# Luckick/EAGCN

Hardware: AMD Instinct MI355X
Metric: molecules/sec fwd+bwd, 2-layer 5-view EAGCN, Tox21 batch (higher is better)
Workload: dtype f32 (bf16x3 split, fp32 accumulate): every fp32 operand leaves its producer as three bf16 planes, six v_mfma_f32_32x32x16_bf16 piece products per 16 k rebuild the fp32 product (csrc/gemm_bx3.hip); aggregation, BatchNorm, head, first layer fp32

## Files before the change

eagcn_amd/_lib.py:

```python
import ctypes as C
import os

_HERE = os.path.dirname(os.path.abspath(__file__))
LIB_PATH = os.path.join(_HERE, 'lib', 'libeagcn_hip.so')

MAX_VIEWS = 8
MAX_SEGS = 8
META_WORDS = 16
META_NLOG = 8
META_T, META_NMAX, META_NTILES, META_BAD_ADJ, META_BAD_REL, META_NEDGE, META_OVERFLOW, META_EDGE_OVERFLOW = range(8)
META_NBLK = 9
STRUCT_CONCATE, STRUCT_WEIGHTED = 0, 1

_fp = C.c_void_p


class Batch(C.Structure):
    _fields_ = [('B', C.c_int32), ('N', C.c_int32), ('K', C.c_int32), ('ldc', C.c_int32),
                ('T', C.c_int32), ('n_max', C.c_int32), ('n_tiles', C.c_int32),
                ('channels', C.c_int32 * MAX_VIEWS),
                ('code', _fp), ('deg_bn', _fp), ('nat', _fp), ('row0', _fp), ('tile0', _fp),
                ('meta', _fp), ('row_mol', _fp), ('row_loc', _fp), ('row_m', _fp), ('row_deg', _fp),
                ('tile_mol', _fp), ('row_info', _fp), ('tile_info', _fp),
                ('rel_vec', _fp * MAX_VIEWS), ('rel_c', C.c_int32 * MAX_VIEWS),
# ... 33 lines not shown
    _fields_ = [('K', C.c_int32), ('mode', C.c_int32), ('att_c', C.c_int32 * MAX_VIEWS), ('att_w', _fp * MAX_VIEWS),
                ('ave_a', _fp), ('self_r', _fp), ('datt_w', _fp * MAX_VIEWS), ('dave_a', _fp), ('dself_r', _fp)]


class Layout(C.Structure):
    _fields_ = [('nseg', C.c_int32), ('width', C.c_int32 * MAX_SEGS), ('pad', C.c_int32 * MAX_SEGS)]


class LayerParams(C.Structure):
    _fields_ = [('K', C.c_int32), ('structure', C.c_int32), ('training', C.c_int32),
                ('width', C.c_int32 * MAX_VIEWS), ('inp', Layout),
                ('dropout', C.c_float), ('bn_eps', C.c_float), ('bn_momentum', C.c_float),
                ('seed', C.c_uint64), ('seed_dev', _fp),
                ('att_w', _fp * MAX_VIEWS), ('self_r', _fp * MAX_VIEWS), ('W', _fp * MAX_VIEWS),
                ('bias', _fp * MAX_VIEWS), ('gamma', _fp * MAX_VIEWS), ('beta', _fp * MAX_VIEWS),
                ('run_mean', _fp * MAX_VIEWS), ('run_var', _fp * MAX_VIEWS), ('ave_w', _fp)]


class LayerBufs(C.Structure):
    _fields_ = [('x', _fp), ('P', _fp), ('Y', _fp), ('rscale', _fp), ('bn', _fp), ('xout', _fp),
                ('pad_row', _fp), ('scratch', _fp), ('scratch_bytes', C.c_size_t),
                ('aux_stream', _fp), ('packed', _fp), ('packed_bytes', C.c_size_t),
                ('stats_hook', _fp), ('stats_user', _fp), ('x_planes', _fp), ('xout_planes', _fp)]


class LayerGrads(C.Structure):
    _fields_ = [('dW', _fp * MAX_VIEWS), ('dbias', _fp * MAX_VIEWS), ('dgamma', _fp * MAX_VIEWS),
                ('dbeta', _fp * MAX_VIEWS), ('datt_w', _fp * MAX_VIEWS), ('dself_r', _fp * MAX_VIEWS),
                ('dave_w', _fp)]


class HeadParams(C.Structure):
    _fields_ = [('f_in', C.c_int32), ('n_den1', C.c_int32), ('n_den2', C.c_int32), ('nclass', C.c_int32),
                ('dropout', C.c_float), ('bn_eps', C.c_float), ('bn_momentum', C.c_float),
                ('den1_w', _fp), ('den2_w', _fp), ('den3_w', _fp),
                ('gbn_w', _fp), ('gbn_b', _fp), ('gbn_rm', _fp), ('gbn_rv', _fp),
                ('bn1_w', _fp), ('bn1_b', _fp), ('bn1_rm', _fp), ('bn1_rv', _fp),
                ('bn2_w', _fp), ('bn2_b', _fp), ('bn2_rm', _fp), ('bn2_rv', _fp)]


class HeadGrads(C.Structure):
    _fields_ = [(n, _fp) for n in ('d_den1_w', 'd_den2_w', 'd_den3_w', 'd_gbn_w', 'd_gbn_b', 'd_bn1_w', 'd_bn1_b',
                                   'd_bn2_w', 'd_bn2_b')]


class Model(C.Structure):
    _fields_ = [('n_layers', C.c_int32), ('molfp_mode', C.c_int32), ('training', C.c_int32),
                ('head_seed', C.c_uint64), ('head_seed_dev', _fp), ('input_packed', C.c_int32), ('aux_stream', _fp),
                ('layer', LayerParams * 4), ('head', HeadParams), ('stats_hook', _fp), ('stats_user', _fp),
                ('stats_world', C.c_int32), ('fuse_readout', C.c_int32), ('fwd_signal', _fp), ('wait_flag', _fp), ('start_signal', _fp)]


class StepLoss(C.Structure):
    _fields_ = [('kind', C.c_int32), ('labels', _fp), ('class_weight', _fp), ('loss', _fp), ('scale', _fp), ('dout', _fp)]


ALLREDUCE_FN = C.CFUNCTYPE(C.c_int, C.c_void_p, C.c_int, C.c_void_p, C.c_void_p)


SIGNATURES = {
    'eagcn_abi_version': (C.c_int, []),
    'eagcn_struct_size': (C.c_size_t, [C.c_int]),
    'eagcn_last_error': (C.c_char_p, []),
    'eagcn_pad16': (C.c_int, [C.c_int]),
    'eagcn_layer_out_ld': (C.c_int, [C.POINTER(LayerParams)]),
    'eagcn_layer_fp': (C.c_int, [C.POINTER(LayerParams)]),
    'eagcn_layer_packed_bytes': (C.c_size_t, [C.POINTER(Batch), C.POINTER(LayerParams)]),
    'eagcn_layer_fwd_scratch_bytes': (C.c_size_t, [C.POINTER(Batch), C.POINTER(LayerParams)]),
    'eagcn_layer_bwd_scratch_bytes': (C.c_size_t, [C.POINTER(Batch), C.POINTER(LayerParams)]),
    'eagcn_index_build': (C.c_int, [_fp, C.POINTER(_fp), C.POINTER(Batch), _fp, _fp]),
    'eagcn_index_from_bonds': (C.c_int, [_fp, _fp, _fp, _fp, C.c_int64, C.POINTER(Batch), _fp, _fp]),
    'eagcn_index_rows': (C.c_int, [C.POINTER(Batch), _fp]),
    'eagcn_set_gemm_mode': (C.c_int, [C.c_int]),
    'eagcn_stream_wait_counter': (C.c_int, [_fp, C.c_uint32, _fp]),
    'eagcn_stream_signal_flag': (C.c_int, [_fp, _fp]),
    'eagcn_stream_wait_flag': (C.c_int, [_fp, C.c_double, _fp]),
    'eagcn_stream_wait_timeouts': (C.c_int, []),
    'eagcn_stream_wait_reset': (None, []),
    'eagcn_adam_step': (C.c_int, [_fp, _fp, _fp, _fp, C.c_int64, _fp, _fp, _fp, _fp]),
    'eagcn_agg_wants_bond_lists': (C.c_int, [C.c_int, C.c_int]),
    'eagcn_agg_wants_bond_lists_for': (C.c_int, [C.c_int, C.c_int, C.c_int]),
    'eagcn_bx3_used_splits': (C.c_int, [C.c_int, C.c_int, C.c_int, C.c_int]),
    'eagcn_set_bx3_wide': (C.c_int, [C.c_int]),
    'eagcn_bx3_pair_used_splits': (C.c_int, [C.c_int] * 7),
    'eagcn_bx3_plane_elems': (C.c_size_t, [C.c_int, C.c_int]),
    'eagcn_bx3_split': (C.c_int, [_fp, C.c_int, C.c_int, _fp, C.c_size_t, C.c_int, C.c_int, _fp]),
    'eagcn_gemm_bx3': (C.c_int, [C.c_int, C.c_int, C.c_int, C.c_int, _fp, C.c_size_t, C.c_int, C.c_int, _fp, C.c_size_t, C.c_int, C.c_int,
                                 _fp, C.c_int, C.c_int, C.c_size_t, C.c_int, _fp]),
    'eagcn_gemm_bx3_pair': (C.c_int, [C.c_int, C.c_int, C.c_int, _fp, C.c_size_t, C.c_int, C.c_int, _fp, C.c_size_t, C.c_int, C.c_int, _fp, C.c_int,
                                      C.c_int, C.c_int, C.c_int, _fp, C.c_size_t, C.c_int, C.c_int, _fp, C.c_size_t, C.c_int, C.c_int, _fp, C.c_int,
                                      C.c_int, C.c_size_t, C.c_int, _fp]),
    'eagcn_pack_rows': (C.c_int, [C.POINTER(Batch), _fp, C.c_int, C.POINTER(Layout), _fp, _fp]),
    'eagcn_unpack_rows': (C.c_int, [C.POINTER(Batch), _fp, C.POINTER(Layout), _fp, _fp, C.c_int, _fp]),
    'eagcn_pad_rows': (C.c_int, [_fp, _fp, C.c_int, C.c_int, C.c_int, _fp, _fp]),
    'eagcn_gat_scratch_bytes': (C.c_size_t, [C.POINTER(Batch), C.c_int]),
    'eagcn_gat_forward': (C.c_int, [C.POINTER(Batch), C.POINTER(GatParams), _fp, _fp, _fp, _fp, _fp]),
    'eagcn_gat_backward': (C.c_int, [C.POINTER(Batch), C.POINTER(GatParams), _fp, _fp, _fp, _fp, _fp, _fp, _fp, _fp, _fp,
                                     C.c_size_t, _fp]),
    'eagcn_pool_scratch_bytes': (C.c_size_t, []),
    'eagcn_pool_attention_forward': (C.c_int, [C.POINTER(Batch), C.POINTER(PoolAtt), _fp, C.c_int, _fp, _fp, _fp]),
    'eagcn_pool_attention_backward': (C.c_int, [C.POINTER(Batch), C.POINTER(PoolAtt), _fp, C.c_int, _fp, _fp, _fp, C.c_size_t,
                                                _fp]),
    'eagcn_pool_mix_forward': (C.c_int, [C.POINTER(Batch), C.POINTER(Layout), _fp, C.c_int, _fp, _fp, _fp, _fp, C.c_int, _fp]),
    'eagcn_pool_mix_backward': (C.c_int, [C.POINTER(Batch), C.POINTER(Layout), _fp, C.c_int, _fp, _fp, _fp, _fp, C.c_int, _fp,
                                          _fp, _fp, _fp]),
    'eagcn_pool_reduce_forward': (C.c_int, [C.POINTER(Batch), _fp, C.c_int, C.c_int, C.c_int, _fp, _fp, _fp, _fp]),
    'eagcn_pool_reduce_backward': (C.c_int, [C.POINTER(Batch), _fp, C.c_int, C.c_int, C.c_int, _fp, _fp, _fp, _fp, _fp]),
    'eagcn_layer_forward': (C.c_int, [C.POINTER(Batch), C.POINTER(LayerParams), C.POINTER(LayerBufs), _fp]),
    'eagcn_layer_backward': (C.c_int, [C.POINTER(Batch), C.POINTER(LayerParams), C.POINTER(LayerBufs),
                                       _fp, _fp, _fp, C.POINTER(LayerGrads), _fp]),
    'eagcn_attention_dense': (C.c_int, [C.POINTER(Batch), C.POINTER(LayerParams), _fp, _fp]),
    'eagcn_readout_forward': (C.c_int, [C.POINTER(Batch), _fp, C.POINTER(Layout), _fp, _fp, C.c_int, _fp,
                                        C.c_int, _fp]),
    'eagcn_readout_backward': (C.c_int, [C.POINTER(Batch), _fp, C.POINTER(Layout), _fp, C.c_int, C.c_int,
                                         _fp, _fp, _fp]),
    'eagcn_gemm_f32': (C.c_int, [C.c_int, C.c_int, C.c_int, C.c_int, C.c_int, _fp, C.c_int, _fp, C.c_int,
                                 _fp, C.c_int, _fp]),
    'eagcn_gemm_f32_dev': (C.c_int, [C.c_int, C.c_int, C.c_int, C.c_int, C.c_int, _fp, C.c_int, _fp, C.c_int,
                                     _fp, C.c_int, _fp, C.c_int, _fp]),
    'eagcn_gemm_sk_workspace_bytes': (C.c_size_t, []),
    'eagcn_gemm_f32_sk': (C.c_int, [C.c_int, C.c_int, C.c_int, C.c_int, C.c_int, _fp, C.c_int, _fp, C.c_int,
                                    _fp, C.c_int, _fp, C.c_size_t, _fp]),
    'eagcn_gemm_pair_sk': (C.c_int, [C.c_int, C.c_int, C.c_int, _fp, C.c_int, _fp, C.c_int, _fp, C.c_int,
                                     C.c_int, C.c_int, C.c_int, _fp, C.c_int, _fp, C.c_int, _fp, C.c_int,
                                     _fp, C.c_size_t, _fp]),
    'eagcn_gemm_pair_sk_slabs': (C.c_int, [C.c_int, C.c_int, C.c_int, _fp, C.c_int, _fp, C.c_int, _fp, C.c_int,
                                           C.c_int, C.c_int, C.c_int, _fp, C.c_int, _fp, C.c_int, _fp, C.c_int,
                                           C.c_size_t, _fp, C.c_size_t, _fp]),
    'eagcn_gemm_sk_plan': (C.c_int, [C.c_int] * 7 + [C.POINTER(C.c_int), C.POINTER(C.c_int)]),
    'eagcn_gemm_sk_timeouts': (C.c_int, []),
    'eagcn_gemm_sk_failed': (C.c_int, []),
    'eagcn_gemm_sk_reset_failed': (None, []),
    'eagcn_gemm_sk_inject_failure': (None, []),
    'eagcn_model_saved_bytes': (C.c_size_t, [C.POINTER(Batch), C.POINTER(Model)]),
    'eagcn_model_scratch_bytes': (C.c_size_t, [C.POINTER(Batch), C.POINTER(Model)]),
    'eagcn_model_atom_rep': (C.c_int, [C.POINTER(Batch), C.POINTER(Model), C.POINTER(C.c_size_t),
                                       C.POINTER(C.c_size_t), C.POINTER(C.c_int)]),
    'eagcn_model_atom_rep_materialize': (C.c_int, [C.POINTER(Batch), C.POINTER(Model), _fp, C.c_size_t, _fp]),
    'eagcn_model_pack_input': (C.c_int, [C.POINTER(Batch), C.POINTER(Model), _fp, _fp, C.c_size_t, _fp]),
    'eagcn_model_forward': (C.c_int, [C.POINTER(Batch), C.POINTER(Model), _fp, _fp, _fp, C.c_size_t, _fp,
                                      C.c_size_t, _fp, _fp, _fp]),
    'eagcn_model_backward': (C.c_int, [C.POINTER(Batch), C.POINTER(Model), _fp, _fp, C.c_size_t, _fp, C.c_size_t,
                                       _fp, _fp, C.POINTER(LayerGrads), C.POINTER(HeadGrads), _fp]),
    'eagcn_model_backward_range': (C.c_int, [C.POINTER(Batch), C.POINTER(Model), _fp, _fp, C.c_size_t, _fp, C.c_size_t,
                                             _fp, _fp, C.POINTER(LayerGrads), C.POINTER(HeadGrads), C.c_int, C.c_int, C.c_int, _fp]),
    'eagcn_model_input_scratch_bytes': (C.c_size_t, [C.POINTER(Batch), C.POINTER(Model)]),
    'eagcn_model_backward_input': (C.c_int, [C.POINTER(Batch), C.POINTER(Model), _fp, _fp, C.c_size_t, _fp, C.c_size_t,
                                             _fp, _fp, C.POINTER(LayerGrads), C.POINTER(HeadGrads), _fp, _fp]),
    'eagcn_attr_alpha': (C.c_float, [C.c_int, C.c_int]),
    'eagcn_attr_weight': (C.c_float, [C.c_int]),
    'eagcn_attr_acc_elems': (C.c_size_t, [C.POINTER(Batch), C.POINTER(Model)]),
    'eagcn_attr_pack_input': (C.c_int, [C.POINTER(Batch), C.POINTER(Model), _fp, _fp, C.c_float, _fp, C.c_size_t, _fp]),
    'eagcn_attr_step': (C.c_int, [C.POINTER(Batch), C.POINTER(Model), _fp, _fp, C.c_size_t, _fp, C.c_size_t, _fp, _fp, C.c_float,
                                  C.c_int, _fp, _fp]),
    'eagcn_attr_finalize': (C.c_int, [C.POINTER(Batch), C.POINTER(Model), _fp, _fp, _fp, _fp, _fp, _fp]),
    'eagcn_model_forward_step': (C.c_int, [C.POINTER(Batch), C.POINTER(Model), _fp, _fp, _fp, C.c_size_t, _fp, C.c_size_t, _fp, _fp,
                                           C.POINTER(StepLoss), _fp, C.POINTER(HeadGrads), _fp]),
    'eagcn_head_saved_bytes': (C.c_size_t, [C.POINTER(HeadParams), C.c_int]),
    'eagcn_head_scratch_bytes': (C.c_size_t, [C.POINTER(HeadParams), C.c_int]),
    'eagcn_head_forward': (C.c_int, [C.POINTER(HeadParams), C.c_int, C.c_int, C.c_uint64, _fp, _fp, _fp, C.c_size_t, _fp, C.c_size_t,
                                     _fp, _fp, _fp]),
    'eagcn_head_backward': (C.c_int, [C.POINTER(HeadParams), C.c_int, C.c_int, C.c_uint64, _fp, _fp, _fp, C.c_size_t, _fp, C.c_size_t,
                                      _fp, _fp, C.POINTER(HeadGrads), _fp, _fp]),
    'eagcn_bce_loss': (C.c_int, [_fp, _fp, _fp, C.c_int, C.c_int, _fp, _fp, _fp]),
    'eagcn_mse_loss': (C.c_int, [_fp, _fp, C.c_int, _fp, _fp, _fp]),
    'eagcn_eval_append': (C.c_int, [_fp, _fp, C.c_int, C.c_int, C.c_int, _fp, _fp, _fp, C.c_int64, _fp]),
# ... 65 lines not shown
```

eagcn_amd/build.py:

```python
import os
import shutil
import subprocess
import sys
from concurrent.futures import ThreadPoolExecutor

HERE = os.path.dirname(os.path.abspath(__file__))
CSRC = os.path.join(HERE, 'csrc')
LIBDIR = os.path.join(HERE, 'lib')
LIB = os.path.join(LIBDIR, 'libeagcn_hip.so')
HIP_SOURCES = ['index.hip', 'gemm.hip', 'gemm3.hip', 'gemm_bx3.hip', 'gemm_bx3w.hip', 'agg.hip', 'lagg.hip', 'lagg_in.hip', 'gat.hip', 'pool.hip', 'layer.hip', 'readout.hip', 'head.hip', 'head2.hip', 'loss.hip', 'attr.hip']
CPP_SOURCES = ['api.cpp']
HEADERS = ['common.h', 'kernels.h', 'lagg_kernel.h', 'gemm_x6.h', 'bx3.h', os.path.join('..', '..', 'include', 'eagcn_hip.h')]
ARCH = 'gfx950'


def _hipcc():
    for cand in (shutil.which('hipcc'), '/opt/rocm/bin/hipcc'):
        if cand and os.path.exists(cand):
            return cand
    raise RuntimeError('hipcc not found: the EAGCN HIP library cannot be built')


def _newest(paths):
    return max(os.path.getmtime(p) for p in paths)


def needs_build():
    srcs = [os.path.join(CSRC, s) for s in HIP_SOURCES + CPP_SOURCES + HEADERS if os.path.exists(os.path.join(CSRC, s))]
    return (not os.path.exists(LIB)) or os.path.getmtime(LIB) < _newest(srcs)


def build_library(force=False, verbose=False):
    if not force and not needs_build():
        return LIB
    hipcc = _hipcc()
    os.makedirs(LIBDIR, exist_ok=True)
    objdir = os.path.join(LIBDIR, 'obj')
    os.makedirs(objdir, exist_ok=True)
    flags = ['--offload-arch=' + ARCH, '-O3', '-std=c++17', '-fPIC', '-Wall', '-Wno-unused-function', '-munsafe-fp-atomics']

    hdr_time = _newest([os.path.join(CSRC, h) for h in HEADERS if os.path.exists(os.path.join(CSRC, h))])

    def compile_one(src):
        obj = os.path.join(objdir, os.path.splitext(src)[0] + '.o')
        if not force and os.path.exists(obj) and os.path.getmtime(obj) > max(hdr_time, os.path.getmtime(os.path.join(CSRC, src))):
            return obj
        cmd = [hipcc] + flags + ['-c', os.path.join(CSRC, src), '-o', obj]
        if src.endswith('.cpp'):
            cmd = [hipcc, '-O2', '-std=c++17', '-fPIC', '-c', os.path.join(CSRC, src), '-o', obj]
        r = subprocess.run(cmd, capture_output=True, text=True)
        if r.returncode != 0:
            raise RuntimeError('hipcc failed on %s:\n%s\n%s' % (src, r.stdout, r.stderr))
        if verbose and r.stderr.strip():
            print(r.stderr, file=sys.stderr)
        return obj

    sources = [s for s in HIP_SOURCES + CPP_SOURCES if os.path.exists(os.path.join(CSRC, s))]
    with ThreadPoolExecutor(max_workers=min(8, len(sources))) as ex:
        objs = list(ex.map(compile_one, sources))
    tmp = LIB + '.tmp'
    r = subprocess.run([hipcc, '--offload-arch=' + ARCH, '-shared', '-fPIC', '-o', tmp] + objs,
                       capture_output=True, text=True)
    if r.returncode != 0:
        raise RuntimeError('link failed:\n%s\n%s' % (r.stdout, r.stderr))
    os.replace(tmp, LIB)
    return LIB


if __name__ == '__main__':
    print(build_library(force='--force' in sys.argv, verbose=True))
```

eagcn_amd/csrc/attr.hip:

```cpp
#include <algorithm>

#include "common.h"
#include "kernels.h"

namespace eagcn {

__device__ __forceinline__ int attr_exact_to_packed(const ColMapD& m, int ce) {
    int eo = 0, po = 0;
    for (int s = 0; s < m.nseg; ++s) {
        if (ce < eo + m.w[s]) return po + (ce - eo);
        eo += m.w[s];
        po += m.p[s];
    }
    return -1;
}
__device__ __forceinline__ int attr_packed_to_exact(const ColMapD& m, int cp) {
    int eo = 0, po = 0;
    for (int s = 0; s < m.nseg; ++s) {
        if (cp < po + m.p[s]) return cp - po < m.w[s] ? eo + (cp - po) : -1;
        eo += m.w[s];
        po += m.p[s];
    }
    return -1;
}
// ... 7 lines not shown
        float v = 0.0f;
        if (ce >= 0) {
            const size_t i = ((size_t)bt.row_mol[r] * Nin + bt.row_loc[r]) * F + ce;
            const float b0 = base ? base[i] : 0.0f;
            v = fmaf(alpha, x[i] - b0, b0);
        }
        packed[e] = v;
    }
}

__global__ __launch_bounds__(256) void attr_accumulate_kernel(eagcn_batch bt, const float* __restrict__ g, float w, int ld, int first,
                                                               float* __restrict__ acc) {
    const uint32_t n4 = (uint32_t)dev_rows(bt) * (uint32_t)ld / 4;
    float4* a4 = reinterpret_cast<float4*>(acc);
    const float4* g4 = reinterpret_cast<const float4*>(g);
    for (uint32_t e = blockIdx.x * blockDim.x + threadIdx.x; e < n4; e += gridDim.x * blockDim.x) {
        const float4 v = g4[e];
        float4 o = first ? make_float4(0.f, 0.f, 0.f, 0.f) : a4[e];
        o.x = fmaf(w, v.x, o.x); o.y = fmaf(w, v.y, o.y); o.z = fmaf(w, v.z, o.z); o.w = fmaf(w, v.w, o.w);
        a4[e] = o;
    }
}

__global__ __launch_bounds__(256) void attr_dense_kernel(eagcn_batch bt, const float* __restrict__ acc, ColMapD m, int ld, int F, int Nin,
                                                          const float* __restrict__ x, const float* __restrict__ base,
                                                          float* __restrict__ attr, float* __restrict__ score) {
    const int nrow = bt.B * Nin;
    for (int q = blockIdx.x * blockDim.x + threadIdx.x; q < nrow; q += gridDim.x * blockDim.x) {
        const int b = q / Nin, i = q - b * Nin;
        const bool stored = i < bt.nat[b] && bt.row0[b] + i < dev_rows(bt);
        const float* ar = acc + (size_t)(stored ? bt.row0[b] + i : 0) * ld;
        const size_t o = (size_t)q * F;
        float s = 0.0f;
        for (int f = 0; f < F; ++f) {
            float v = 0.0f;
            if (stored) {
                v = ar[attr_exact_to_packed(m, f)];
                if (x) v *= x[o + f] - (base ? base[o + f] : 0.0f);
            }
            attr[o + f] = v;
            s += v;
        }
        if (score) score[q] = s;
    }
}

static inline int attr_grid(size_t n) { return (int)std::max<size_t>(1, std::min<size_t>((n + 255) / 256, 4096)); }
static inline int attr_nin(const eagcn_batch* b) { return b->n_logical > 0 ? b->n_logical : b->N; }

int launch_attr_dense(const eagcn_batch* b, const eagcn_layout* in, const float* acc, const float* x, const float* base, float* attr,
                      float* score, hipStream_t s) {
    const int Nin = attr_nin(b);
    ProfScope ps(PROF_PACK, s);
    attr_dense_kernel<<<attr_grid((size_t)b->B * Nin), 256, 0, s>>>(*b, acc, make_colmap(in), layout_ld(in), layout_width(in), Nin, x,
                                                                   base, attr, score);
    EAGCN_LAUNCH_CHECK();
    return EAGCN_OK;
}

}

using namespace eagcn;

extern "C" float eagcn_attr_alpha(int step, int steps) { return steps > 0 ? ((float)step + 0.5f) / (float)steps : 0.0f; }
extern "C" float eagcn_attr_weight(int steps) { return steps > 0 ? 1.0f / (float)steps : 0.0f; }

extern "C" size_t eagcn_attr_acc_elems(const eagcn_batch* b, const eagcn_model* m) {
    return (b && m) ? (size_t)std::max(b->T, 1) * layout_ld(&m->layer[0].in) : 0;
}

extern "C" int eagcn_attr_pack_input(const eagcn_batch* b, const eagcn_model* m, const float* afm, const float* baseline, float alpha,
                                     void* saved, size_t saved_bytes, void* stream) {
    EAGCN_CHECK_ARG(b && m && afm && saved, "eagcn_attr_pack_input: null argument");
    float* x0 = nullptr;
    int rc = model_input_slot(b, m, saved, saved_bytes, &x0, "eagcn_attr_pack_input");
    if (rc) return rc;
    if (b->T == 0) return EAGCN_OK;
    const eagcn_layout* in = &m->layer[0].in;
    hipStream_t s = (hipStream_t)stream;
    ProfScope ps(PROF_PACK, s);
    attr_pack_kernel<<<attr_grid((size_t)b->T * layout_ld(in)), 256, 0, s>>>(*b, afm, baseline, alpha, make_colmap(in), layout_ld(in),
                                                                           layout_width(in), attr_nin(b), x0);
    EAGCN_LAUNCH_CHECK();
    return EAGCN_OK;
}

extern "C" int eagcn_attr_step(const eagcn_batch* b, const eagcn_model* m, const int64_t* size, void* saved, size_t saved_bytes,
                               void* scratch, size_t scratch_bytes, const float* dout, const float* dgraph_rep, float weight, int first,
                               float* acc, void* stream) {
    EAGCN_CHECK_ARG(b && m && acc, "eagcn_attr_step: null argument");
    const int ld = layout_ld(&m->layer[0].in);
    EAGCN_CHECK_ARG((ld & 3) == 0 && (reinterpret_cast<uintptr_t>(acc) & 15) == 0,
                    "eagcn_attr_step: accumulator not 16-byte aligned / input row width %d not a multiple of 4", ld);
    float* dx0 = nullptr;
    int rc = model_backward_input_packed(b, m, size, saved, saved_bytes, scratch, scratch_bytes, dout, dgraph_rep, nullptr, nullptr,
                                         &dx0, stream, "eagcn_attr_step");
    if (rc) return rc;
    if (b->T == 0) return EAGCN_OK;
    hipStream_t s = (hipStream_t)stream;
    ProfScope ps(PROF_PACK, s);
    attr_accumulate_kernel<<<attr_grid((size_t)b->T * ld / 4), 256, 0, s>>>(*b, dx0, weight, ld, first ? 1 : 0, acc);
    EAGCN_LAUNCH_CHECK();
    return EAGCN_OK;
}

extern "C" int eagcn_attr_finalize(const eagcn_batch* b, const eagcn_model* m, const float* afm, const float* baseline, const float* acc,
                                   float* attr, float* score, void* stream) {
    EAGCN_CHECK_ARG(b && m && afm && attr && score, "eagcn_attr_finalize: null argument");
    EAGCN_CHECK_ARG(b->T == 0 || acc, "eagcn_attr_finalize: null accumulator");
    return launch_attr_dense(b, &m->layer[0].in, acc, afm, baseline, attr, score, (hipStream_t)stream);
}
```

eagcn_amd/csrc/head.hip:

```cpp
#include <stdlib.h>

#include <algorithm>

#include "common.h"
#include "kernels.h"

namespace eagcn {

__global__ void wait_counter_kernel(const uint32_t* __restrict__ word, uint32_t value, int* __restrict__ err,
                                    unsigned long long budget_ticks) {
    if (threadIdx.x == 0) {
        const unsigned long long t0 = wall_clock64();
        while ((int32_t)(__hip_atomic_load(word, __ATOMIC_ACQUIRE, __HIP_MEMORY_SCOPE_AGENT) - value) < 0) {
            __builtin_amdgcn_s_sleep(64);
            if (wall_clock64() - t0 > budget_ticks) {
                if (err) __hip_atomic_store(err, 1, __ATOMIC_RELAXED, __HIP_MEMORY_SCOPE_SYSTEM);
                break;
            }
        }
    }
}



// ... 156 lines not shown
    EAGCN_CHECK_ARG(h->f_in >= 1 && h->n_den1 >= 1 && h->n_den2 >= 1 && h->nclass >= 1, "%s: bad head sizes", who);
    EAGCN_CHECK_ARG(h->den1_w && h->den2_w && h->den3_w && h->gbn_w && h->gbn_b && h->gbn_rm && h->gbn_rv &&
                        h->bn1_w && h->bn1_b && h->bn1_rm && h->bn1_rv && h->bn2_w && h->bn2_b && h->bn2_rm &&
                        h->bn2_rv, "%s: null head parameter", who);
    const eagcn_layer_params* last = &m->layer[m->n_layers - 1];
    const int f_last = last->structure == EAGCN_STRUCT_CONCATE ? [&] { int s = 0; for (int k = 0; k < last->K; ++k) s += last->width[k]; return s; }()
                                                                 : last->width[0];
    EAGCN_CHECK_ARG(f_last == h->f_in, "%s: head expects %d features, last layer yields %d", who, h->f_in, f_last);
    EAGCN_CHECK_ARG(!m->training || b->B > 1, "%s: BatchNorm in training mode needs more than one molecule", who);
    return EAGCN_OK;
}

static eagcn_layout out_layout(const eagcn_layer_params* p) {
    eagcn_layout l;
    memset(&l, 0, sizeof(l));
    if (p->structure == EAGCN_STRUCT_CONCATE) {
        l.nseg = p->K;
        for (int k = 0; k < p->K; ++k) { l.width[k] = p->width[k]; l.pad[k] = pad16(p->width[k]); }
    } else {
        l.nseg = 1;
        l.width[0] = p->width[0];
        l.pad[0] = pad16(p->width[0]);
    }
    return l;
}

static bool fused_readout(const eagcn_model* m) {
    static const bool env = [] { const char* v = getenv("EAGCN_NO_FUSED_READOUT"); return !(v && v[0] == '1'); }();
    return env && m->fuse_readout && m->layer[m->n_layers - 1].structure == EAGCN_STRUCT_CONCATE;
}

static bool hidden_planes_only(const eagcn_batch* b, const eagcn_model* m, const ModelSaved& sv, int l) {
    return l + 1 < m->n_layers && sv.L[l].xout_planes && layer_reads_planes_only(b, &m->layer[l + 1], m->aux_stream != nullptr);
}

static void fill_drop(float p, int training, int* do_drop, uint32_t* thr, float* inv_keep) {
    *do_drop = (training && p > 0.0f) ? 1 : 0;
    *thr = (uint32_t)std::min(4294967295.0, (double)p * 4294967296.0);
    *inv_keep = 1.0f / (1.0f - p);
}

}

using namespace eagcn;

#define RC(call) do { int rc_ = (call); if (rc_) return rc_; } while (0)

extern "C" size_t eagcn_model_saved_bytes(const eagcn_batch* b, const eagcn_model* m) {
    return carve_saved(nullptr, b, m, nullptr);
}
extern "C" size_t eagcn_model_scratch_bytes(const eagcn_batch* b, const eagcn_model* m) {
    return carve_scratch(nullptr, b, m, nullptr);
}
extern "C" int eagcn_model_atom_rep(const eagcn_batch* b, const eagcn_model* m, size_t* xout_offset,
                                    size_t* pad_row_offset, int* ld) {
    EAGCN_CHECK_ARG(b && m && xout_offset && pad_row_offset && ld, "eagcn_model_atom_rep: null argument");
    ModelSaved s;
    carve_saved(nullptr, b, m, &s);
    *xout_offset = s.xout_last_off;
    *pad_row_offset = s.pad_last_off;
    *ld = eagcn_layer_out_ld(&m->layer[m->n_layers - 1]);
    return EAGCN_OK;
}

extern "C" int eagcn_model_atom_rep_materialize(const eagcn_batch* b, const eagcn_model* m, void* saved, size_t saved_bytes,
                                                 void* stream) {
    EAGCN_CHECK_ARG(b && m && saved, "eagcn_model_atom_rep_materialize: null argument");
    if (!fused_readout(m)) return EAGCN_OK;
    ModelSaved sv;
    EAGCN_CHECK_ARG(carve_saved(saved, b, m, &sv) <= saved_bytes, "eagcn_model_atom_rep_materialize: saved block too small");
    const int l = m->n_layers - 1;
    LayerSaved& L = sv.L[l];
    eagcn_layer_bufs w;
    memset(&w, 0, sizeof(w));
    w.Y = L.Y; w.bn = L.bn; w.xout = L.xout; w.pad_row = L.pad_row; w.packed = L.packed; w.packed_bytes = L.packed_bytes;
    return layer_apply_impl(b, &m->layer[l], &w, stream);
}

extern "C" int eagcn_model_pack_input(const eagcn_batch* b, const eagcn_model* m, const float* afm, void* saved,
                                      size_t saved_bytes, void* stream) {
    EAGCN_CHECK_ARG(b && m && afm && saved, "eagcn_model_pack_input: null argument");
    ModelSaved sv;
    EAGCN_CHECK_ARG(carve_saved(saved, b, m, &sv) <= saved_bytes, "eagcn_model_pack_input: saved block too small");
    return eagcn_pack_rows(b, afm, layout_width(&m->layer[0].in), &m->layer[0].in, sv.x0, stream);
}

struct HeadPlan {
    HeadFwd f1, f2, f3;
    HeadBwd b3, b2, b1;
    HeadGbn bg;
    double *st_g, *st_1, *st_2, *sb_g, *sb_1, *sb_2;
    bool sync;
};
static HeadPlan head_plan(const eagcn_batch* b, const eagcn_model* m, const ModelSaved& sv, const ModelScratch& sc, float* out,
                          float* graph_rep, const float* dout, const float* dgraph_rep, const eagcn_head_grads* hg) {
    HeadPlan P;
    const eagcn_head_params* h = &m->head;
    const int B = b->B, F = h->f_in, n1 = h->n_den1, n2 = h->n_den2, nc = h->nclass;
    P.st_g = sc.hst; P.st_1 = sc.hst + 2 * F + 2; P.st_2 = sc.hst + 2 * (F + n1) + 4;
    P.sb_g = sc.hsb; P.sb_1 = sc.hsb + 2 * F + 2; P.sb_2 = sc.hsb + 2 * (F + n1) + 4;
    P.sync = m->stats_hook && m->training;
    const int copies = P.sync ? 1 : HEAD_COPIES;
    HeadDrop nodrop{0, 0u, 1.0f, 0, nullptr}, drop1 = nodrop;
    {
        int on; uint32_t thr; float inv_keep;
        fill_drop(h->dropout, m->training, &on, &thr, &inv_keep);
        drop1 = HeadDrop{on, thr, inv_keep, m->head_seed, m->head_seed_dev};
    }
    P.f1 = HeadFwd{B, F, n1, sv.g, P.st_g, h->gbn_w, h->gbn_b, h->gbn_rm, h->gbn_rv, sv.bn_g, h->den1_w, sv.h1, nullptr, P.st_1,
                   m->training, 0, h->bn_eps, h->bn_momentum, nodrop};
    P.f2 = HeadFwd{B, n1, n2, sv.h1, P.st_1, h->bn1_w, h->bn1_b, h->bn1_rm, h->bn1_rv, sv.bn_1, h->den2_w, sv.h2, graph_rep, P.st_2,
                   m->training, 1, h->bn_eps, h->bn_momentum, drop1};
    P.f3 = HeadFwd{B, n2, nc, sv.h2, P.st_2, h->bn2_w, h->bn2_b, h->bn2_rm, h->bn2_rv, sv.bn_2, h->den3_w, out, nullptr, nullptr,
                   m->training, 1, h->bn_eps, h->bn_momentum, nodrop};
    if (P.sync) { P.f1.cnt_in = P.st_g + 2 * F; P.f2.cnt_in = P.st_1 + 2 * n1; P.f3.cnt_in = P.st_2 + 2 * n2; }
    P.f3.nw = 8;
    P.f1.signal = m->fwd_signal;
    P.f1.st_copies = P.f2.st_copies = P.f3.st_copies = copies;
    P.f1.st_stride = P.f2.st_stride = P.f3.st_stride = sc.n_hst;
    if (!hg) return P;
    const double *cn_g = sc.hst + 2 * F, *cn_1 = sc.hst + 2 * F + 2 + 2 * n1, *cn_2 = sc.hst + 2 * (F + n1) + 4 + 2 * n2;
    const float gscale = P.sync && m->stats_world > 1 ? 1.0f / (float)m->stats_world : 1.0f;
    P.b3 = HeadBwd{B, n2, nc, sv.h2, sv.bn_2, 1, nodrop, h->den3_w, dout, nullptr, nullptr, nullptr, nullptr, nullptr, nullptr,
                   sc.da2, P.sb_2, hg->d_den3_w, m->training};
    P.b2 = HeadBwd{B, n1, n2, sv.h1, sv.bn_1, 1, drop1, h->den2_w, sc.da2, sv.h2, sv.bn_2, P.sb_2, dgraph_rep, hg->d_bn2_w, hg->d_bn2_b,
                   sc.da1, P.sb_1, hg->d_den2_w, m->training};
    P.b1 = HeadBwd{B, F, n1, sv.g, sv.bn_g, 0, nodrop, h->den1_w, sc.da1, sv.h1, sv.bn_1, P.sb_1, nullptr, hg->d_bn1_w, hg->d_bn1_b,
                   sc.dgn, P.sb_g, hg->d_den1_w, m->training};
    if (P.sync) { P.b2.cnt_y = cn_2; P.b2.gscale = gscale; P.b1.cnt_y = cn_1; P.b1.gscale = gscale; }
    P.b3.nw = 8;
    const int ks = sc.hdw_ks;
    float* part3 = sc.hdw;
    float* part2 = part3 + (size_t)ks * n2 * nc;
    float* part1 = part2 + (size_t)ks * n1 * n2;
    if (ks > 1) {
        P.b3.ks = ks; P.b3.dW_part = part3;
        P.b2.ks = ks; P.b2.dW_part = part2;
        P.b1.ks = ks; P.b1.dW_part = part1;
    }
    P.bg = HeadGbn{B, F, sc.dgn, sv.g, sv.bn_g, P.sb_g, sc.dg, hg->d_gbn_w, hg->d_gbn_b, m->training};
    if (P.sync) { P.bg.cnt = cn_g; P.bg.gscale = gscale; }
    if (ks > 1) {
        P.bg.sum[0] = HeadDwSum{hg->d_den3_w, part3, n2 * nc, ks};
        P.bg.sum[1] = HeadDwSum{hg->d_den2_w, part2, n1 * n2, ks};
        P.bg.sum[2] = HeadDwSum{hg->d_den1_w, part1, F * n1, ks};
        P.bg.nsum = 3;
    }
    return P;
}

static int model_forward_trunk(const eagcn_batch* b, const eagcn_model* m, const float* afm, const int64_t* size, void* saved,
                               size_t saved_bytes, void* scratch, size_t scratch_bytes, ModelSaved& sv, ModelScratch& sc,
                               void* stream, const char* who) {
    hipStream_t s = (hipStream_t)stream;
    RC(check_model(b, m, who));
    EAGCN_CHECK_GEMM3(who);
    EAGCN_CHECK_ARG((afm || m->input_packed) && saved && scratch, "%s: null buffer", who);
    EAGCN_CHECK_ARG(m->molfp_mode == 0 || size, "%s: 'ave' read-out needs size", who);
    EAGCN_CHECK_ARG(carve_saved(saved, b, m, &sv) <= saved_bytes, "%s: saved block too small", who);
    EAGCN_CHECK_ARG(carve_scratch(scratch, b, m, &sc) <= scratch_bytes, "%s: scratch too small", who);
    const eagcn_head_params* h = &m->head;
    HandOff ho{m->start_signal, m->wait_flag, wait_err_word(), 200000000ull};
    if (!m->input_packed && (m->wait_flag || m->start_signal)) {
        handoff_kernel<<<1, 64, 0, s>>>(ho);
        EAGCN_LAUNCH_CHECK();
        ho.start = nullptr; ho.flag = nullptr;
    }
    ZeroJob zj;
    RC(gemm3_zero_job(sc.layer, sc.layer_bytes, sc.hst, (HEAD_COPIES + 1) * sc.n_hst + HEAD_WS, &zj));
    if (!m->input_packed)
        RC(eagcn_pack_rows(b, afm, layout_width(&m->layer[0].in), &m->layer[0].in, sv.x0, stream));
    const float* x = sv.x0;
    {
        const eagcn_layer_params* ps[4];
        void* pk[4];
        size_t pkb[4];
        for (int l = 0; l < m->n_layers; ++l) { ps[l] = &m->layer[l]; pk[l] = sv.L[l].packed; pkb[l] = sv.L[l].packed_bytes; }
        RC(pack_params_all(b, ps, pk, pkb, m->n_layers, stream, &zj, &ho));
    }
    for (int l = 0; l < m->n_layers; ++l) {
        LayerSaved& L = sv.L[l];
        eagcn_layer_bufs w;
        memset(&w, 0, sizeof(w));
        w.x = x; w.P = L.P; w.Y = L.Y; w.rscale = L.rscale; w.bn = L.bn; w.xout = L.xout; w.pad_row = L.pad_row;
        w.scratch = sc.layer; w.scratch_bytes = sc.layer_bytes; w.packed = L.packed; w.packed_bytes = L.packed_bytes;
        w.stats_hook = m->stats_hook; w.stats_user = m->stats_user;
        w.x_planes = l > 0 ? sv.L[l - 1].xout_planes : nullptr; w.xout_planes = L.xout_planes;
        const bool po = hidden_planes_only(b, m, sv, l);
        RC(layer_forward_impl(b, &m->layer[l], &w, stream, true, l == m->n_layers - 1 && fused_readout(m), po));
        x = po ? nullptr : L.xout;
    }
    const eagcn_layer_params* last = &m->layer[m->n_layers - 1];
    const LayerSaved& LL = sv.L[m->n_layers - 1];
    const eagcn_layout lay = out_layout(last);
    const int B = b->B, F = h->f_in, n1 = h->n_den1, n2 = h->n_den2;
    double *st_g = sc.hst, *st_1 = sc.hst + 2 * F + 2, *st_2 = sc.hst + 2 * (F + n1) + 4;
    const int copies = (m->stats_hook && m->training) ? 1 : HEAD_COPIES;
    if (fused_readout(m)) {
        ReadoutBn rb;
        rb.Y = LL.Y; rb.ldy = LL.fp; rb.bn = LL.bn; rb.fp = LL.fp;
        fill_drop(last->dropout, last->training, &rb.do_drop, &rb.thr, &rb.inv_keep);
        rb.seed = last->seed; rb.seed_dev = last->seed_dev;
        rb.size = size; rb.mode = m->molfp_mode; rb.g = sv.g; rb.F = F; rb.st = st_g;
        rb.cnt0 = st_g + 2 * F; rb.cnt1 = st_1 + 2 * n1; rb.cnt2 = st_2 + 2 * n2;
        rb.st_copies = copies; rb.st_stride = sc.n_hst;
        RC(readout_bn_forward(b, &lay, rb, stream));
    } else if (pad_sampled(m))
        RC(readout_forward_sampled(b, LL.xout, &lay, last, LL.bn + (size_t)LL.fp , size,
                                   m->molfp_mode, sv.g, F, sv.pad_cnt, sv.padc, sv.pad_tab, stream));
    else
        RC(eagcn_readout_forward(b, LL.xout, &lay, last->structure == EAGCN_STRUCT_WEIGHTED ? LL.pad_row : nullptr,
                                 size, m->molfp_mode, sv.g, F, stream));
    if (!fused_readout(m)) RC(head_colstats(sv.g, B, F, st_g, s, st_g + 2 * F, st_1 + 2 * n1, st_2 + 2 * n2));
    return EAGCN_OK;
}

static int stats_hook_call(const eagcn_model* m, bool sync, double* buf, int n, void* stream) {
    if (!sync) return EAGCN_OK;
    if (m->stats_hook(buf, n, stream, m->stats_user)) {
        set_error("eagcn_model: the sync-BatchNorm all-reduce hook failed");
        return EAGCN_ERR_HIP;
    }
    return EAGCN_OK;
}

static int head_forward_launches(const eagcn_model* m, const HeadPlan& P, void* stream) {
    hipStream_t s = (hipStream_t)stream;
    const eagcn_head_params* h = &m->head;
    RC(stats_hook_call(m, P.sync, P.st_g, 2 * h->f_in + 1, stream));
    RC(head_fwd(P.f1, s));
    RC(stats_hook_call(m, P.sync, P.st_1, 2 * h->n_den1 + 1, stream));
    RC(head_fwd(P.f2, s));
    RC(stats_hook_call(m, P.sync, P.st_2, 2 * h->n_den2 + 1, stream));
    RC(head_fwd(P.f3, s));
    return EAGCN_OK;
}
static int head_backward_launches(const eagcn_model* m, const HeadPlan& P, void* stream) {
    hipStream_t s = (hipStream_t)stream;
    const eagcn_head_params* h = &m->head;
    RC(head_bwd(P.b3, s));
    RC(stats_hook_call(m, P.sync, P.sb_2, 2 * h->n_den2, stream));
    RC(head_bwd(P.b2, s));
    RC(stats_hook_call(m, P.sync, P.sb_1, 2 * h->n_den1, stream));
    RC(head_bwd(P.b1, s));
    RC(stats_hook_call(m, P.sync, P.sb_g, 2 * h->f_in, stream));
    RC(head_gbn_bwd(P.bg, s));
    return EAGCN_OK;
}
static int readout_pad_backward(const eagcn_batch* b, const eagcn_model* m, const int64_t* size, const ModelSaved& sv,
                                const ModelScratch& sc, void* stream) {
    const eagcn_layer_params* last = &m->layer[m->n_layers - 1];
    const eagcn_layout lay = out_layout(last);
    const int F = m->head.f_in;
    if (pad_sampled(m)) return readout_backward_pad_views(b, sc.dg, &lay, size, m->molfp_mode, F, last->K, sv.pad_cnt, last->dropout, sc.dpad, stream);
    if (last->structure == EAGCN_STRUCT_WEIGHTED) return readout_backward_pad(b, sc.dg, &lay, size, m->molfp_mode, F, sc.dpad, stream);
    return EAGCN_OK;
}

extern "C" int eagcn_model_forward(const eagcn_batch* b, const eagcn_model* m, const float* afm,
                                   const int64_t* size, void* saved, size_t saved_bytes, void* scratch,
                                   size_t scratch_bytes, float* out, float* graph_rep, void* stream) {
    EAGCN_CHECK_ARG(out && graph_rep, "eagcn_model_forward: null buffer");
    ModelSaved sv;
    ModelScratch sc;
    RC(model_forward_trunk(b, m, afm, size, saved, saved_bytes, scratch, scratch_bytes, sv, sc, stream, "eagcn_model_forward"));
    const HeadPlan P = head_plan(b, m, sv, sc, out, graph_rep, nullptr, nullptr, nullptr);
    return head_forward_launches(m, P, stream);
}

namespace eagcn {
static int check_head(const eagcn_head_params* h, int B, int training, const char* who) {
    EAGCN_CHECK_ARG(h, "%s: null argument", who);
// ... 198 lines not shown
    pend_out.eacc = nullptr;
    for (int l = layer_hi; l >= layer_lo; --l) {
        const int t = top_l - l;
        float* cur = (t & 1) ? sc.dxb : sc.dxa;
        float* other = (t & 1) ? sc.dxa : sc.dxb;
        LayerSaved& L = sv.L[l];
        eagcn_layer_bufs w;
        memset(&w, 0, sizeof(w));
        w.x = l == 0 ? sv.x0 : (hidden_planes_only(b, m, sv, l - 1) ? nullptr : sv.L[l - 1].xout);
        w.P = L.P; w.Y = L.Y; w.rscale = L.rscale; w.bn = L.bn; w.xout = L.xout; w.pad_row = L.pad_row;
        w.scratch = sc.layer; w.scratch_bytes = sc.layer_bytes; w.packed = L.packed; w.packed_bytes = L.packed_bytes;
        w.aux_stream = m->aux_stream;
        w.stats_hook = m->stats_hook; w.stats_user = m->stats_user;
        w.x_planes = l > 0 ? sv.L[l - 1].xout_planes : nullptr;
        const bool top = l == top_l;
        const float* dpad = (weighted && top) ? sc.dpad : nullptr;
        RC(layer_backward_impl(b, &m->layer[l], &w, top ? nullptr : cur, top ? &rgd : nullptr, dpad,
                               l > 0 ? other : dx0, input_only ? nullptr : &lg[l], stream, top && sampled, top ? &zb : nullptr,
                               pend_in.eacc ? &pend_in : nullptr, (l > layer_lo && !input_only) ? &pend_out : nullptr, input_only));
        pend_in = pend_out;
        if (l == layer_lo) pend_in.eacc = nullptr;
    }
    if (forked) RC(stream_after(s, side));
    return EAGCN_OK;
}

extern "C" int eagcn_model_backward_range(const eagcn_batch* b, const eagcn_model* m, const int64_t* size, void* saved,
                                          size_t saved_bytes, void* scratch, size_t scratch_bytes, const float* dout,
                                          const float* dgraph_rep, const eagcn_layer_grads* lg,
                                          const eagcn_head_grads* hg, int with_head, int layer_hi, int layer_lo, void* stream) {
    RC(check_model(b, m, "eagcn_model_backward"));
    EAGCN_CHECK_GEMM3("eagcn_model_backward");
    return model_backward_impl(b, m, size, saved, saved_bytes, scratch, scratch_bytes, dout, dgraph_rep, lg, hg, with_head, layer_hi,
                               layer_lo, nullptr, false, stream);
}

struct InputScratch { float* dx0; eagcn_head_grads hg; };
static size_t carve_input_scratch(void* base, const eagcn_batch* b, const eagcn_model* m, InputScratch* out) {
    Carver2 c(base);
    c.off = carve_scratch(nullptr, b, m, nullptr);
    InputScratch t;
    const eagcn_head_params* h = &m->head;
    const size_t F = h->f_in, n1 = h->n_den1, n2 = h->n_den2, nc = h->nclass;
    t.dx0 = c.take<float>((size_t)std::max(b->T, 1) * layout_ld(&m->layer[0].in));
    t.hg.d_den1_w = c.take<float>(F * n1);
    t.hg.d_den2_w = c.take<float>(n1 * n2);
    t.hg.d_den3_w = c.take<float>(n2 * nc);
    t.hg.d_gbn_w = c.take<float>(F);
    t.hg.d_gbn_b = c.take<float>(F);
    t.hg.d_bn1_w = c.take<float>(n1);
    t.hg.d_bn1_b = c.take<float>(n1);
    t.hg.d_bn2_w = c.take<float>(n2);
    t.hg.d_bn2_b = c.take<float>(n2);
    if (out) *out = t;
    return c.off;
}

static int check_engine_model(const eagcn_batch* b, const eagcn_model* m, const char* who) {
    RC(check_model(b, m, who));
    EAGCN_CHECK_ARG(m->molfp_mode == 0 || m->molfp_mode == 1, "%s: read-out mode %d has no engine path", who, m->molfp_mode);
    for (int l = 0; l < m->n_layers; ++l)
        EAGCN_CHECK_ARG(m->layer[l].structure == EAGCN_STRUCT_CONCATE || m->layer[l].structure == EAGCN_STRUCT_WEIGHTED,
                        "%s: layer %d has structure %d, which the engine does not run", who, l, m->layer[l].structure);
    return EAGCN_OK;
}

int eagcn::model_backward_input_packed(const eagcn_batch* b, const eagcn_model* m, const int64_t* size, void* saved, size_t saved_bytes,
                                       void* scratch, size_t scratch_bytes, const float* dout, const float* dgraph_rep,
                                       const eagcn_layer_grads* lg, const eagcn_head_grads* hg, float** dx0, void* stream,
                                       const char* who) {
    EAGCN_CHECK_ARG(b && m, "%s: null argument", who);
    EAGCN_CHECK_ARG((lg == nullptr) == (hg == nullptr), "%s: lg and hg are both given (full backward) or both NULL (input-only)", who);
    RC(check_engine_model(b, m, who));
    EAGCN_CHECK_GEMM3(who);
    EAGCN_CHECK_ARG(saved && scratch && dout, "%s: null buffer", who);
    InputScratch is;
    EAGCN_CHECK_ARG(carve_input_scratch(scratch, b, m, &is) <= scratch_bytes, "%s: scratch too small (eagcn_model_input_scratch_bytes)", who);
    *dx0 = is.dx0;
    const bool input_only = lg == nullptr;
    return model_backward_impl(b, m, size, saved, saved_bytes, scratch, scratch_bytes, dout, dgraph_rep, lg, input_only ? &is.hg : hg, 1,
                               m->n_layers - 1, 0, is.dx0, input_only, stream);
}

int eagcn::model_input_slot(const eagcn_batch* b, const eagcn_model* m, void* saved, size_t saved_bytes, float** x0, const char* who) {
    ModelSaved sv;
    EAGCN_CHECK_ARG(carve_saved(saved, b, m, &sv) <= saved_bytes, "%s: saved block too small", who);
    *x0 = sv.x0;
    return EAGCN_OK;
}

extern "C" size_t eagcn_model_input_scratch_bytes(const eagcn_batch* b, const eagcn_model* m) {
    return (b && m) ? carve_input_scratch(nullptr, b, m, nullptr) : 0;
}

extern "C" int eagcn_model_backward_input(const eagcn_batch* b, const eagcn_model* m, const int64_t* size, void* saved,
                                          size_t saved_bytes, void* scratch, size_t scratch_bytes, const float* dout,
                                          const float* dgraph_rep, const eagcn_layer_grads* lg, const eagcn_head_grads* hg,
                                          float* dafm, void* stream) {
    EAGCN_CHECK_ARG(dafm, "eagcn_model_backward_input: null dafm");
    float* dx0 = nullptr;
    RC(model_backward_input_packed(b, m, size, saved, saved_bytes, scratch, scratch_bytes, dout, dgraph_rep, lg, hg, &dx0, stream,
                                   "eagcn_model_backward_input"));
    return launch_attr_dense(b, &m->layer[0].in, dx0, nullptr, nullptr, dafm, nullptr, (hipStream_t)stream);
}

extern "C" int eagcn_stream_signal_flag(uint32_t* flag, void* stream) {
    EAGCN_CHECK_ARG(flag != nullptr, "eagcn_stream_signal_flag: null flag");
    eagcn::signal_flag_kernel<<<1, 64, 0, (hipStream_t)stream>>>(flag);
    EAGCN_LAUNCH_CHECK();
    return EAGCN_OK;
}
extern "C" int eagcn_stream_wait_flag(uint32_t* flag, double budget_seconds, void* stream) {
    EAGCN_CHECK_ARG(flag != nullptr && budget_seconds > 0.0, "eagcn_stream_wait_flag: null flag / no budget");
    return eagcn::launch_wait_flag(flag, budget_seconds, (hipStream_t)stream);
}
extern "C" int eagcn_stream_wait_timeouts(void) {
    return eagcn::g_wait_err_host ? __atomic_load_n(eagcn::g_wait_err_host, __ATOMIC_RELAXED) : 0;
}
extern "C" void eagcn_stream_wait_reset(void) {
    if (eagcn::g_wait_err_host) __atomic_store_n(eagcn::g_wait_err_host, 0, __ATOMIC_RELAXED);
}

extern "C" int eagcn_stream_wait_counter(const uint32_t* counter, uint32_t value, void* stream) {
    EAGCN_CHECK_ARG(counter != nullptr, "eagcn_stream_wait_counter: null counter");
    eagcn::wait_counter_kernel<<<1, 64, 0, (hipStream_t)stream>>>(counter, value, eagcn::wait_err_word(), 200000000ull);
    EAGCN_LAUNCH_CHECK();
    return EAGCN_OK;
}
```

eagcn_amd/csrc/index.hip:

```cpp
#include <algorithm>

#include <stdlib.h>

#include "common.h"
#include "kernels.h"

namespace eagcn {

struct RelPtrs {
    const float* p[EAGCN_MAX_VIEWS];
    int c[EAGCN_MAX_VIEWS];
};

template <int NIT, int RPW>
__global__ __launch_bounds__(256) void index_scan_kernel(const float* __restrict__ adj, RelPtrs rel,
                                                          int B, int N, int Ncap, int K, int ldc,
                                                          uint8_t* __restrict__ code,
                                                          int32_t* __restrict__ deg_bn,
                                                          int32_t* __restrict__ nat,
                                                          int32_t* __restrict__ ecnt,
                                                          int32_t* __restrict__ meta) {
    const int lane = threadIdx.x & 63;
    const long row_first = ((long)blockIdx.x * 4 + (threadIdx.x >> 6)) * RPW;
    const long nrows = (long)B * N;
// ... 547 lines not shown
                for (int u = 0; u < 8; ++u) v[u] = (i0 + u < n && s_live[i0 + u]) ? code0[(size_t)(i0 + u) * bt.ldc + j] : 0;
#pragma unroll
                for (int u = 0; u < 8; ++u) cc += v[u] ? 1 : 0;
            }
        }
        s_ccnt[j] = cc;
    }
    __syncthreads();
    for (int pass = 0; pass < 2; ++pass) {
        int* cnt = pass ? s_ccnt : s_cnt;
        int v[4], tot = 0;
#pragma unroll
        for (int u = 0; u < 4; ++u) { const int i = tid * 4 + u; v[u] = i < n ? cnt[i] : 0; tot += v[u]; }
        s_scan[tid] = tot;
        __syncthreads();
        for (int o = 1; o < 256; o <<= 1) {
            const int x = tid >= o ? s_scan[tid - o] : 0;
            __syncthreads();
            s_scan[tid] += x;
            __syncthreads();
        }
        int run = s_scan[tid] - tot;
        __syncthreads();
#pragma unroll
        for (int u = 0; u < 4; ++u) {
            const int i = tid * 4 + u;
            if (i < n) {
                int* ptr = (pass ? bt.col_ptr : bt.row_ptr) + (size_t)(r0 + i) * 2;
                const bool fits = e0 + run + v[u] <= bt.E;
                ptr[0] = e0 + run;
                ptr[1] = fits ? v[u] : 0;
                cnt[i] = fits ? e0 + run : -1;
                run += v[u];
            }
        }
        __syncthreads();
    }
    auto codes = [&](int i, int j) -> uint64_t {
        uint8_t c[EAGCN_MAX_VIEWS];
#pragma unroll
        for (int k = 0; k < EAGCN_MAX_VIEWS; ++k) c[k] = k < bt.K ? code0[k * plane + (size_t)i * bt.ldc + j] : 0;
        uint64_t c64 = 0;
#pragma unroll
        for (int k = 0; k < EAGCN_MAX_VIEWS; ++k) c64 |= (uint64_t)c[k] << (8 * k);
        return c64;
    };
    for (int i = tid; i < n; i += 256) {
        int e = s_cnt[i];
        int ec = s_ccnt[i];
        if constexpr (BITMAP) {
            if (s_live[i] && e >= 0)
                for (int w = 0; w < Wn; ++w) {
                    uint32_t m = bits[i * W + w];
                    while (m) { const int j = 32 * w + __ffs(m) - 1; m &= m - 1u; bt.nbr[e] = j; bt.ecode[e] = codes(i, j); ++e; }
                }
            if (ec >= 0)
                for (int w = 0; w < Wn; ++w) {
                    uint32_t m = bitsT[i * W + w];
                    while (m) { const int ii = 32 * w + __ffs(m) - 1; m &= m - 1u; bt.tnbr[ec] = ii; bt.tcode[ec] = codes(ii, i); ++ec; }
                }
        } else {
            if (s_live[i] && e >= 0)
                for (int j = 0; j < n; ++j)
                    if (bond(i, j)) { bt.nbr[e] = j; bt.ecode[e] = codes(i, j); ++e; }
            if (ec >= 0)
                for (int ii = 0; ii < n; ++ii)
                    if (bond(ii, i)) { bt.tnbr[ec] = ii; bt.tcode[ec] = codes(ii, i); ++ec; }
        }
    }
}

typedef ColMapD ColMap;
__device__ __forceinline__ int packed_to_exact(const ColMap& m, int cp) {
    int eo = 0, po = 0;
    for (int s = 0; s < m.nseg; ++s) {
        if (cp < po + m.p[s]) return (cp - po < m.w[s]) ? eo + (cp - po) : -1;
        eo += m.w[s];
        po += m.p[s];
    }
    return -1;
}

__global__ __launch_bounds__(256) void pack_rows_kernel(eagcn_batch bt, const float* __restrict__ dense,
                                                         int F, ColMap m, int ld, float* __restrict__ packed, int Nin) {
    const uint32_t total = (uint32_t)dev_rows(bt) * (uint32_t)ld;
    for (uint32_t e = blockIdx.x * blockDim.x + threadIdx.x; e < total; e += gridDim.x * blockDim.x) {
        int r = (int)(e / (uint32_t)ld), cp = (int)(e - (uint32_t)r * (uint32_t)ld);
        int ce = packed_to_exact(m, cp);
        float v = 0.0f;
        if (ce >= 0) v = dense[((size_t)bt.row_mol[r] * Nin + bt.row_loc[r]) * F + ce];
        packed[e] = v;
    }
}

__global__ __launch_bounds__(256) void pad_rows_kernel(const float* __restrict__ rows, const int32_t* __restrict__ off,
                                                        int B, int N, int F, float* __restrict__ out) {
    const size_t total = (size_t)B * N * F;
    for (size_t e = (size_t)blockIdx.x * blockDim.x + threadIdx.x; e < total; e += (size_t)gridDim.x * blockDim.x) {
        const int f = (int)(e % F);
        const size_t bi = e / F;
        const int i = (int)(bi % N), b = (int)(bi / N);
        const int o = off[b], n = off[b + 1] - o;
        out[e] = i < n ? rows[(size_t)(o + i) * F + f] : 0.0f;
    }
}

__global__ __launch_bounds__(256) void unpack_rows_kernel(eagcn_batch bt, const float* __restrict__ packed,
                                                           ColMap m, int ld, const float* __restrict__ pad_row,
                                                           float* __restrict__ dense, int F) {
    const size_t total = (size_t)bt.B * bt.N * F;
    for (size_t e = (size_t)blockIdx.x * blockDim.x + threadIdx.x; e < total;
         e += (size_t)gridDim.x * blockDim.x) {
        int ce = (int)(e % F);
        size_t bi = e / F;
        int i = (int)(bi % bt.N), b = (int)(bi / bt.N);
        int eo = 0, po = 0, cp = -1;
        for (int s = 0; s < m.nseg; ++s) {
            if (ce < eo + m.w[s]) { cp = po + (ce - eo); break; }
            eo += m.w[s];
            po += m.p[s];
        }
        float v;
        if (i < bt.nat[b]) v = packed[(size_t)(bt.row0[b] + i) * ld + cp];
        else v = pad_row ? pad_row[cp] : 0.0f;
        dense[e] = v;
    }
}

}

using namespace eagcn;

extern "C" int eagcn_index_build(const float* adj, const float* const* rel, eagcn_batch* b,
                                 int32_t* host_meta, void* stream) {
    hipStream_t s = (hipStream_t)stream;
    EAGCN_CHECK_ARG(adj && rel && b && host_meta, "eagcn_index_build: null argument");
    EAGCN_CHECK_ARG(b->B > 0 && b->N > 0, "eagcn_index_build: B and N must be positive");
    EAGCN_CHECK_ARG(b->K >= 1 && b->K <= EAGCN_MAX_VIEWS, "eagcn_index_build: K=%d out of range", b->K);
    EAGCN_CHECK_ARG(b->ldc >= b->N && (b->ldc % 16) == 0, "eagcn_index_build: ldc must be a multiple of 16 >= N");
    EAGCN_CHECK_ARG(b->code && b->deg_bn && b->nat && b->row0 && b->tile0 && b->meta,
                    "eagcn_index_build: index buffers not allocated");
    RelPtrs rp;
    for (int k = 0; k < EAGCN_MAX_VIEWS; ++k) {
        rp.p[k] = k < b->K ? rel[k] : nullptr;
        rp.c[k] = k < b->K ? b->channels[k] : 0;
        if (k < b->K) {
            EAGCN_CHECK_ARG(rel[k] != nullptr, "eagcn_index_build: relation tensor %d is null", k);
            EAGCN_CHECK_ARG(rp.c[k] >= 1 && rp.c[k] <= EAGCN_MAX_CHANNELS,
                            "eagcn_index_build: view %d has %d channels (1..%d supported)", k, rp.c[k],
                            EAGCN_MAX_CHANNELS);
        }
    }
    const int Nin = b->n_logical > 0 ? b->n_logical : b->N;
    EAGCN_CHECK_ARG(Nin <= b->N, "eagcn_index_build: n_logical %d exceeds the capacity N=%d", Nin, b->N);
    ProfScope ps(PROF_INDEX, s);
    EAGCN_CHECK_ARG(b->ecnt && b->edge0, "eagcn_index_build: bond-list buffers not allocated");
    EAGCN_CHECK_ARG((long)b->B * b->N < (1L << 31), "eagcn_index_build: B * N = %ld rows", (long)b->B * b->N);
    {
        const int rcz = index_clear(b->meta, b->nat, b->ecnt, b->B, Nin < b->N ? b->deg_bn : nullptr, (long)b->B * b->N, s);
        if (rcz) return rcz;
    }
    const long rows = (long)b->B * Nin;
    constexpr int RPW = 1;
    const unsigned sgrid = (unsigned)((rows + 4 * RPW - 1) / (4 * RPW));
    const int nit = cdiv((Nin + 15) / 16 * 16, 256);
    EAGCN_CHECK_ARG(nit <= 4, "eagcn_index_build: N=%d exceeds the supported 1024 atoms", b->N);
    static const bool scan4 = [] { const char* v = getenv("EAGCN_SCAN4"); return !(v && v[0] == '0'); }();
    if (scan4) {
// ... 13 lines not shown
        switch (nit) {
            case 1: EAGCN_SCAN(1); break;
            case 2: EAGCN_SCAN(2); break;
            case 3: EAGCN_SCAN(3); break;
            default: EAGCN_SCAN(4); break;
        }
#undef EAGCN_SCAN
        EAGCN_LAUNCH_CHECK();
    }
    index_offsets_kernel<<<1, 1024, 0, s>>>(b->nat, b->B, b->deg_bn, b->B * b->N, b->row0, b->tile0, b->meta, b->T, b->ecnt, b->edge0, b->E, b->n_logical > 0 ? b->n_logical : 0);
    EAGCN_LAUNCH_CHECK();
    EAGCN_HIP(hipMemcpyAsync(host_meta, b->meta, EAGCN_META_WORDS * sizeof(int32_t), hipMemcpyDeviceToHost, s));
    return EAGCN_OK;
}

extern "C" int eagcn_index_from_bonds(const int32_t* bond_mol, const int32_t* bond_i, const int32_t* bond_j,
                                      const uint8_t* bond_code, int64_t E, eagcn_batch* b, int32_t* host_meta,
                                      void* stream) {
    hipStream_t s = (hipStream_t)stream;
    EAGCN_CHECK_ARG(b && host_meta, "eagcn_index_from_bonds: null argument");
    EAGCN_CHECK_ARG(E == 0 || (bond_mol && bond_i && bond_j && bond_code), "eagcn_index_from_bonds: null bond arrays");
    EAGCN_CHECK_ARG(b->B > 0 && b->N > 0 && b->K >= 1 && b->K <= EAGCN_MAX_VIEWS, "eagcn_index_from_bonds: bad batch shape");
    EAGCN_CHECK_ARG(b->ldc >= b->N && (b->ldc % 16) == 0, "eagcn_index_from_bonds: ldc must be a multiple of 16 >= N");
    EAGCN_CHECK_ARG(b->code && b->deg_bn && b->nat && b->row0 && b->tile0 && b->meta,
                    "eagcn_index_from_bonds: index buffers not allocated");
    RelPtrs rp;
    for (int k = 0; k < EAGCN_MAX_VIEWS; ++k) { rp.p[k] = nullptr; rp.c[k] = k < b->K ? b->channels[k] : 0; }
    ProfScope ps(PROF_INDEX, s);
    EAGCN_CHECK_ARG(b->ecnt && b->edge0, "eagcn_index_from_bonds: bond-list buffers not allocated");
    EAGCN_CHECK_ARG((long)b->B * b->N < (1L << 31), "eagcn_index_from_bonds: B * N = %ld rows", (long)b->B * b->N);
    {
        const int rcz = index_clear(b->meta, b->nat, b->ecnt, b->B, b->deg_bn, (long)b->B * b->N, s);
        if (rcz) return rcz;
    }
    EAGCN_HIP(hipMemsetAsync(b->code, 0, (size_t)b->K * b->B * b->N * b->ldc, s));
    if (E > 0) {
        const int grid = (int)std::min<long>((E + 255) / 256, 4096);
        index_bonds_kernel<<<grid, 256, 0, s>>>(bond_mol, bond_i, bond_j, bond_code, (long)E, b->B, b->N,
                                                b->n_logical > 0 ? std::min(b->n_logical, b->N) : b->N, b->K, b->ldc, rp,
                                                b->code, b->deg_bn, b->nat, b->ecnt, b->meta);
        EAGCN_LAUNCH_CHECK();
    }
    index_offsets_kernel<<<1, 1024, 0, s>>>(b->nat, b->B, b->deg_bn, b->B * b->N, b->row0, b->tile0, b->meta, b->T, b->ecnt, b->edge0, b->E, b->n_logical > 0 ? b->n_logical : 0);
    EAGCN_LAUNCH_CHECK();
    EAGCN_HIP(hipMemcpyAsync(host_meta, b->meta, EAGCN_META_WORDS * sizeof(int32_t), hipMemcpyDeviceToHost, s));
    return EAGCN_OK;
}

extern "C" int eagcn_index_rows(const eagcn_batch* b, void* stream) {
    hipStream_t s = (hipStream_t)stream;
    EAGCN_CHECK_ARG(b, "eagcn_index_rows: null batch");
    if (b->T == 0) return EAGCN_OK;
    EAGCN_CHECK_ARG(b->row_mol && b->row_loc && b->row_m && b->row_deg && b->tile_mol && b->row_info && b->tile_info,
                    "eagcn_index_rows: per-row buffers not allocated");
    EAGCN_CHECK_ARG(b->N <= 1024, "eagcn_index_rows: N=%d exceeds the supported 1024 atoms", b->N);
    EAGCN_CHECK_ARG(b->edge0 && b->mol_info && b->row_ptr && b->col_ptr && (b->E == 0 || (b->nbr && b->tnbr && b->ecode && b->tcode)),
                    "eagcn_index_rows: bond-list buffers not allocated");
    ProfScope ps(PROF_INDEX, s);
    index_rows_kernel<<<b->B, 256, 0, s>>>(*b);
    EAGCN_LAUNCH_CHECK();
    if (!b->build_lists) return EAGCN_OK;
    const int rb = b->blk ? lagg_block_rows(b) : 0;
    const int W = (b->N + 31) / 32;
    const size_t dyn = (size_t)2 * b->N * W * sizeof(uint32_t);
    static const size_t lds_cap = [] {
        int dev = 0, v = 0;
        if (hipGetDevice(&dev) != hipSuccess || hipDeviceGetAttribute(&v, hipDeviceAttributeMaxSharedMemoryPerBlock, dev) != hipSuccess) v = 64 * 1024;
        size_t cap = (size_t)v > 12 * 1024 ? (size_t)v - 12 * 1024 : 0;
        if (cap > 52 * 1024 &&
            hipFuncSetAttribute((const void*)index_csr_kernel<true>, hipFuncAttributeMaxDynamicSharedMemorySize, (int)cap) != hipSuccess) {
            (void)hipGetLastError();
            cap = 52 * 1024;
        }
        return cap;
    }();
    if (b->N <= 512 && dyn <= lds_cap) index_csr_kernel<true><<<b->B + (rb > 0 ? 1 : 0), 256, dyn, s>>>(*b, W, rb);
    else index_csr_kernel<false><<<b->B + (rb > 0 ? 1 : 0), 256, 0, s>>>(*b, W, rb);
    EAGCN_LAUNCH_CHECK();
    return EAGCN_OK;
}

extern "C" int eagcn_pack_rows(const eagcn_batch* b, const float* dense, int F, const eagcn_layout* lay,
                               float* packed, void* stream) {
    hipStream_t s = (hipStream_t)stream;
    EAGCN_CHECK_ARG(b && dense && lay && packed, "eagcn_pack_rows: null argument");
    EAGCN_CHECK_ARG(layout_width(lay) == F, "eagcn_pack_rows: layout width %d != F %d", layout_width(lay), F);
    if (b->T == 0) return EAGCN_OK;
    int ld = layout_ld(lay);
    size_t total = (size_t)b->T * ld;
    int grid = (int)std::min<size_t>((total + 255) / 256, 4096);
    ProfScope ps(PROF_PACK, s);
    pack_rows_kernel<<<grid, 256, 0, s>>>(*b, dense, F, make_colmap(lay), ld, packed, b->n_logical > 0 ? b->n_logical : b->N);
    EAGCN_LAUNCH_CHECK();
    return EAGCN_OK;
}

extern "C" int eagcn_pad_rows(const float* rows, const int32_t* mol_offset, int B, int N, int F, float* out, void* stream) {
    hipStream_t s = (hipStream_t)stream;
    EAGCN_CHECK_ARG(rows && mol_offset && out && B > 0 && N > 0 && F > 0, "eagcn_pad_rows: bad argument");
    const size_t total = (size_t)B * N * F;
    ProfScope ps(PROF_PACK, s);
    pad_rows_kernel<<<(int)std::min<size_t>((total + 255) / 256, 4096), 256, 0, s>>>(rows, mol_offset, B, N, F, out);
    EAGCN_LAUNCH_CHECK();
    return EAGCN_OK;
}

extern "C" int eagcn_unpack_rows(const eagcn_batch* b, const float* packed, const eagcn_layout* lay,
                                 const float* pad_row, float* dense, int F, void* stream) {
    hipStream_t s = (hipStream_t)stream;
    EAGCN_CHECK_ARG(b && lay && dense, "eagcn_unpack_rows: null argument");
    EAGCN_CHECK_ARG(b->T == 0 || packed, "eagcn_unpack_rows: null packed matrix");
    EAGCN_CHECK_ARG(layout_width(lay) == F, "eagcn_unpack_rows: layout width %d != F %d", layout_width(lay), F);
    int ld = layout_ld(lay);
    size_t total = (size_t)b->B * b->N * F;
    int grid = (int)std::min<size_t>((total + 255) / 256, 4096);
    ProfScope ps(PROF_PACK, s);
    unpack_rows_kernel<<<grid, 256, 0, s>>>(*b, packed, make_colmap(lay), ld, pad_row, dense, F);
    EAGCN_LAUNCH_CHECK();
    return EAGCN_OK;
}
```

eagcn_amd/csrc/kernels.h:

```cpp
#pragma once
#include "bx3.h"
#include "common.h"

namespace eagcn {

struct AggArgs {
    eagcn_batch bt;
    ViewCols vc;
    const float* src; int lds;
    float* dst; int ldd;
    const float* sig;
    const float* rsig;
    float* rscale;
    double* stats;
    int nchunk;
    int cpw = 1;
    int xcd = 0;
    bool w_rowm = false;
    BxOut planes = {nullptr, 0, 0, 0};
    const float* bn_tab = nullptr; const float* bn_cc = nullptr; int bn_fp = 0;
    const float* w_aw = nullptr;
    int w_drop = 0; uint32_t w_thr = 0; float w_inv_keep = 1.0f; uint64_t w_seed = 0; const uint64_t* w_seed_dev = nullptr;
};
int agg_grid_x(const eagcn_batch* b);
bool agg_ksplit(const eagcn_batch* b);
int launch_agg(AggArgs a, bool trans, hipStream_t s);
constexpr int LAGG_RB = 256;
constexpr int LAGG_MAXM = 16;
struct EdgeArgs;
int lagg_parts();
bool lagg_wfuse();
bool lagg_use(const eagcn_batch* b, int dir, bool absorbs_bn, const ViewCols* vc = nullptr);
bool lagg_wanted(int B, int N, int structure);
int lagg_block_rows(const eagcn_batch* b);
int lagg_slabs(const eagcn_batch* b);
int launch_lagg_fwd(AggArgs a, hipStream_t s);
int launch_lagg_bwd(AggArgs a, const EdgeArgs& e, hipStream_t s, bool edge = true);
int launch_lagg_bwd_input(const AggArgs& a, const EdgeArgs& e, dim3 grid, hipStream_t s);

struct EdgeArgs {
    eagcn_batch bt;
    ViewCols vc;
    const float* dY; const float* Y; const float* P; int ld;
    const float* sig; const float* rsig; const float* rscale;
    double* datt;
    int atomic;
    int xcd = 0;
};
constexpr int EDGE_SLAB = 264;
constexpr int EDGE_COPIES = 8;
inline size_t edge_acc_bytes() { return align256((size_t)EDGE_COPIES * EAGCN_MAX_VIEWS * EDGE_SLAB * sizeof(double)); }
int edge_grid_x(const eagcn_batch* b);
int launch_edge_grad(const EdgeArgs& a, hipStream_t s);
int launch_agg_edge(AggArgs a, const EdgeArgs& e, hipStream_t s);

enum { BN_SC = 0, BN_SH, BN_MU, BN_INV };

struct ColMapD {
    int nseg;
    int w[EAGCN_MAX_SEGS], p[EAGCN_MAX_SEGS];
};
inline ColMapD make_colmap(const eagcn_layout* l) {
    ColMapD m;
    m.nseg = l->nseg;
    for (int i = 0; i < EAGCN_MAX_SEGS; ++i) {
        m.w[i] = i < l->nseg ? l->width[i] : 0;
        m.p[i] = i < l->nseg ? l->pad[i] : 0;
    }
    return m;
}

struct ReadoutGrad {
    const float* dg; int F;
    const int64_t* size; int mode;
    ColMapD map;
};
int launch_readout_bwd_rows(const eagcn_batch* b, const ReadoutGrad& rg, int ld, float* dx, hipStream_t s);
struct G2Prob {
    const float* A; const float* B; float* C;
    int lda, ldb, ldc;
    int M, N, K;
    const int* M_dev;
    const int* K_dev;
};
struct DwScatter {
    float* dW[EAGCN_MAX_VIEWS];
    ViewCols vc;
    ColMapD in;
    int in_identity;
};
constexpr int G3_XSEG = 8;
struct G3Plan {
    int a[G3_XSEG + 1];
    int c[G3_XSEG + 1];
};
__host__ __device__ inline void g3_plan(int RB, int CT0, int ipt0, int T1, int ipt1, int G, G3Plan& pl) {
    const long total = (long)RB * CT0 * ipt0 + (long)T1 * ipt1;
    const int R = 4 * G;
    const long per = total / R, rem = total - per * R;
    const int qn = G >> 3, rn = G & 7;
    pl.a[0] = 0;
    pl.c[0] = 0;
    for (int x = 1; x < G3_XSEG; ++x) {
        const long L = 4L * (x * qn + (x < rn ? x : rn));
        const long tgt = L * per + (L < rem ? L : rem);
        int a = (int)(((long)RB * L + R / 2) / R);
        a = a < pl.a[x - 1] ? pl.a[x - 1] : (a > RB ? RB : a);
        long cc = T1 > 0 ? (tgt - (long)a * CT0 * ipt0 + T1 / 2) / T1 : 0;
        if (tgt - (long)a * CT0 * ipt0 < 0) cc = 0;
        int c = (int)(cc > ipt1 ? ipt1 : cc);
        c = c < pl.c[x - 1] ? pl.c[x - 1] : c;
        pl.a[x] = a;
        pl.c[x] = c;
    }
    pl.a[G3_XSEG] = RB;
    pl.c[G3_XSEG] = ipt1;
}
size_t gemm3_workspace_bytes();
bool gemm3_xk_enabled();
int gemm3_grid();
int gemm3_clear_flags(void* workspace, size_t bytes, hipStream_t s, double* zero = nullptr, int nzero = 0);
// ... 11 lines not shown
inline int gemm_planes() { const int m = gemm_mode(); return m == 3 ? 3 : m == 4 ? 1 : 0; }
struct ZeroJob { unsigned* u; int nu; double* d; int nd; };
struct HandOff { uint32_t* start; uint32_t* flag; int* err; unsigned long long budget; };
__device__ __forceinline__ void handoff_body(const HandOff& h) {
    if (h.start) __hip_atomic_fetch_add(h.start, 1u, __ATOMIC_RELEASE, __HIP_MEMORY_SCOPE_AGENT);
    if (h.flag) {
        const unsigned long long t0 = wall_clock64();
        while (__hip_atomic_load(h.flag, __ATOMIC_ACQUIRE, __HIP_MEMORY_SCOPE_AGENT) == 0u) {
            __builtin_amdgcn_s_sleep(8);
            if (wall_clock64() - t0 > h.budget) {
                if (h.err) __hip_atomic_store(h.err, 1, __ATOMIC_RELAXED, __HIP_MEMORY_SCOPE_SYSTEM);
                break;
            }
        }
        __hip_atomic_store(h.flag, 0u, __ATOMIC_RELAXED, __HIP_MEMORY_SCOPE_AGENT);
    }
}
int gemm3_zero_job(void* workspace, size_t bytes, double* zero, int nzero, ZeroJob* out);
int zero_fill(void* p, size_t bytes, hipStream_t s);
bool gemm3_ok(const GemmDesc& g);
int launch_gemm3(const GemmDesc& g, const DwScatter* sc, void* workspace, size_t bytes, hipStream_t s);
int launch_gemm3_pair(const GemmDesc& dx, const GemmDesc& dw, const DwScatter* sc, void* workspace, size_t bytes, hipStream_t s,
                      size_t xk_slab = 0);

constexpr int HEAD_COPIES = 8;
struct HeadDrop { int on; uint32_t thr; float inv_keep; uint64_t seed; const uint64_t* seed_dev; };
struct HeadFwd {
    int B, K, N;
    const float* x; const double* st_in; const float *gamma, *beta; float *run_mean, *run_var; float* bn;
    const float* W; float* y; float* y2; double* st_out;
    int training, relu; float eps, momentum; HeadDrop drop;
    const double* cnt_in = nullptr;
    int st_copies = 1, st_stride = 0;
    const float* lab = nullptr; int nlab = 0; unsigned* lab_cnt = nullptr;
    int nw = 0;
    uint32_t* signal = nullptr;
};
struct HeadBwd {
    int B, K, N;
    const float* x; const float* bnp; int relu_p; HeadDrop drop; const float* W;
    const float* dy; const float* y; const float* bny; const double* sb_y; const float* extra;
    float *dgamma_y, *dbeta_y; float* dyp; double* sb_p; float* dW; int training;
    const double* cnt_y = nullptr;
    float gscale = 1.0f;
    int ks = 1; float* dW_part = nullptr;
    int nw = 0;
};
inline int head_dw_chunks(int B) { return B > 256 ? (B + 255) / 256 < 16 ? (B + 255) / 256 : 16 : 1; }
struct HeadDwSum { float* dst; const float* part; int n, ks; };
struct HeadGbn { int B, F; const float *dgn, *g, *bn; const double* sb; float *dg, *dgamma, *dbeta; int training;
                 const double* cnt = nullptr; float gscale = 1.0f;
                 HeadDwSum sum[3] = {}; int nsum = 0; };
struct HeadLoss { int kind;
                  const float* labels; const float* weight; float* loss; const float* scale; float* dout; };
struct HeadMid { HeadFwd f3; HeadBwd b3; HeadLoss L;
                 double* ws; };
constexpr int HEAD_WS = 4;
struct HeadLossFin { float* loss; const double* ws; const float* scale; int kind, n; };
bool head_mid_ok(int n_den2, int nclass);
int head_mid(const HeadMid& a, hipStream_t s);
int head_bwd_pair(const HeadBwd& a, const HeadBwd& e, const HeadLossFin& lf, hipStream_t s);
int head_colstats(const float* g, int B, int F, double* st, hipStream_t s, double* cnt0 = nullptr, double* cnt1 = nullptr,
                  double* cnt2 = nullptr);
int head_fwd(const HeadFwd& a, hipStream_t s);
int head_bwd(const HeadBwd& a, hipStream_t s);
int head_gbn_bwd(const HeadGbn& a, hipStream_t s);

struct EdgeDrain {
    double* eacc; int K;
    float* datt_w[EAGCN_MAX_VIEWS]; float* dself_r[EAGCN_MAX_VIEWS]; int channels[EAGCN_MAX_VIEWS];
    const float* rsig;
};
int layer_backward_impl(const eagcn_batch* b, const eagcn_layer_params* p, const eagcn_layer_bufs* w,
                        const float* dxout, const ReadoutGrad* rg, const float* dpad_row, float* dx,
                        const eagcn_layer_grads* g, void* stream, bool dpad_views = false,
                        const ZeroJob* zero_after = nullptr, const EdgeDrain* drain_in = nullptr, EdgeDrain* drain_out = nullptr,
                        bool input_only = false);
int model_backward_input_packed(const eagcn_batch* b, const eagcn_model* m, const int64_t* size, void* saved, size_t saved_bytes,
                                void* scratch, size_t scratch_bytes, const float* dout, const float* dgraph_rep,
                                const eagcn_layer_grads* lg, const eagcn_head_grads* hg, float** dx0, void* stream, const char* who);
int launch_attr_dense(const eagcn_batch* b, const eagcn_layout* in, const float* acc, const float* x, const float* base, float* attr,
                      float* score, hipStream_t s);
int model_input_slot(const eagcn_batch* b, const eagcn_model* m, void* saved, size_t saved_bytes, float** x0, const char* who);
int layer_forward_impl(const eagcn_batch* b, const eagcn_layer_params* p, const eagcn_layer_bufs* w, void* stream,
                       bool prepacked, bool skip_apply = false, bool planes_only = false);
bool layer_reads_planes_only(const eagcn_batch* b, const eagcn_layer_params* p, bool aux_stream);
int layer_apply_impl(const eagcn_batch* b, const eagcn_layer_params* p, const eagcn_layer_bufs* w, void* stream);
int pack_params_all(const eagcn_batch* b, const eagcn_layer_params* const* ps, void* const* packed,
                    const size_t* packed_bytes, int n, void* stream, const ZeroJob* zj = nullptr, const HandOff* ho = nullptr);
struct ReadoutBn {
    const float* Y; int ldy;
    const float* bn; int fp;
    int do_drop; uint32_t thr; float inv_keep; uint64_t seed; const uint64_t* seed_dev;
    const int64_t* size; int mode;
    float* g; int F;
    double* st;
    int st_copies = 1, st_stride = 0;
    bool pair = false;
    double *cnt0, *cnt1, *cnt2;
};
int readout_bn_forward(const eagcn_batch* b, const eagcn_layout* lay, const ReadoutBn& a, void* stream);
int readout_forward_sampled(const eagcn_batch* b, const float* x, const eagcn_layout* lay, const eagcn_layer_params* p,
                            const float* bn_sh, const int64_t* size, int mode, float* g, int F, uint16_t* cnt, float* padc,
                            uint32_t* tab, void* stream);
int readout_backward_pad_views(const eagcn_batch* b, const float* dg, const eagcn_layout* lay, const int64_t* size, int mode,
                               int F, int K, const uint16_t* cnt, float dropout, float* dpad, void* stream);
int readout_backward_pad(const eagcn_batch* b, const float* dg, const eagcn_layout* lay, const int64_t* size,
                         int mode, int F, float* dpad_row, void* stream);

}
```

eagcn_amd/csrc/layer.hip:

```cpp
#include <algorithm>

#include <stdlib.h>

#include "common.h"
#include "kernels.h"

namespace eagcn {

struct ParamPtrs {
    const float* att_w[EAGCN_MAX_VIEWS];
    const float* self_r[EAGCN_MAX_VIEWS];
    const float* W[EAGCN_MAX_VIEWS];
    const float* bias[EAGCN_MAX_VIEWS];
    const float* gamma[EAGCN_MAX_VIEWS];
    const float* beta[EAGCN_MAX_VIEWS];
    float* run_mean[EAGCN_MAX_VIEWS];
    float* run_var[EAGCN_MAX_VIEWS];
    const float* ave_w;
    int channels[EAGCN_MAX_VIEWS];
    const float* rel_vec[EAGCN_MAX_VIEWS];
    int rel_c[EAGCN_MAX_VIEWS];
};
__device__ __forceinline__ float att_logit(const ParamPtrs& pp, int k, int c) {
    if (!pp.rel_vec[k]) return pp.att_w[k][c - 1];
// ... 469 lines not shown
                for (int v = 0; v < EAGCN_MAX_VIEWS; ++v) da[v] += (v == k) ? dak : 0.0;
            }
        }
    }
    if (weighted && !APPLY) {
#pragma unroll
        for (int v = 0; v < EAGCN_MAX_VIEWS; ++v) {
            const double t = wave_sum(da[v]);
            if ((threadIdx.x & 63) == 0 && t != 0.0) atomicAdd(&da_s[v], t);
        }
        __syncthreads();
        if (threadIdx.x < EAGCN_MAX_VIEWS)
            a.slab_da[((size_t)blockIdx.y * gridDim.x + blockIdx.x) * EAGCN_MAX_VIEWS + threadIdx.x] = da_s[threadIdx.x];
    }
}

template <int L>
__global__ __launch_bounds__(256) void bn_bwd_finalize_kernel(const double* __restrict__ slab,
                                                               const double* __restrict__ slab_da, int nslab,
                                                               int fp, double M, int training,
                                                               const float* __restrict__ bn, ViewCols vc,
                                                               GradPtrs gp, float* __restrict__ cc, const int32_t* __restrict__ meta, int nvirt,
                                                               int batch_B, int da_chunks, int da_stride,
                                                               const double* __restrict__ gsum, double* __restrict__ zero, int nzero) {
    if (blockIdx.x == 0 && zero)
        for (int i = threadIdx.x; i < nzero; i += blockDim.x) zero[i] = 0.0;
    if (meta[EAGCN_META_NLOG] > 0) M = (double)batch_B * (double)meta[EAGCN_META_NLOG];
    nslab = max(1, min(nslab, (meta[EAGCN_META_T] + nvirt + BWD_ROWS - 1) / BWD_ROWS));
    const int cpr = blockIdx.x * (256 / L) + threadIdx.x / L, sl = threadIdx.x % L;
    const int cp = min(cpr, fp - 1);
    if (blockIdx.x == 0 && gp.dave_w) {
        const int v = threadIdx.x >> 5, l = threadIdx.x & 31;
        double t = 0.0;
        if (v < vc.K)
            for (int y = 0; y < da_chunks; ++y)
                for (int s = l; s < nslab; s += 32) t += slab_da[((size_t)y * da_stride + s) * EAGCN_MAX_VIEWS + v];
#pragma unroll
        for (int o = 16; o > 0; o >>= 1) t += __shfl_xor(t, o);
        if (v < vc.K && l == 0) gp.dave_w[v] = (float)t;
    }
    double s1, s2;
    slab_sum<L>(slab, nslab, fp, cp, sl, s1, s2);
    if (cpr >= fp || sl != 0) return;
    {
        double g1 = s1, g2 = s2;
        if (gsum) { g1 = gsum[2 * cp]; g2 = gsum[2 * cp + 1]; M = gsum[2 * fp]; }
        cc[cp] = training ? (float)(g1 / M) : 0.0f;
        cc[fp + cp] = training ? (float)(g2 / M) : 0.0f;
    }
    const int k = col_view(vc, cp), f = cp - vc.off[k];
    if (f < vc.width[k]) {
        gp.dgamma[k][f] = (float)s2;
        gp.dbeta[k][f] = (float)s1;
        gp.dbias[k][f] = training ? 0.0f : (float)((double)bn[BN_SC * fp + cp] * s1);
    }
}

__global__ __launch_bounds__(256) void bn_bwd_apply_kernel(eagcn_batch bt, int fp, const float* __restrict__ Y, int ldy,
                                                            const float* __restrict__ bn,
                                                            const float* __restrict__ cc, float* __restrict__ dH) {
    const uint32_t g4 = fp / 4;
    const uint32_t total = (uint32_t)dev_rows(bt) * g4;
    for (uint32_t e = blockIdx.x * blockDim.x + threadIdx.x; e < total; e += gridDim.x * blockDim.x) {
        const int r = (int)(e / g4), c = (int)(e - (uint32_t)r * g4) * 4;
        const float4 y = *reinterpret_cast<const float4*>(Y + (size_t)r * ldy + c);
        float4 d = *reinterpret_cast<float4*>(dH + (size_t)r * fp + c);
        const float4 sc = *reinterpret_cast<const float4*>(bn + BN_SC * fp + c);
        const float4 mu = *reinterpret_cast<const float4*>(bn + BN_MU * fp + c);
        const float4 iv = *reinterpret_cast<const float4*>(bn + BN_INV * fp + c);
        const float4 c1 = *reinterpret_cast<const float4*>(cc + c);
        const float4 c2 = *reinterpret_cast<const float4*>(cc + fp + c);
        d.x = sc.x * (d.x - c1.x - (y.x - mu.x) * iv.x * c2.x);
        d.y = sc.y * (d.y - c1.y - (y.y - mu.y) * iv.y * c2.y);
        d.z = sc.z * (d.z - c1.z - (y.z - mu.z) * iv.z * c2.z);
        d.w = sc.w * (d.w - c1.w - (y.w - mu.w) * iv.w * c2.w);
        *reinterpret_cast<float4*>(dH + (size_t)r * fp + c) = d;
    }
}

__global__ __launch_bounds__(256) void unpack_grads_kernel(GradPtrs gp, ParamPtrs pp, ViewCols vc, ColMapD in,
                                                            int ld_in, int fp, const float* __restrict__ dWcat,
                                                            int nsplit, size_t slab, double* __restrict__ datt,
                                                            int nedge, const float* __restrict__ rsig, int wblocks,
                                                            const int32_t* __restrict__ meta, int xk_G, int edge_drain, int bx_per, int bx_wide) {
    nedge = nedge < 0 ? -nedge : min(nedge, (meta[EAGCN_META_T] + 15) / 16);
    const int bxm = bx_wide ? BX3W_BM : BX3_BM, bxn = bx_wide ? BX3W_BN : BX3_BN;
    nsplit = nsplit < 0 ? bx3_used_splits_wave(-nsplit, meta[EAGCN_META_T], ((ld_in + bxm - 1) / bxm) * ((fp + bxn - 1) / bxn),
                                          bx_per > 0 ? ((meta[EAGCN_META_T] + bxm - 1) / bxm) * ((ld_in + bxn - 1) / bxn) : 0, max(1, (fp + 31) >> 5), bx_per)
                        : max(1, min(nsplit, meta[EAGCN_META_T] >> 7));
    if ((int)blockIdx.x < wblocks) {
        const int tid = blockIdx.x * blockDim.x + threadIdx.x;
        if (xk_G > 0) {
            const int e = tid;
            if (e >= ld_in * fp) return;
            const int ip = e / fp, cp = e % fp;
            const int k = col_view(vc, cp), f = cp - vc.off[k];
            const int fi = packed_to_exact(in, ip);
            if (fi < 0 || f >= vc.width[k]) return;
            const int T = meta[EAGCN_META_T];
            G3Plan pl;
            g3_plan((T + 63) / 64, (ld_in + 63) / 64, max(1, (fp + 15) / 16), ((ld_in + 63) / 64) * ((fp + 63) / 64),
                    max(1, (T + 15) / 16), xk_G, pl);
            float v[G3_XSEG];
#pragma unroll
            for (int x = 0; x < G3_XSEG; ++x) v[x] = pl.c[x + 1] > pl.c[x] ? dWcat[(size_t)x * slab + e] : 0.0f;
            float t = 0.0f;
#pragma unroll
            for (int x = 0; x < G3_XSEG; ++x) t += v[x];
            gp.dW[k][(size_t)fi * vc.width[k] + f] = T > 0 ? t : 0.0f;
            return;
        }
        const int sub = tid & 3;
        const int e = (tid >> 2) * 4;
        if (e >= ld_in * fp) return;
        const int ip = e / fp, cp = e % fp;
        const int k = col_view(vc, cp), f = cp - vc.off[k];
        const int fi = packed_to_exact(in, ip);
        if (fi < 0 || f >= vc.width[k]) return;
        float4 s0 = make_float4(0.f, 0.f, 0.f, 0.f), s1 = s0;
        int z = sub;
#pragma unroll 4
        for (; z + 4 < nsplit; z += 8) {
            const float4 a0 = *reinterpret_cast<const float4*>(dWcat + (size_t)z * slab + e);
            const float4 a1 = *reinterpret_cast<const float4*>(dWcat + (size_t)(z + 4) * slab + e);
            s0.x += a0.x; s0.y += a0.y; s0.z += a0.z; s0.w += a0.w;
            s1.x += a1.x; s1.y += a1.y; s1.z += a1.z; s1.w += a1.w;
        }
        if (z < nsplit) {
            const float4 a0 = *reinterpret_cast<const float4*>(dWcat + (size_t)z * slab + e);
            s0.x += a0.x; s0.y += a0.y; s0.z += a0.z; s0.w += a0.w;
        }
        float t[4] = {s0.x + s1.x, s0.y + s1.y, s0.z + s1.z, s0.w + s1.w};
#pragma unroll
        for (int j = 0; j < 4; ++j) { t[j] += __shfl_xor(t[j], 1); t[j] += __shfl_xor(t[j], 2); }
        const float tv = sub == 0 ? t[0] : sub == 1 ? t[1] : sub == 2 ? t[2] : t[3];
        if (f + sub < vc.width[k]) gp.dW[k][(size_t)fi * vc.width[k] + f + sub] = tv;
        return;
    }
    const int er = ((int)blockIdx.x - wblocks) * 16 + (threadIdx.x >> 4), sl = threadIdx.x & 15;
    const int tot = vc.K * EDGE_SLAB;
    const int e = min(er, tot - 1);
    const int k = e / EDGE_SLAB, c = e % EDGE_SLAB;
    const bool general = pp.rel_vec[k] != nullptr && c != 256;
    double t = 0.0;
    if (!general) {
        for (int z0 = sl; z0 < nedge; z0 += 16 * 8) {
            double v[8];
#pragma unroll
            for (int u = 0; u < 8; ++u) {
                const int z = z0 + 16 * u;
                v[u] = z < nedge ? datt[(size_t)z * tot + e] : 0.0;
            }
#pragma unroll
            for (int u = 0; u < 8; ++u) t += v[u];
            if (edge_drain && er < tot) {
#pragma unroll
                for (int u = 0; u < 8; ++u) {
                    const int z = z0 + 16 * u;
                    if (z < nedge) datt[(size_t)z * tot + e] = 0.0;
                }
            }
        }
    } else if (c >= 1 && c <= pp.rel_c[k]) {
        const float* vec = pp.rel_vec[k];
        const int C = pp.rel_c[k], D = pp.channels[k];
        for (int z = sl; z < nedge; z += 16)
            for (int code = 1; code <= D; ++code)
                t += datt[(size_t)z * tot + k * EDGE_SLAB + code] * (double)vec[(size_t)(code - 1) * C + (c - 1)];
    }
#pragma unroll
    for (int o = 8; o > 0; o >>= 1) t += __shfl_xor(t, o);
    if (er >= tot || sl != 0) return;
    if (c == 256) {
        const double r = (double)rsig[k];
        gp.dself_r[k][0] = (float)(t * r * (1.0 - r));
    } else if (c >= 1 && c <= (pp.rel_vec[k] ? pp.rel_c[k] : pp.channels[k])) {
        gp.datt_w[k][c - 1] = (float)t;
    }
}

__global__ __launch_bounds__(256) void attention_dense_kernel(eagcn_batch bt, ParamPtrs pp, float* __restrict__ out) {
    const size_t total = (size_t)bt.K * bt.B * bt.N * bt.N;
    for (size_t e = (size_t)blockIdx.x * blockDim.x + threadIdx.x; e < total;
         e += (size_t)gridDim.x * blockDim.x) {
        const int j = (int)(e % bt.N);
        const size_t kbi = e / bt.N;
        const int k = (int)(kbi / ((size_t)bt.B * bt.N));
        const size_t bi = kbi - (size_t)k * bt.B * bt.N;
        const uint32_t c = bt.deg_bn[bi] > 0 ? bt.code[kbi * bt.ldc + j] : 0u;
        out[e] = (c >= 1 && (int)c <= pp.channels[k]) ? sigmoidf_(att_logit(pp, k, (int)c)) : 0.0f;
    }
}

struct Carver {
    char* base;
    size_t off = 0;
    explicit Carver(void* p) : base((char*)p) {}
    template <typename T>
    T* take(size_t n) {
        T* p = base ? (T*)(base + off) : nullptr;
        off = align256(off + n * sizeof(T));
        return p;
    }
};

struct LayerDims {
    ViewCols vc;
    int fp, ld_in, fin, ldo, gx, gxb, nsplit;
    int gslab;
    size_t wslab;
    size_t wpslab, wtpslab;
    int np;
    int bx_splits;
};
static LayerDims layer_dims(const eagcn_batch* b, const eagcn_layer_params* p) {
    LayerDims d;
    d.vc = view_cols(p);
    d.fp = d.vc.off[p->K];
    d.ld_in = layout_ld(&p->in);
    d.fin = layout_width(&p->in);
    d.ldo = p->structure == EAGCN_STRUCT_CONCATE ? d.fp : pad16(p->width[0]);
    d.gx = agg_grid_x(b);
    d.gslab = std::max(d.gx, lagg_use(b, 0, false, &d.vc) ? lagg_slabs(b) : 0);
    {
        const long by_rows = cdiv(b->T + 1, BWD_ROWS);
        const long by_bytes = std::max<long>(64, (32L << 20) / ((long)d.fp * 16));
        d.gxb = (int)std::max<long>(1, std::min<long>(std::min<long>(by_rows, 2048), by_bytes));
    }
    const int tiles = cdiv(d.ld_in, 64) * cdiv(d.fp, 64);
    d.nsplit = std::max(1, std::min(std::max(1, 1024 / tiles), cdiv(std::max(b->T, 1), 128)));
    d.wslab = (size_t)d.ld_in * d.fp;
    d.wpslab = bx_plane_elems(d.ld_in, d.fp);
    d.wtpslab = bx_plane_elems(d.fp, d.ld_in);
    d.np = (d.ld_in >= 128 && (d.ld_in & 15) == 0 && (d.fp & 15) == 0) ? gemm_planes() : 0;
    d.bx_splits = std::max(1, std::min(std::min(1023, std::max(64, cdiv(std::max(b->T, 1), 4096))), std::max(cdiv(std::max(b->T, 1), 4096), cdiv(std::max(b->T, 1), 256))));
    return d;
}

static bool gemm3_layer(int ld_in) {
    static const bool on = [] { const char* v = getenv("EAGCN_NO_GEMM3"); return !(v && v[0] == '1'); }();
    return on && ld_in >= 128 && gemm_mode() != 2;
}

struct Packed { float *Wcat, *WcatT, *colp, *sig, *rsig; uint16_t *Wp, *WTp; };
struct FwdScratch { void* gws; double* eacc; float *Wcat, *WcatT, *colp, *sig, *rsig; uint16_t *Wp, *WTp; double* stats; double* gsum;
                    uint16_t* xp; };
static size_t carve_packed(void* base, const LayerDims& d, Packed* s) {
    Carver c(base);
    Packed t;
    t.Wcat = c.take<float>(d.wslab);
    t.WcatT = c.take<float>(d.wslab);
    t.colp = c.take<float>((size_t)CP_ROWS * d.fp);
    t.sig = c.take<float>(EAGCN_MAX_VIEWS * 256);
    t.rsig = c.take<float>(EAGCN_MAX_VIEWS);
    t.Wp = c.take<uint16_t>(d.np ? (size_t)d.np * d.wpslab : 1);
    t.WTp = c.take<uint16_t>(d.np ? (size_t)d.np * d.wtpslab : 1);
    if (s) *s = t;
    return c.off;
}
struct BwdScratch {
    void* gws;
    double* eacc;
    float *Wcat, *WcatT, *colp, *sig, *rsig, *dY, *dP, *cc, *dWcat;
    uint16_t *Wp, *WTp;
    double *slab, *slab_da, *datt, *gsum;
    uint16_t *dPp, *xp;
};
static size_t carve_fwd(void* base, const eagcn_batch* b, const LayerDims& d, FwdScratch* s) {
    Carver c(base);
    FwdScratch t;
    t.gws = c.take<char>(gemm3_workspace_bytes());
    t.eacc = (double*)c.take<char>(edge_acc_bytes());
    t.Wcat = c.take<float>(d.wslab);
    t.WcatT = c.take<float>(d.wslab);
    t.colp = c.take<float>((size_t)CP_ROWS * d.fp);
    t.sig = c.take<float>(EAGCN_MAX_VIEWS * 256);
    t.rsig = c.take<float>(EAGCN_MAX_VIEWS);
    t.Wp = c.take<uint16_t>(d.np ? (size_t)d.np * d.wpslab : 1);
    t.WTp = c.take<uint16_t>(d.np ? (size_t)d.np * d.wtpslab : 1);
    t.stats = c.take<double>((size_t)d.gslab * d.fp * 2);
    t.gsum = c.take<double>((size_t)2 * d.fp + 8);
    t.xp = c.take<uint16_t>(d.np ? (size_t)d.np * bx_plane_elems(b->T, d.ld_in) : 1);
    if (s) *s = t;
    return c.off;
}
static size_t carve_bwd(void* base, const eagcn_batch* b, const LayerDims& d, BwdScratch* s) {
    Carver c(base);
    BwdScratch t;
    t.gws = c.take<char>(gemm3_workspace_bytes());
    t.eacc = (double*)c.take<char>(edge_acc_bytes());
    t.Wcat = c.take<float>(d.wslab);
    t.WcatT = c.take<float>(d.wslab);
    t.colp = c.take<float>((size_t)CP_ROWS * d.fp);
    t.sig = c.take<float>(EAGCN_MAX_VIEWS * 256);
    t.rsig = c.take<float>(EAGCN_MAX_VIEWS);
    t.Wp = c.take<uint16_t>(d.np ? (size_t)d.np * d.wpslab : 1);
    t.WTp = c.take<uint16_t>(d.np ? (size_t)d.np * d.wtpslab : 1);
    t.dY = c.take<float>((size_t)std::max(b->T, 1) * d.fp);
    t.dP = c.take<float>((size_t)std::max(b->T, 1) * d.fp);
    t.cc = c.take<float>((size_t)2 * d.fp);
    t.dWcat = c.take<float>(d.wslab * std::max(std::max(d.nsplit, G3_XSEG), d.np ? d.bx_splits : 1));
    t.slab = c.take<double>((size_t)d.gxb * d.fp * 2);
    t.slab_da = c.take<double>((size_t)d.gxb * cdiv(d.fp, 1024) * EAGCN_MAX_VIEWS);
    t.datt = c.take<double>((size_t)edge_grid_x(b) * EAGCN_MAX_VIEWS * EDGE_SLAB);
    t.gsum = c.take<double>((size_t)2 * d.fp + 8);
    t.dPp = c.take<uint16_t>(d.np ? (size_t)d.np * bx_plane_elems(b->T, d.fp) : 1);
    t.xp = c.take<uint16_t>(d.np ? (size_t)d.np * bx_plane_elems(b->T, d.ld_in) : 1);
    if (s) *s = t;
    return c.off;
}

static int check_layer(const eagcn_batch* b, const eagcn_layer_params* p, const char* who) {
    EAGCN_CHECK_ARG(b && p, "%s: null argument", who);
    EAGCN_CHECK_ARG(p->K >= 1 && p->K <= EAGCN_MAX_VIEWS && p->K == b->K,
                    "%s: layer has %d views, batch index has %d", who, p->K, b->K);
    EAGCN_CHECK_ARG(p->structure == EAGCN_STRUCT_CONCATE || p->structure == EAGCN_STRUCT_WEIGHTED,
                    "%s: unknown structure %d", who, p->structure);
    EAGCN_CHECK_ARG(p->in.nseg >= 1 && p->in.nseg <= EAGCN_MAX_SEGS, "%s: bad input layout", who);
    for (int s = 0; s < p->in.nseg; ++s)
        EAGCN_CHECK_ARG(p->in.width[s] >= 1 && p->in.pad[s] >= p->in.width[s] && (p->in.pad[s] % 4) == 0,
                        "%s: input segment %d: width %d pad %d (pad must be a multiple of 4 >= width)", who, s,
                        p->in.width[s], p->in.pad[s]);
    for (int k = 0; k < p->K; ++k) {
        EAGCN_CHECK_ARG(p->width[k] >= 1, "%s: view %d has width %d", who, k, p->width[k]);
        EAGCN_CHECK_ARG(p->att_w[k] && p->self_r[k] && p->W[k] && p->bias[k] && p->gamma[k] && p->beta[k] &&
                            p->run_mean[k] && p->run_var[k], "%s: view %d has a null parameter", who, k);
        if (p->structure == EAGCN_STRUCT_WEIGHTED)
            EAGCN_CHECK_ARG(p->width[k] == p->width[0], "%s: Weighted_sum needs equal view widths", who);
    }
    if (p->structure == EAGCN_STRUCT_WEIGHTED) EAGCN_CHECK_ARG(p->ave_w, "%s: Weighted_sum needs ave_w", who);
    EAGCN_CHECK_ARG(p->dropout >= 0.0f && p->dropout < 1.0f, "%s: dropout %f out of [0,1)", who, p->dropout);
    EAGCN_CHECK_ARG((uint64_t)std::max(b->T, 0) * (uint64_t)view_cols(p).off[p->K] / 4 < (1ull << 32),
                    "%s: %d rows x %d packed columns exceed the 32-bit element index of the BatchNorm passes", who, b->T,
                    view_cols(p).off[p->K]);
    return EAGCN_OK;
}

static ParamPtrs param_ptrs(const eagcn_batch* b, const eagcn_layer_params* p) {
    ParamPtrs pp;
    memset(&pp, 0, sizeof(pp));
    for (int k = 0; k < p->K; ++k) {
        pp.att_w[k] = p->att_w[k]; pp.self_r[k] = p->self_r[k]; pp.W[k] = p->W[k]; pp.bias[k] = p->bias[k];
        pp.gamma[k] = p->gamma[k]; pp.beta[k] = p->beta[k]; pp.run_mean[k] = p->run_mean[k];
        pp.run_var[k] = p->run_var[k]; pp.channels[k] = b->channels[k];
        pp.rel_vec[k] = b->rel_vec[k]; pp.rel_c[k] = b->rel_c[k];
    }
    pp.ave_w = p->structure == EAGCN_STRUCT_WEIGHTED ? p->ave_w : nullptr;
    return pp;
}

static inline int ew_grid(size_t n) { return (int)std::max<size_t>(1, std::min<size_t>((n + 255) / 256, 2048)); }

}

static int apply_launch_(const eagcn_batch* b, const eagcn_layer_params* p, const eagcn_layer_bufs* w, const eagcn::LayerDims& d,
                         const float* colp, hipStream_t s, bool planes_only = false);
#define apply_launch apply_launch_

using namespace eagcn;

extern "C" int eagcn_pad16(int w) { return pad16(w); }
extern "C" int eagcn_layer_fp(const eagcn_layer_params* p) { return view_cols(p).off[p->K]; }
extern "C" int eagcn_layer_out_ld(const eagcn_layer_params* p) {
    return p->structure == EAGCN_STRUCT_CONCATE ? eagcn_layer_fp(p) : pad16(p->width[0]);
}
extern "C" size_t eagcn_layer_packed_bytes(const eagcn_batch* b, const eagcn_layer_params* p) {
    LayerDims d = layer_dims(b, p);
    return carve_packed(nullptr, d, nullptr);
}
extern "C" size_t eagcn_layer_fwd_scratch_bytes(const eagcn_batch* b, const eagcn_layer_params* p) {
    LayerDims d = layer_dims(b, p);
    return carve_fwd(nullptr, b, d, nullptr);
}
extern "C" size_t eagcn_layer_bwd_scratch_bytes(const eagcn_batch* b, const eagcn_layer_params* p) {
    LayerDims d = layer_dims(b, p);
    return carve_bwd(nullptr, b, d, nullptr);
}

extern "C" int eagcn_layer_forward(const eagcn_batch* b, const eagcn_layer_params* p, const eagcn_layer_bufs* w,
                                   void* stream) {
    EAGCN_CHECK_GEMM3("eagcn_layer_forward");
    if (w && w->scratch && w->scratch_bytes >= gemm3_workspace_bytes()) {
        int rc = gemm3_clear_flags(w->scratch, w->scratch_bytes, (hipStream_t)stream);
        if (rc) return rc;
    }
    return layer_forward_impl(b, p, w, stream, false);
}

int eagcn::pack_params_all(const eagcn_batch* b, const eagcn_layer_params* const* ps, void* const* packed,
                           const size_t* packed_bytes, int n, void* stream, const ZeroJob* zj, const HandOff* ho) {
    hipStream_t s = (hipStream_t)stream;
    EAGCN_CHECK_ARG(n >= 1 && n <= 4, "pack_params_all: 1..4 layers");
    PackJob jobs[4];
    size_t wmax = 0;
    for (int l = 0; l < 4; ++l) {
        const int ll = l < n ? l : n - 1;
        int rc = check_layer(b, ps[ll], "eagcn_model_forward");
        if (rc) return rc;
        const LayerDims d = layer_dims(b, ps[ll]);
        Packed pk;
        const size_t pneed = carve_packed(packed[ll], d, &pk);
        if (pneed > packed_bytes[ll]) {
            set_error("pack_params_all: packed buffer of layer %d too small (%zu < %zu)", ll, packed_bytes[ll], pneed);
            return EAGCN_ERR_SCRATCH;
        }
        jobs[l].pp = param_ptrs(b, ps[ll]); jobs[l].vc = d.vc; jobs[l].in = make_colmap(&ps[ll]->in);
        jobs[l].ld_in = d.ld_in; jobs[l].fp = d.fp;
        jobs[l].Wcat = pk.Wcat; jobs[l].WcatT = pk.WcatT; jobs[l].colp = pk.colp; jobs[l].sig = pk.sig; jobs[l].rsig = pk.rsig;
        jobs[l].wp = BxOut{d.np ? pk.Wp : nullptr, d.wpslab, d.np, d.ld_in};
        jobs[l].wtp = BxOut{d.np ? pk.WTp : nullptr, d.wtpslab, d.np, d.fp};
        if (l < n) wmax = std::max(wmax, d.wslab);
    }
    PackJobs pj{jobs[0], jobs[1], jobs[2], jobs[3]};
    ProfScope ps_(PROF_PACK, s);
    const ZeroJob none{nullptr, 0, nullptr, 0};
    const HandOff noho{nullptr, nullptr, nullptr, 0};
    pack_params_multi_kernel<<<dim3(ew_grid(wmax), n), 256, 0, s>>>(pj, zj ? *zj : none, ho ? *ho : noho);
    EAGCN_LAUNCH_CHECK();
    return EAGCN_OK;
}

int eagcn::layer_forward_impl(const eagcn_batch* b, const eagcn_layer_params* p, const eagcn_layer_bufs* w,
                              void* stream, bool prepacked, bool skip_apply, bool planes_only) {
    hipStream_t s = (hipStream_t)stream;
    int rc = check_layer(b, p, "eagcn_layer_forward");
    if (rc) return rc;
    EAGCN_CHECK_ARG(w && w->bn && w->xout && w->pad_row && w->scratch, "eagcn_layer_forward: null buffer");
    EAGCN_CHECK_ARG(b->T == 0 || ((w->x || w->x_planes) && w->P && w->Y && w->rscale), "eagcn_layer_forward: null activation buffer");
    EAGCN_CHECK_ARG(!planes_only || (w->xout_planes && gemm_planes()), "eagcn_layer_forward: planes-only output without plane images");
    const LayerDims d = layer_dims(b, p);
    FwdScratch sc;
    const size_t need = carve_fwd(w->scratch, b, d, &sc);
    if (need > w->scratch_bytes) {
        set_error("eagcn_layer_forward: scratch too small (%zu < %zu)", w->scratch_bytes, need);
        return EAGCN_ERR_SCRATCH;
    }
    const ParamPtrs pp = param_ptrs(b, p);
    const ColMapD in = make_colmap(&p->in);
    if (w->packed) {
        Packed pk;
        const size_t pneed = carve_packed(w->packed, d, &pk);
        if (pneed > w->packed_bytes) {
            set_error("eagcn_layer_forward: packed buffer too small (%zu < %zu)", w->packed_bytes, pneed);
            return EAGCN_ERR_SCRATCH;
        }
        sc.Wcat = pk.Wcat; sc.WcatT = pk.WcatT; sc.colp = pk.colp; sc.sig = pk.sig; sc.rsig = pk.rsig;
        sc.Wp = pk.Wp; sc.WTp = pk.WTp;
    }
    EAGCN_CHECK_ARG(!prepacked || w->packed, "eagcn_layer_forward: prepacked parameters need the packed block");
    if (!prepacked) {
        ProfScope ps(PROF_PACK, s);
        pack_params_kernel<<<ew_grid(d.wslab), 256, 0, s>>>(pp, d.vc, in, d.ld_in, d.fp, sc.Wcat, sc.WcatT, sc.colp, sc.sig, sc.rsig,
                                                            BxOut{d.np ? sc.Wp : nullptr, d.wpslab, d.np, d.ld_in},
                                                            BxOut{d.np ? sc.WTp : nullptr, d.wtpslab, d.np, d.fp});
    }
    EAGCN_LAUNCH_CHECK();
    double fsum = 0.0;
    for (int k = 0; k < p->K; ++k) fsum += p->width[k];
    const double gemm_work = 2.0 * (double)b->T * (double)d.fin * fsum;
    int nslab = 0, tiles_per_wg = agg_ksplit(b) ? 1 : 4;
    if (b->T > 0) {
        GemmDesc g3{0, 1, b->T, d.fp, d.ld_in, w->x, d.ld_in, sc.WcatT, d.ld_in, w->P, d.fp, 1, 0, gemm_work};
        g3.M_dev = b->meta + EAGCN_META_T;
        BxProb bp;
        memset(&bp, 0, sizeof(bp));
        if (d.np) {
            const size_t xstride = bx_plane_elems(b->T, d.ld_in);
            const uint16_t* xp = w->x_planes;
            if (!xp) {
                EAGCN_CHECK_ARG(w->x, "eagcn_layer_forward: neither an fp32 input nor its plane images");
                rc = launch_bx3_split(w->x, b->T, b->meta + EAGCN_META_T, d.ld_in, sc.xp, xstride, b->T, d.np, s);
                if (rc) return rc;
                xp = sc.xp;
            }
            bp.A = BxPlanes{xp, xstride, d.ld_in, b->T}; bp.B = BxPlanes{sc.WTp, d.wtpslab, d.ld_in, d.fp}; bp.C = w->P; bp.ldc = d.fp;
            bp.M = b->T; bp.N = d.fp; bp.K = d.ld_in; bp.M_dev = b->meta + EAGCN_META_T; bp.tn = 0; bp.splits = 1;
        }
        if (d.np && bx3_ok(bp)) {
            rc = launch_bx3(bp, nullptr, d.np, s, gemm_work, PROF_GEMM, bx3_pick_wide(bp, nullptr, b->t_hint));
        } else if (!w->x) {
            set_error("eagcn_layer_forward: the input exists as plane images only and the plane product does not apply");
            return EAGCN_ERR_ARG;
        } else if (gemm3_layer(d.ld_in) && gemm3_ok(g3)) {
            rc = launch_gemm3(g3, nullptr, sc.gws, gemm3_workspace_bytes(), s);
        } else {
            GemmDesc g{0, 0, b->T, d.fp, d.ld_in, w->x, d.ld_in, sc.Wcat, d.fp, w->P, d.fp, 1, 0, gemm_work};
            g.M_dev = b->meta + EAGCN_META_T;
            rc = launch_gemm(g, s);
        }
        if (rc) return rc;
        {
            AggArgs a;
            a.bt = *b; a.vc = d.vc; a.src = w->P; a.lds = d.fp; a.dst = w->Y; a.ldd = d.fp;
            a.sig = sc.sig; a.rsig = sc.rsig; a.rscale = w->rscale; a.stats = sc.stats; a.nchunk = 1;
            if (lagg_use(b, 0, false, &d.vc)) {
                rc = launch_lagg_fwd(a, s);
                nslab = lagg_slabs(b);
                tiles_per_wg = -1;
            } else {
                rc = launch_agg(a, false, s);
                nslab = d.gx;
            }
            if (rc) return rc;
        }
    }
    const double M = (double)b->B * (double)b->N;
    {
    ProfScope psbn(PROF_BN, s);
    if (w->stats_hook && p->training) {
        if (nslab > 64) bn_stats_sum_kernel<64><<<cdiv(d.fp, 4), 256, 0, s>>>(sc.stats, nslab, d.fp, M, sc.gsum, b->meta, 1, tiles_per_wg, 0, b->B);
        else bn_stats_sum_kernel<16><<<cdiv(d.fp, 16), 256, 0, s>>>(sc.stats, nslab, d.fp, M, sc.gsum, b->meta, 1, tiles_per_wg, 0, b->B);
        EAGCN_LAUNCH_CHECK();
        if (w->stats_hook(sc.gsum, 2 * d.fp + 1, stream, w->stats_user)) {
            set_error("eagcn_layer_forward: the sync-BatchNorm all-reduce hook failed");
            return EAGCN_ERR_HIP;
        }
        bn_finalize_kernel<16><<<cdiv(d.fp, 16), 256, 0, s>>>(sc.gsum, 1, d.fp, M, p->training, p->bn_eps, p->bn_momentum, sc.colp,
                                                                pp, d.vc, w->bn, b->meta, 0, b->B, sc.gsum + 2 * d.fp);
    } else if (nslab > 64)
        bn_finalize_kernel<64><<<cdiv(d.fp, 4), 256, 0, s>>>(sc.stats, nslab, d.fp, M, p->training, p->bn_eps,
                                                               p->bn_momentum, sc.colp, pp, d.vc, w->bn, b->meta, tiles_per_wg, b->B, nullptr);
    else
        bn_finalize_kernel<16><<<cdiv(d.fp, 16), 256, 0, s>>>(sc.stats, nslab, d.fp, M, p->training, p->bn_eps,
                                                                p->bn_momentum, sc.colp, pp, d.vc, w->bn, b->meta, tiles_per_wg, b->B, nullptr);
    EAGCN_LAUNCH_CHECK();
    }
    if (skip_apply) return EAGCN_OK;
    return apply_launch(b, p, w, d, sc.colp, s, planes_only);
}

bool eagcn::layer_reads_planes_only(const eagcn_batch* b, const eagcn_layer_params* p, bool aux_stream) {
    static const bool on = [] { const char* v = getenv("EAGCN_PLANES_ONLY"); return !(v && v[0] == '0'); }();
    if (!on || aux_stream || !b || !p || b->T <= 0) return false;
    const LayerDims d = layer_dims(b, p);
    if (!d.np) return false;
    const uint16_t* pl = reinterpret_cast<const uint16_t*>(static_cast<uintptr_t>(4096));
    float* fo = reinterpret_cast<float*>(static_cast<uintptr_t>(4096));
    const size_t xstride = bx_plane_elems(b->T, d.ld_in), pstride = bx_plane_elems(b->T, d.fp);
    BxProb bp, bx, bw;
    memset(&bp, 0, sizeof(bp)); memset(&bx, 0, sizeof(bx)); memset(&bw, 0, sizeof(bw));
    bp.A = BxPlanes{pl, xstride, d.ld_in, b->T}; bp.B = BxPlanes{pl, d.wtpslab, d.ld_in, d.fp}; bp.C = fo; bp.ldc = d.fp;
    bp.M = b->T; bp.N = d.fp; bp.K = d.ld_in; bp.M_dev = b->meta + EAGCN_META_T; bp.tn = 0; bp.splits = 1;
    bx.A = BxPlanes{pl, pstride, d.fp, b->T}; bx.B = BxPlanes{pl, d.wpslab, d.fp, d.ld_in}; bx.C = fo; bx.ldc = d.ld_in;
    bx.M = b->T; bx.N = d.ld_in; bx.K = d.fp; bx.M_dev = b->meta + EAGCN_META_T; bx.tn = 0; bx.splits = 1;
// ... 73 lines not shown
    EAGCN_CHECK_ARG(!input_only || (dx && !drain_in), "eagcn_layer_backward: the input-only form needs dx and takes no edge reduction");
    EAGCN_CHECK_ARG(b->T == 0 || ((dxout || rg) && (input_only || w->x || w->x_planes) && w->P && w->Y && w->rscale),
                    "eagcn_layer_backward: null activation buffer");
    if (!input_only)
        for (int k = 0; k < p->K; ++k)
            EAGCN_CHECK_ARG(g->dW[k] && g->dbias[k] && g->dgamma[k] && g->dbeta[k] && g->datt_w[k] && g->dself_r[k],
                            "eagcn_layer_backward: view %d has a null gradient buffer", k);
    const LayerDims d = layer_dims(b, p);
    BwdScratch sc;
    const size_t need = carve_bwd(w->scratch, b, d, &sc);
    if (need > w->scratch_bytes) {
        set_error("eagcn_layer_backward: scratch too small (%zu < %zu)", w->scratch_bytes, need);
        return EAGCN_ERR_SCRATCH;
    }
    const ParamPtrs pp = param_ptrs(b, p);
    GradPtrs gp;
    memset(&gp, 0, sizeof(gp));
    if (input_only) {
        EAGCN_CHECK_ARG(d.wslab >= (size_t)3 * d.fp + EAGCN_MAX_VIEWS, "eagcn_layer_backward: no room for the discarded BatchNorm gradients");
        for (int k = 0; k < p->K; ++k) {
            gp.dgamma[k] = sc.dWcat + d.vc.off[k];
            gp.dbeta[k] = sc.dWcat + d.fp + d.vc.off[k];
            gp.dbias[k] = sc.dWcat + 2 * d.fp + d.vc.off[k];
        }
        gp.dave_w = p->structure == EAGCN_STRUCT_WEIGHTED ? sc.dWcat + 3 * d.fp : nullptr;
    } else {
        for (int k = 0; k < p->K; ++k) {
            gp.dW[k] = g->dW[k]; gp.dbias[k] = g->dbias[k]; gp.dgamma[k] = g->dgamma[k]; gp.dbeta[k] = g->dbeta[k];
            gp.datt_w[k] = g->datt_w[k]; gp.dself_r[k] = g->dself_r[k];
        }
        gp.dave_w = p->structure == EAGCN_STRUCT_WEIGHTED ? g->dave_w : nullptr;
    }
    const ColMapD in = make_colmap(&p->in);
    if (w->packed) {
        Packed pk;
        const size_t pneed = carve_packed(w->packed, d, &pk);
        if (pneed > w->packed_bytes) {
            set_error("eagcn_layer_backward: packed buffer too small (%zu < %zu)", w->packed_bytes, pneed);
            return EAGCN_ERR_SCRATCH;
        }
        sc.Wcat = pk.Wcat; sc.WcatT = pk.WcatT; sc.colp = pk.colp; sc.sig = pk.sig; sc.rsig = pk.rsig;
        sc.Wp = pk.Wp; sc.WTp = pk.WTp;
    } else {
        ProfScope ps(PROF_PACK, s);
        pack_params_kernel<<<ew_grid(d.wslab), 256, 0, s>>>(pp, d.vc, in, d.ld_in, d.fp, sc.Wcat, sc.WcatT, sc.colp, sc.sig, sc.rsig,
                                                            BxOut{d.np ? sc.Wp : nullptr, d.wpslab, d.np, d.ld_in},
                                                            BxOut{d.np ? sc.WTp : nullptr, d.wtpslab, d.np, d.fp});
    }
    EAGCN_LAUNCH_CHECK();
    double fsum = 0.0;
    for (int k = 0; k < p->K; ++k) fsum += p->width[k];
    const double gemm_work = 2.0 * (double)b->T * (double)d.fin * fsum;

    BwdArgs ba;
    ba.meta = b->meta; ba.Tcap = b->T; ba.row_mol = b->row_mol; ba.row_m = b->row_m;
    ba.vc = d.vc; ba.structure = p->structure; ba.fp = d.fp;
    ba.nvirt = (dpad_row && p->structure == EAGCN_STRUCT_WEIGHTED) ? 1 : 0;
    ba.dxout = dxout; ba.ldo = d.ldo; ba.dpad = dpad_row; ba.dpad_views = dpad_views ? 1 : 0;
    if (rg) ba.rg = *rg; else memset(&ba.rg, 0, sizeof(ba.rg)); ba.Y = w->Y; ba.ldy = d.fp; ba.bn = w->bn;
    ba.colp = sc.colp; ba.dH = sc.dY; ba.slab = sc.slab; ba.slab_da = sc.slab_da;
    ba.do_drop = (p->training && p->dropout > 0.0f) ? 1 : 0;
    ba.thr = (uint32_t)std::min(4294967295.0, (double)p->dropout * 4294967296.0);
    ba.inv_keep = 1.0f / (1.0f - p->dropout);
    ba.seed = p->seed;
    ba.seed_dev = p->seed_dev;
    ba.zero = zero_after ? zero_after->d : nullptr;
    ba.nzero = zero_after ? zero_after->nd : 0;
    if (drain_in && drain_in->eacc) ba.drain = *drain_in; else memset(&ba.drain, 0, sizeof(ba.drain));
    const int rows = b->T + ba.nvirt;
    const int gxb = std::max(1, std::min(rows, d.gxb));
    bool fused_bn_apply = false, fused_w_apply = false, w_rows = false, fused_c_apply = false;
    bool lagg_bwd = false;
    {
        static const bool edge_atomic0 = [] { const char* v = getenv("EAGCN_EDGE_SLABS"); return !(v && v[0] == '1'); }();
        bool general0 = false;
        for (int k = 0; k < p->K; ++k) general0 = general0 || pp.rel_vec[k] != nullptr;
        const bool wt0 = p->structure == EAGCN_STRUCT_WEIGHTED;
        const bool absorbs = lagg_fuses_bn() && (!bn_bwd_two_pass(wt0) || (wt0 && lagg_wfuse()));
        lagg_bwd = b->T > 0 && edge_atomic0 && !general0 && lagg_use(b, 1, absorbs);
        if (input_only) lagg_bwd = b->T > 0 && lagg_use(b, 1, true);
    }
    const double M = (double)b->B * (double)b->N;
    const bool eval_in = input_only && !p->training;
    if (eval_in) {
        const bool wt = p->structure == EAGCN_STRUCT_WEIGHTED, dg = ba.rg.dg != nullptr;
        if (b->T > 0 && lagg_bwd) {
            if (dg) {
                rc = launch_readout_bwd_rows(b, ba.rg, d.ldo, sc.dY, s);
                if (rc) return rc;
                w_rows = true;
            }
            if (wt) fused_w_apply = true; else fused_c_apply = true;
        } else if (b->T > 0) {
            rc = zero_fill(sc.cc, (size_t)2 * d.fp * sizeof(float), s);
            if (rc) return rc;
            ba.cc = sc.cc;
            launch_bn_bwd_pass(true, wt, dg, false, dim3(std::max(1, std::min(b->T, d.gxb)), cdiv(d.fp, 1024)), ba, s);
            EAGCN_LAUNCH_CHECK();
        }
        if (zero_after && zero_after->nd) { rc = zero_fill(zero_after->d, (size_t)zero_after->nd * sizeof(double), s); if (rc) return rc; }
    } else {
        ProfScope ps(PROF_BN, s);
        const int ny = cdiv(d.fp, 1024);
        {
            const bool wt = p->structure == EAGCN_STRUCT_WEIGHTED, dr = ba.do_drop != 0;
            bool dg = ba.rg.dg != nullptr;
            const dim3 grid(gxb, ny);
            ba.cc = sc.cc;
            ba.store_dh = bn_bwd_two_pass(wt) ? 0 : 1;
            static const bool rows_first = [] { const char* v = getenv("EAGCN_W_ROWS_FIRST"); return !(v && v[0] == '0'); }();
            if (wt && dg && b->T > 0 && bn_bwd_two_pass(wt) && lagg_bwd && lagg_fuses_bn() && lagg_wfuse() && rows_first) {
                rc = launch_readout_bwd_rows(b, ba.rg, d.ldo, sc.dY, s);
                if (rc) return rc;
                w_rows = true;
                ba.dxout = sc.dY;
                dg = false;
            }
            launch_bn_bwd_pass(false, wt, dg, dr, grid, ba, s);
        }
        EAGCN_LAUNCH_CHECK();
        const double* gsum = nullptr;
        if (w->stats_hook && p->training) {
            if (gxb > 64) bn_stats_sum_kernel<64><<<cdiv(d.fp, 4), 256, 0, s>>>(sc.slab, gxb, d.fp, M, sc.gsum, b->meta, 2, 0, ba.nvirt, b->B);
            else bn_stats_sum_kernel<16><<<cdiv(d.fp, 16), 256, 0, s>>>(sc.slab, gxb, d.fp, M, sc.gsum, b->meta, 2, 0, ba.nvirt, b->B);
            EAGCN_LAUNCH_CHECK();
            if (w->stats_hook(sc.gsum, 2 * d.fp + 1, stream, w->stats_user)) {
                set_error("eagcn_layer_backward: the sync-BatchNorm all-reduce hook failed");
                return EAGCN_ERR_HIP;
            }
            gsum = sc.gsum;
        }
        if (gxb > 64)
            bn_bwd_finalize_kernel<64><<<cdiv(d.fp, 4), 256, 0, s>>>(sc.slab, sc.slab_da, gxb, d.fp, M, p->training, w->bn,
                                                                       d.vc, gp, sc.cc, b->meta, ba.nvirt, b->B, ny, gxb, gsum, ba.zero, ba.nzero);
        else
            bn_bwd_finalize_kernel<16><<<cdiv(d.fp, 16), 256, 0, s>>>(sc.slab, sc.slab_da, gxb, d.fp, M, p->training, w->bn,
                                                                        d.vc, gp, sc.cc, b->meta, ba.nvirt, b->B, ny, gxb, gsum, ba.zero, ba.nzero);
        EAGCN_LAUNCH_CHECK();
        if (b->T > 0) {
            const bool wt = p->structure == EAGCN_STRUCT_WEIGHTED, dg = ba.rg.dg != nullptr, dr = ba.do_drop != 0;
            if (bn_bwd_two_pass(wt) && wt && lagg_bwd && lagg_fuses_bn() && lagg_wfuse()) {
                fused_w_apply = true;
                if (dg && !w_rows) {
                    rc = launch_readout_bwd_rows(b, ba.rg, d.ldo, sc.dY, s);
                    if (rc) return rc;
                }
            } else if (bn_bwd_two_pass(wt)) launch_bn_bwd_pass(true, wt, dg, dr, dim3(std::max(1, std::min(b->T, d.gxb)), ny), ba, s);
            else if (lagg_bwd && lagg_fuses_bn()) fused_bn_apply = true;
            else bn_bwd_apply_kernel<<<ew_grid((size_t)b->T * d.fp / 4), 256, 0, s>>>(*b, d.fp, w->Y, d.fp, w->bn, sc.cc, sc.dY);
            EAGCN_LAUNCH_CHECK();
        }
    }
    int nsplit = 0, nedge = 0, xk_G = 0;
    bool bx_slabs = false;
    int bx_per = 0;
    int bx_wide = 0;
    hipStream_t side = w->aux_stream ? (hipStream_t)w->aux_stream : s;
    const bool forked = side != s;
    if (b->T > 0) {
        AggArgs a;
        a.bt = *b; a.vc = d.vc; a.src = sc.dY; a.lds = d.fp; a.dst = sc.dP; a.ldd = d.fp;
        a.sig = sc.sig; a.rsig = sc.rsig; a.rscale = w->rscale; a.stats = nullptr; a.nchunk = 1;
        const size_t xstride = bx_plane_elems(b->T, d.ld_in), pstride = bx_plane_elems(b->T, d.fp);
        BxProb bx, bw;
        memset(&bx, 0, sizeof(bx));
        memset(&bw, 0, sizeof(bw));
        bool use_bx = false;
        if (d.np && !w->aux_stream) {
            bx.A = BxPlanes{sc.dPp, pstride, d.fp, b->T}; bx.B = BxPlanes{sc.Wp, d.wpslab, d.fp, d.ld_in}; bx.C = dx; bx.ldc = d.ld_in;
            bx.M = b->T; bx.N = d.ld_in; bx.K = d.fp; bx.M_dev = b->meta + EAGCN_META_T; bx.tn = 0; bx.splits = 1;
            bw.A = BxPlanes{w->x_planes ? w->x_planes : sc.xp, xstride, d.ld_in, b->T}; bw.B = BxPlanes{sc.dPp, pstride, d.fp, b->T};
            bw.C = sc.dWcat; bw.ldc = d.fp; bw.M = d.ld_in; bw.N = d.fp; bw.K = b->T; bw.K_dev = b->meta + EAGCN_META_T; bw.tn = 1;
            bw.splits = d.bx_splits; bw.slab = d.wslab;
            use_bx = bx3_ok(bw) && (!dx || bx3_ok(bx));
        }
        if (use_bx) {
            a.planes = BxOut{sc.dPp, pstride, d.np, b->T};
            if (!w->x_planes && !input_only) {
                rc = launch_bx3_split(w->x, b->T, b->meta + EAGCN_META_T, d.ld_in, sc.xp, xstride, b->T, d.np, s);
                if (rc) return rc;
            }
        } else if (!w->x && !input_only) {
            set_error("eagcn_layer_backward: the input exists as plane images only and the plane products do not apply");
            return EAGCN_ERR_ARG;
        }
        EdgeArgs e;
        e.bt = *b; e.vc = d.vc; e.dY = sc.dY; e.Y = w->Y; e.P = w->P; e.ld = d.fp; e.sig = sc.sig;
        e.rsig = sc.rsig; e.rscale = w->rscale; e.datt = sc.datt; e.atomic = 0;
        static const bool edge_atomic = [] { const char* v = getenv("EAGCN_EDGE_SLABS"); return !(v && v[0] == '1'); }();
        bool general_rel = false;
        for (int k = 0; k < p->K; ++k) general_rel = general_rel || pp.rel_vec[k] != nullptr;
        if (edge_atomic && !general_rel) { e.datt = sc.eacc; e.atomic = 1; }
        static const bool colaunch = [] { const char* v = getenv("EAGCN_NO_COLAUNCH"); return !(v && v[0] == '1'); }();
        nedge = e.atomic ? -EDGE_COPIES : edge_grid_x(b);
        if (input_only) {
            if (lagg_bwd) {
                if (fused_bn_apply || fused_w_apply || fused_c_apply) { a.bn_tab = w->bn; a.bn_cc = eval_in ? nullptr : sc.cc; a.bn_fp = d.fp; }
                if (fused_w_apply || fused_c_apply) {
                    a.src = (ba.rg.dg || w_rows) ? sc.dY : dxout; a.lds = d.ldo;
                    a.w_aw = sc.colp + (size_t)CP_AVEW * d.fp;
                    a.w_rowm = fused_c_apply;
                    a.w_drop = ba.do_drop; a.w_thr = ba.thr; a.w_inv_keep = ba.inv_keep; a.w_seed = ba.seed; a.w_seed_dev = ba.seed_dev;
                }
                rc = launch_lagg_bwd(a, e, s, false);
            } else {
                rc = launch_agg(a, true, s);
            }
            if (rc) return rc;
            if (use_bx) {
                rc = launch_bx3(bx, nullptr, d.np, s, gemm_work, PROF_GEMM, bx3_pick_wide(bx, nullptr, b->t_hint));
            } else {
                GemmDesc gx{0, 1, b->T, d.ld_in, d.fp, sc.dP, d.fp, sc.Wcat, d.fp, dx, d.ld_in, 1, 0, gemm_work};
                gx.M_dev = b->meta + EAGCN_META_T;
                rc = launch_gemm(gx, s);
            }
            return rc;
        }
        if (lagg_bwd && e.atomic) {
            if (fused_bn_apply || fused_w_apply) { a.bn_tab = w->bn; a.bn_cc = sc.cc; a.bn_fp = d.fp; }
            if (fused_w_apply) {
                a.src = (ba.rg.dg || w_rows) ? sc.dY : dxout; a.lds = d.ldo;
                a.w_aw = sc.colp + (size_t)CP_AVEW * d.fp;
                a.w_drop = ba.do_drop; a.w_thr = ba.thr; a.w_inv_keep = ba.inv_keep; a.w_seed = ba.seed; a.w_seed_dev = ba.seed_dev;
            }
            rc = launch_lagg_bwd(a, e, s);
            if (rc) return rc;
        } else if (!forked && colaunch) {
            rc = launch_agg_edge(a, e, s);
            if (rc) return rc;
        } else {
            if (forked) { rc = stream_after(side, s); if (rc) return rc; }
            rc = launch_edge_grad(e, side);
            if (rc) return rc;
            rc = launch_agg(a, true, s);
            if (rc) return rc;
        }
        if (forked) { rc = stream_after(side, s); if (rc) return rc; }
        nsplit = d.nsplit;
        GemmDesc gw{1, 0, d.ld_in, d.fp, b->T, w->x, d.ld_in, sc.dP, d.fp, sc.dWcat, d.fp, nsplit, d.wslab, gemm_work};
        gw.K_dev = b->meta + EAGCN_META_T;
        GemmDesc gx{0, 1, b->T, d.ld_in, d.fp, sc.dP, d.fp, sc.Wcat, d.fp, dx, d.ld_in, 1, 0, gemm_work};
        gx.M_dev = b->meta + EAGCN_META_T;
        static const bool pair = [] { const char* v = getenv("EAGCN_NO_PAIR"); return !(v && v[0] == '1'); }();
        static const bool use3 = [] { const char* v = getenv("EAGCN_NO_GEMM3"); return !(v && v[0] == '1'); }();
        DwScatter dsc;
        for (int k = 0; k < EAGCN_MAX_VIEWS; ++k) dsc.dW[k] = gp.dW[k];
        dsc.vc = d.vc;
        dsc.in = in;
        if (use_bx) {
            bx_wide = dx ? bx3_pick_wide(bx, &bw, b->t_hint) : bx3_pick_wide(bw, nullptr, b->t_hint);
            rc = dx ? launch_bx3(bx, &bw, d.np, s, 2.0 * gemm_work, PROF_GEMM_PAIR, bx_wide) : launch_bx3(bw, nullptr, d.np, s, gemm_work, PROF_GEMM, bx_wide);
            if (rc) return rc;
            nsplit = d.bx_splits;
            bx_slabs = true;
            bx_per = (dx && bx3_pair_policy()) ? std::max(1, bx3_grid() >> 3) : 0;
        } else if (use3 && !forked && dx && gemm3_layer(d.ld_in) && gemm3_ok(gw) && gemm3_ok(gx) && gemm3_xk_enabled()) {
            rc = launch_gemm3_pair(gx, gw, nullptr, sc.gws, gemm3_workspace_bytes(), s, d.wslab);
            if (rc) return rc;
            nsplit = 1;
            xk_G = gemm3_grid();
        } else if (use3 && !forked && dx && gemm3_layer(d.ld_in) && gemm3_ok(gw) && gemm3_ok(gx)) {
            rc = launch_gemm3_pair(gx, gw, &dsc, sc.gws, gemm3_workspace_bytes(), s);
            if (rc) return rc;
            nsplit = 0;
        } else if (dx && !forked && colaunch && pair) {
            rc = launch_gemm_pair(gx, gw, s);
            if (rc) return rc;
        } else {
            rc = launch_gemm(gw, side);
            if (rc) return rc;
            if (dx) { rc = launch_gemm(gx, s); if (rc) return rc; }
        }
    }
    if (b->T == 0 && input_only) return EAGCN_OK;
    if (b->T == 0) {
        for (int k = 0; k < p->K; ++k)
            { int rcz = zero_fill(gp.dW[k], (size_t)d.fin * p->width[k] * sizeof(float), side); if (rcz) return rcz; }
    }
    {
        const int wblocks = nsplit > 0 ? cdiv((int)d.wslab, 256) : 0;
        double* edge_src = nedge == -EDGE_COPIES ? sc.eacc : sc.datt;
        const int edge_drain = edge_src == sc.eacc ? 1 : 0;
        static const bool defer_env = [] { const char* v = getenv("EAGCN_NO_EDGE_DEFER"); return !(v && v[0] == '1'); }();
        if (defer_env && drain_out && edge_drain && wblocks == 0 && !forked && b->T > 0) {
            drain_out->eacc = sc.eacc; drain_out->K = p->K; drain_out->rsig = sc.rsig;
            for (int k = 0; k < EAGCN_MAX_VIEWS; ++k) {
                drain_out->datt_w[k] = gp.datt_w[k]; drain_out->dself_r[k] = gp.dself_r[k]; drain_out->channels[k] = pp.channels[k];
            }
            return EAGCN_OK;
        }
        ProfScope psu(PROF_PACK, side);
        unpack_grads_kernel<<<wblocks + cdiv(p->K * EDGE_SLAB, 16), 256, 0, side>>>(gp, pp, d.vc, in, d.ld_in, d.fp, sc.dWcat,
                                                                                    bx_slabs ? -nsplit : nsplit, d.wslab, edge_src, nedge, sc.rsig,
                                                                                    wblocks, b->meta, xk_G, edge_drain, bx_per, bx_wide);
        EAGCN_LAUNCH_CHECK();
    }
    if (forked) { rc = stream_after(s, side); if (rc) return rc; }
    return EAGCN_OK;
}

extern "C" int eagcn_attention_dense(const eagcn_batch* b, const eagcn_layer_params* p, float* out, void* stream) {
    hipStream_t s = (hipStream_t)stream;
    EAGCN_CHECK_ARG(b && p && out, "eagcn_attention_dense: null argument");
    EAGCN_CHECK_ARG(p->K == b->K, "eagcn_attention_dense: view count mismatch");
    EAGCN_CHECK_ARG(b->code, "eagcn_attention_dense: batch has no code map");
    ParamPtrs pp;
    memset(&pp, 0, sizeof(pp));
    for (int k = 0; k < p->K; ++k) {
        EAGCN_CHECK_ARG(p->att_w[k], "eagcn_attention_dense: view %d has no attention weight", k);
        pp.att_w[k] = p->att_w[k];
        pp.channels[k] = b->channels[k];
        pp.rel_vec[k] = b->rel_vec[k]; pp.rel_c[k] = b->rel_c[k];
    }
    const size_t total = (size_t)b->K * b->B * b->N * b->N;
    attention_dense_kernel<<<ew_grid(total), 256, 0, s>>>(*b, pp, out);
    EAGCN_LAUNCH_CHECK();
    return EAGCN_OK;
}
```

eagcn_amd/ops.py:

```python
import ctypes as C
import os

import torch

from . import _lib as L


def _stream():
    return C.c_void_p(torch.cuda.current_stream().cuda_stream)


def _ptr(t):
    return C.c_void_p(t.data_ptr()) if t is not None else C.c_void_p(0)


def _need_cuda_f32(t, name):
    if not isinstance(t, torch.Tensor) or not t.is_cuda:
        raise L.EagcnHipError('%s must be a tensor on the MI355X (got %s): eagcn_amd has no CPU path'
                              % (name, getattr(t, 'device', type(t))))
    if t.dtype != torch.float32:
        raise L.EagcnHipError('%s must be float32 (got %s)' % (name, t.dtype))
    return t.contiguous()


# ... 238 lines not shown
    return _UnpackRows.apply(index, layout, packed, pad_row)


def _seed_fields(seed):
    if isinstance(seed, torch.Tensor):
        if not seed.is_cuda or seed.dtype != torch.int64 or seed.numel() != 1:
            raise L.EagcnHipError('a device seed must be a 1-element int64 device tensor')
        return 0, seed.data_ptr()
    return int(seed) & (2 ** 63 - 1), None


class LayerSpec:

    def __init__(self, structure, widths, in_layout, dropout, bn_eps=1e-5, bn_momentum=0.1):
        self.structure = {'Concate': L.STRUCT_CONCATE, 'Weighted_sum': L.STRUCT_WEIGHTED}[structure]
        self.structure_name = structure
        self.widths = [int(w) for w in widths]
        self.K = len(self.widths)
        self.in_layout = in_layout
        self.dropout = float(dropout)
        self.bn_eps, self.bn_momentum = float(bn_eps), float(bn_momentum)
        self.fp = sum(L.pad16(w) for w in self.widths)
        if self.structure == L.STRUCT_CONCATE:
            self.out_layout = ColLayout(self.widths, [L.pad16(w) for w in self.widths])
        else:
            self.out_layout = ColLayout([self.widths[0]], [L.pad16(self.widths[0])])

    def cparams(self, training, seed, views, ave_w):
        p = L.LayerParams()
        p.K, p.structure, p.training = self.K, self.structure, int(bool(training))
        for k, w in enumerate(self.widths):
            p.width[k] = w
        p.inp = self.in_layout.c
        p.dropout, p.bn_eps, p.bn_momentum = self.dropout, self.bn_eps, self.bn_momentum
        p.seed, p.seed_dev = _seed_fields(seed)
        for k, v in enumerate(views):
            p.att_w[k], p.self_r[k], p.W[k] = v['att_w'].data_ptr(), v['self_r'].data_ptr(), v['W'].data_ptr()
            p.bias[k], p.gamma[k], p.beta[k] = v['bias'].data_ptr(), v['gamma'].data_ptr(), v['beta'].data_ptr()
            p.run_mean[k], p.run_var[k] = v['run_mean'].data_ptr(), v['run_var'].data_ptr()
        p.ave_w = ave_w.data_ptr() if ave_w is not None else None
        return p


_PARAM_KEYS = ('att_w', 'self_r', 'W', 'bias', 'gamma', 'beta')


class _LayerFn(torch.autograd.Function):

    @staticmethod
    def forward(ctx, index, spec, training, seed, buffers, x, ave_w, *flat):
        lib = L.load()
        K = spec.K
        x = x.contiguous()
        if x.shape != (index.T, spec.in_layout.ld):
            raise L.EagcnHipError('packed input is %s, expected %s' % (tuple(x.shape), (index.T, spec.in_layout.ld)))
        views = []
        for k in range(K):
            v = {name: flat[k * 6 + i] for i, name in enumerate(_PARAM_KEYS)}
            for name, t in v.items():
                if not t.is_cuda or t.dtype != torch.float32 or not t.is_contiguous():
                    raise L.EagcnHipError('parameter %s of view %d must be a contiguous fp32 device tensor' % (name, k))
            v['run_mean'], v['run_var'] = buffers[k]
            fin = spec.in_layout.width
            if tuple(v['W'].shape) != (fin, spec.widths[k]):
                raise L.EagcnHipError('view %d weight is %s, expected %s' % (k, tuple(v['W'].shape), (fin, spec.widths[k])))
            if v['att_w'].numel() != index.channels[k]:
                raise L.EagcnHipError('view %d attention weight has %d channels, relation tensor has %d'
                                      % (k, v['att_w'].numel(), index.channels[k]))
            views.append(v)
        p = spec.cparams(training, seed, views, ave_w)
        dev, T, fp = x.device, index.T, spec.fp
        f32 = dict(dtype=torch.float32, device=dev)
        P = torch.empty((T, fp), **f32)
        Y = torch.empty((T, fp), **f32)
        rscale = torch.empty((K, T), **f32)
        bn = torch.empty((4, fp), **f32)
        xout = torch.empty((T, spec.out_layout.ld), **f32)
        pad_row = torch.empty(spec.out_layout.ld, **f32)
        nbytes = lib.eagcn_layer_fwd_scratch_bytes(index.ref(), C.byref(p))
        scratch = torch.empty(nbytes, dtype=torch.uint8, device=dev)
        w = L.LayerBufs()
        w.x, w.P, w.Y, w.rscale, w.bn = x.data_ptr(), P.data_ptr(), Y.data_ptr(), rscale.data_ptr(), bn.data_ptr()
        w.xout, w.pad_row, w.scratch, w.scratch_bytes = xout.data_ptr(), pad_row.data_ptr(), scratch.data_ptr(), nbytes
        L.check(lib.eagcn_layer_forward(index.ref(), C.byref(p), C.byref(w), _stream()), 'eagcn_layer_forward')
        ctx.index, ctx.spec, ctx.training, ctx.seed, ctx.buffers = index, spec, training, seed, buffers
        ctx.save_for_backward(x, P, Y, rscale, bn, ave_w, *flat)
        if spec.structure == L.STRUCT_CONCATE:
            ctx.mark_non_differentiable(pad_row)
        return xout, pad_row

    @staticmethod
    def backward(ctx, dxout, dpad):
        lib = L.load()
        index, spec = ctx.index, ctx.spec
        x, P, Y, rscale, bn, ave_w, *flat = ctx.saved_tensors
        K = spec.K
        views = []
        for k in range(K):
            v = {name: flat[k * 6 + i] for i, name in enumerate(_PARAM_KEYS)}
            v['run_mean'], v['run_var'] = ctx.buffers[k]
            views.append(v)
        p = spec.cparams(ctx.training, ctx.seed, views, ave_w)
        dev = x.device
        dxout = dxout.contiguous()
        grads = [torch.empty_like(t) for t in flat]
        dave = torch.empty_like(ave_w) if ave_w is not None else None
        g = L.LayerGrads()
        for k in range(K):
            gk = grads[k * 6:(k + 1) * 6]
            g.datt_w[k], g.dself_r[k], g.dW[k] = gk[0].data_ptr(), gk[1].data_ptr(), gk[2].data_ptr()
            g.dbias[k], g.dgamma[k], g.dbeta[k] = gk[3].data_ptr(), gk[4].data_ptr(), gk[5].data_ptr()
        g.dave_w = dave.data_ptr() if dave is not None else None
        need_dx = ctx.needs_input_grad[5]
        dx = torch.empty_like(x) if need_dx else None
        nbytes = lib.eagcn_layer_bwd_scratch_bytes(index.ref(), C.byref(p))
        scratch = torch.empty(nbytes, dtype=torch.uint8, device=dev)
        w = L.LayerBufs()
        w.x, w.P, w.Y, w.rscale, w.bn = x.data_ptr(), P.data_ptr(), Y.data_ptr(), rscale.data_ptr(), bn.data_ptr()
        w.scratch, w.scratch_bytes = scratch.data_ptr(), nbytes
        dpad_ptr = C.c_void_p(0)
        if spec.structure == L.STRUCT_WEIGHTED and dpad is not None:
            dpad = dpad.contiguous()
            dpad_ptr = _ptr(dpad)
        L.check(lib.eagcn_layer_backward(index.ref(), C.byref(p), C.byref(w), _ptr(dxout), dpad_ptr, _ptr(dx),
                                         C.byref(g), _stream()), 'eagcn_layer_backward')
        return (None, None, None, None, None, dx, dave, *grads)


def layer_forward(index, spec, training, seed, buffers, x, ave_w, flat_params):
    return _LayerFn.apply(index, spec, training, seed, buffers, x, ave_w, *flat_params)


class _GatFn(torch.autograd.Function):

    @staticmethod
    def forward(ctx, index, fin, ld_in, F, training, seed, dropout, att_dropout, alpha, x, W, a):
        lib = L.load()
        if not getattr(index, 'bond_lists', False):
            raise L.EagcnHipError('the GAT layer needs a batch index with bond lists: BatchIndex(..., bond_lists=True)')
        x, W, a = x.contiguous(), W.contiguous(), a.contiguous()
        if x.shape != (index.T, ld_in) or tuple(W.shape) != (fin, F) or a.numel() != 2 * F:
            raise L.EagcnHipError('GAT layer: x %s W %s a %s for fin=%d ld=%d F=%d' % (tuple(x.shape), tuple(W.shape), tuple(a.shape), fin, ld_in, F))
        p = L.GatParams()
        p.fin, p.ld_in, p.F, p.training = fin, ld_in, F, int(bool(training))
        p.alpha, p.att_dropout, p.dropout = float(alpha), float(att_dropout), float(dropout)
        p.seed, p.seed_dev = _seed_fields(seed)
        p.W, p.a = W.data_ptr(), a.data_ptr()
        Fp = (F + 15) // 16 * 16
        f32 = dict(dtype=torch.float32, device=x.device)
        h = torch.empty((index.T, Fp), **f32)
        s12 = torch.empty((2, index.T), **f32)
        xout = torch.empty((index.T, Fp), **f32)
        L.check(lib.eagcn_gat_forward(index.ref(), C.byref(p), x.data_ptr(), h.data_ptr(), s12.data_ptr(), xout.data_ptr(),
                                      _stream()), 'eagcn_gat_forward')
        ctx.index, ctx.p_args = index, (fin, ld_in, F, training, seed, dropout, att_dropout, alpha)
        ctx.save_for_backward(x, W, a, h, s12, xout)
        return xout

    @staticmethod
    def backward(ctx, dxout):
        lib = L.load()
        x, W, a, h, s12, xout = ctx.saved_tensors
        fin, ld_in, F, training, seed, dropout, att_dropout, alpha = ctx.p_args
        index = ctx.index
        p = L.GatParams()
        p.fin, p.ld_in, p.F, p.training = fin, ld_in, F, int(bool(training))
        p.alpha, p.att_dropout, p.dropout = float(alpha), float(att_dropout), float(dropout)
        p.seed, p.seed_dev = _seed_fields(seed)
        p.W, p.a = W.data_ptr(), a.data_ptr()
        dxout = dxout.contiguous()
        dW, da = torch.empty_like(W), torch.empty_like(a)
        dx = torch.empty_like(x) if ctx.needs_input_grad[9] else None
        nbytes = lib.eagcn_gat_scratch_bytes(index.ref(), F)
        scratch = torch.empty(nbytes, dtype=torch.uint8, device=x.device)
        L.check(lib.eagcn_gat_backward(index.ref(), C.byref(p), x.data_ptr(), h.data_ptr(), s12.data_ptr(), xout.data_ptr(),
                                       dxout.data_ptr(), _ptr(dx) if dx is not None else C.c_void_p(0), dW.data_ptr(),
                                       da.data_ptr(), scratch.data_ptr(), nbytes, _stream()), 'eagcn_gat_backward')
        return (None,) * 9 + (dx, dW, da)


def gat_layer(index, fin, ld_in, F, training, seed, dropout, att_dropout, alpha, x, W, a):
    return _GatFn.apply(index, fin, ld_in, F, training, seed, dropout, att_dropout, alpha, x, W, a)


def attention_dense(index, att_weights):
    lib = L.load()
    p = L.LayerParams()
    p.K = index.K
    for k, a in enumerate(att_weights):
        p.att_w[k] = a.data_ptr()
    out = torch.empty((index.K, index.B, index.N, index.N), dtype=torch.float32, device=index.device)
    L.check(lib.eagcn_attention_dense(index.ref(), C.byref(p), _ptr(out), _stream()), 'eagcn_attention_dense')
    return out


class _Readout(torch.autograd.Function):
    @staticmethod
    def forward(ctx, index, layout, mode, size, x, pad_row):
        F = layout.width
        g = torch.empty((index.B, F), dtype=torch.float32, device=x.device)
        if mode == 1:
            size = size.to(device=x.device, dtype=torch.int64).contiguous()
        L.check(L.load().eagcn_readout_forward(index.ref(), _ptr(x), C.byref(layout.c), _ptr(pad_row),
                                               _ptr(size) if mode == 1 else C.c_void_p(0), mode, _ptr(g), F,
                                               _stream()), 'eagcn_readout_forward')
        ctx.index, ctx.layout, ctx.mode, ctx.size = index, layout, mode, size
        ctx.has_pad = pad_row is not None
        return g
# ... 534 lines not shown
```

include/eagcn_hip.h:

```cpp
#ifndef EAGCN_HIP_H
#define EAGCN_HIP_H

#include <stddef.h>
#include <stdint.h>

#ifdef __cplusplus
extern "C" {
#endif

#define EAGCN_MAX_VIEWS 8
#define EAGCN_MAX_SEGS 8
#define EAGCN_MAX_CHANNELS 255
#define EAGCN_STRUCT_CONCATE 0
#define EAGCN_STRUCT_WEIGHTED 1

#define EAGCN_OK 0
#define EAGCN_ERR_ARG (-1)
#define EAGCN_ERR_HIP (-2)
#define EAGCN_ERR_SCRATCH (-3)

#define EAGCN_META_T 0
#define EAGCN_META_NMAX 1
#define EAGCN_META_NTILES 2
#define EAGCN_META_BAD_ADJ 3
// ... 217 lines not shown

int eagcn_stream_signal_flag(uint32_t* flag, void* stream);
int eagcn_stream_wait_flag(uint32_t* flag, double budget_seconds, void* stream);
int eagcn_stream_wait_timeouts(void);
void eagcn_stream_wait_reset(void);

int eagcn_stream_wait_counter(const uint32_t* counter, uint32_t value, void* stream);

size_t eagcn_model_saved_bytes(const eagcn_batch* b, const eagcn_model* m);
size_t eagcn_model_scratch_bytes(const eagcn_batch* b, const eagcn_model* m);
int eagcn_model_atom_rep(const eagcn_batch* b, const eagcn_model* m, size_t* xout_offset,
                         size_t* pad_row_offset, int* ld);
int eagcn_model_atom_rep_materialize(const eagcn_batch* b, const eagcn_model* m, void* saved, size_t saved_bytes, void* stream);
int eagcn_model_pack_input(const eagcn_batch* b, const eagcn_model* m, const float* afm, void* saved,
                           size_t saved_bytes, void* stream);
int eagcn_model_forward(const eagcn_batch* b, const eagcn_model* m, const float* afm, const int64_t* size,
                        void* saved, size_t saved_bytes, void* scratch, size_t scratch_bytes, float* out,
                        float* graph_rep, void* stream);
int eagcn_model_backward(const eagcn_batch* b, const eagcn_model* m, const int64_t* size, void* saved,
                         size_t saved_bytes, void* scratch, size_t scratch_bytes, const float* dout,
                         const float* dgraph_rep, const eagcn_layer_grads* lg, const eagcn_head_grads* hg,
                         void* stream);

int eagcn_model_backward_range(const eagcn_batch* b, const eagcn_model* m, const int64_t* size, void* saved,
                               size_t saved_bytes, void* scratch, size_t scratch_bytes, const float* dout,
                               const float* dgraph_rep, const eagcn_layer_grads* lg, const eagcn_head_grads* hg,
                               int with_head, int layer_hi, int layer_lo, void* stream);

size_t eagcn_model_input_scratch_bytes(const eagcn_batch* b, const eagcn_model* m);
int eagcn_model_backward_input(const eagcn_batch* b, const eagcn_model* m, const int64_t* size, void* saved,
                               size_t saved_bytes, void* scratch, size_t scratch_bytes, const float* dout,
                               const float* dgraph_rep, const eagcn_layer_grads* lg, const eagcn_head_grads* hg,
                               float* dafm, void* stream);

float eagcn_attr_alpha(int step, int steps);
float eagcn_attr_weight(int steps);
size_t eagcn_attr_acc_elems(const eagcn_batch* b, const eagcn_model* m);
int eagcn_attr_pack_input(const eagcn_batch* b, const eagcn_model* m, const float* afm, const float* baseline, float alpha,
                          void* saved, size_t saved_bytes, void* stream);
int eagcn_attr_step(const eagcn_batch* b, const eagcn_model* m, const int64_t* size, void* saved, size_t saved_bytes,
                    void* scratch, size_t scratch_bytes, const float* dout, const float* dgraph_rep, float weight, int first,
                    float* acc, void* stream);
int eagcn_attr_finalize(const eagcn_batch* b, const eagcn_model* m, const float* afm, const float* baseline, const float* acc,
                        float* attr, float* score, void* stream);

typedef struct eagcn_step_loss {
    int32_t kind;
    const float* labels;
    const float* class_weight;
    float* loss;
    const float* scale;
    float* dout;
} eagcn_step_loss;
int eagcn_model_forward_step(const eagcn_batch* b, const eagcn_model* m, const float* afm, const int64_t* size,
                             void* saved, size_t saved_bytes, void* scratch, size_t scratch_bytes, float* out,
                             float* graph_rep, const eagcn_step_loss* loss, const float* dgraph_rep,
                             const eagcn_head_grads* hg, void* stream);

size_t eagcn_head_saved_bytes(const eagcn_head_params* h, int B);
size_t eagcn_head_scratch_bytes(const eagcn_head_params* h, int B);
int eagcn_head_forward(const eagcn_head_params* h, int B, int training, uint64_t seed, const uint64_t* seed_dev, const float* g,
                       void* saved, size_t saved_bytes, void* scratch, size_t scratch_bytes, float* out, float* graph_rep,
                       void* stream);
int eagcn_head_backward(const eagcn_head_params* h, int B, int training, uint64_t seed, const uint64_t* seed_dev, const float* g,
                        void* saved, size_t saved_bytes, void* scratch, size_t scratch_bytes, const float* dout,
                        const float* dgraph_rep, const eagcn_head_grads* hg, float* dg, void* stream);

int eagcn_bce_loss(const float* logits, const float* labels, const float* class_weight, int B, int T,
                   float* loss, float* dlogits, void* stream);
int eagcn_mse_loss(const float* pred, const float* target, int n, float* loss, float* dpred, void* stream);

int eagcn_adam_step(float* param, const float* grad, float* exp_avg, float* exp_avg_sq, int64_t n, const double* hyper_dev,
                    int64_t* step_dev, uint32_t* ticket_dev, void* stream);

int eagcn_eval_append(const float* logits, const float* labels, int B, int T, int classification, float* scores,
                      float* targets, uint8_t* valid, int64_t row_offset, void* stream);

int eagcn_set_gemm_mode(int mode);

size_t eagcn_bx3_plane_elems(int rows_cap, int ld);
int eagcn_bx3_split(const float* x, int rows, int ld, uint16_t* planes, size_t plane_stride, int rows_cap, int np, void* stream);
int eagcn_bx3_used_splits(int splits, int M, int N, int K);
int eagcn_set_bx3_wide(int mode);
int eagcn_bx3_pair_used_splits(int splits, int M, int N, int K, int M0, int N0, int K0);
int eagcn_gemm_bx3(int tn, int M, int N, int K, const uint16_t* A, size_t a_pstride, int lda, int a_rows, const uint16_t* B,
                   size_t b_pstride, int ldb, int b_rows, float* C, int ldc, int splits, size_t slab, int np, void* stream);
int eagcn_gemm_bx3_pair(int M0, int N0, int K0, const uint16_t* A0, size_t a0_pstride, int lda0, int a0_rows, const uint16_t* B0,
                        size_t b0_pstride, int ldb0, int b0_rows, float* C0, int ldc0, int M1, int N1, int K1, const uint16_t* A1,
                        size_t a1_pstride, int lda1, int a1_rows, const uint16_t* B1, size_t b1_pstride, int ldb1, int b1_rows,
                        float* C1, int ldc1, int splits, size_t slab, int np, void* stream);

int eagcn_gemm_f32(int ta, int tb, int M, int N, int K, const float* A, int lda, const float* B,
                   int ldb, float* C, int ldc, void* stream);
int eagcn_gemm_f32_dev(int ta, int tb, int M, int N, int K, const float* A, int lda, const float* B,
                       int ldb, float* C, int ldc, const int32_t* extent_dev, int which, void* stream);

size_t eagcn_gemm_sk_workspace_bytes(void);
int eagcn_gemm_f32_sk(int ta, int tb, int M, int N, int K, const float* A, int lda, const float* B, int ldb, float* C,
                      int ldc, void* workspace, size_t workspace_bytes, void* stream);
int eagcn_gemm_pair_sk(int M0, int N0, int K0, const float* A0, int lda0, const float* B0, int ldb0, float* C0, int ldc0,
                       int M1, int N1, int K1, const float* A1, int lda1, const float* B1, int ldb1, float* C1, int ldc1,
                       void* workspace, size_t workspace_bytes, void* stream);
int eagcn_gemm_pair_sk_slabs(int M0, int N0, int K0, const float* A0, int lda0, const float* B0, int ldb0, float* C0, int ldc0,
                             int M1, int N1, int K1, const float* A1, int lda1, const float* B1, int ldb1, float* C1, int ldc1,
                             size_t slab, void* workspace, size_t workspace_bytes, void* stream);
int eagcn_gemm_sk_plan(int M0, int N0, int K0, int M1, int N1, int K1, int wgs, int* a, int* c);
int eagcn_gemm_sk_timeouts(void);
int eagcn_gemm_sk_failed(void);
void eagcn_gemm_sk_reset_failed(void);
void eagcn_gemm_sk_inject_failure(void);

void eagcn_prof_enable(int on);
void eagcn_prof_reset(void);
int eagcn_prof_ntags(void);
const char* eagcn_prof_tag_name(int tag);
int eagcn_prof_read(int tag, double* total_ms, double* work, int64_t* launches);

#ifdef __cplusplus
}
#endif
#endif
```

Baseline: 711,300.

## Aggregate raw inputs before the first-layer projection (aggregate-then-transform)

For the first layer, when the input width is small (up to FIRST_VW), the input features are replicated per view and aggregated over neighbours first. Only then is the per-view weight applied, using a dedicated fp32 kernel that also emits the BatchNorm statistics. The backward pass mirrors this: the BN backward is folded into a kernel that computes dZ and weight-gradient slabs, and the aggregation backward then runs on the narrow input width. The aim is to cut aggregation traffic and GEMM launches for the narrow first layer. In exchange it adds a replication pass, extra scratch use, and a recomputation GEMM on paths that need P.

```diff
diff --git a/eagcn_amd/_lib.py b/eagcn_amd/_lib.py
--- a/eagcn_amd/_lib.py
+++ b/eagcn_amd/_lib.py
@@ -139,6 +139,7 @@
     'eagcn_agg_wants_bond_lists_for': (C.c_int, [C.c_int, C.c_int, C.c_int]),
     'eagcn_bx3_used_splits': (C.c_int, [C.c_int, C.c_int, C.c_int, C.c_int]),
     'eagcn_set_bx3_wide': (C.c_int, [C.c_int]),
+    'eagcn_set_first_layer_mode': (C.c_int, [C.c_int]),
     'eagcn_bx3_pair_used_splits': (C.c_int, [C.c_int] * 7),
     'eagcn_bx3_plane_elems': (C.c_size_t, [C.c_int, C.c_int]),
     'eagcn_bx3_split': (C.c_int, [_fp, C.c_int, C.c_int, _fp, C.c_size_t, C.c_int, C.c_int, _fp]),
diff --git a/eagcn_amd/build.py b/eagcn_amd/build.py
--- a/eagcn_amd/build.py
+++ b/eagcn_amd/build.py
@@ -8,7 +8,7 @@
 CSRC = os.path.join(HERE, 'csrc')
 LIBDIR = os.path.join(HERE, 'lib')
 LIB = os.path.join(LIBDIR, 'libeagcn_hip.so')
-HIP_SOURCES = ['index.hip', 'gemm.hip', 'gemm3.hip', 'gemm_bx3.hip', 'gemm_bx3w.hip', 'agg.hip', 'lagg.hip', 'lagg_in.hip', 'gat.hip', 'pool.hip', 'layer.hip', 'readout.hip', 'head.hip', 'head2.hip', 'loss.hip', 'attr.hip']
+HIP_SOURCES = ['index.hip', 'gemm.hip', 'gemm3.hip', 'gemm_bx3.hip', 'gemm_bx3w.hip', 'agg.hip', 'lagg.hip', 'lagg_in.hip', 'first.hip', 'gat.hip', 'pool.hip', 'layer.hip', 'readout.hip', 'head.hip', 'head2.hip', 'loss.hip', 'attr.hip']
 CPP_SOURCES = ['api.cpp']
 HEADERS = ['common.h', 'kernels.h', 'lagg_kernel.h', 'gemm_x6.h', 'bx3.h', os.path.join('..', '..', 'include', 'eagcn_hip.h')]
 ARCH = 'gfx950'
diff --git a/eagcn_amd/csrc/attr.hip b/eagcn_amd/csrc/attr.hip
--- a/eagcn_amd/csrc/attr.hip
+++ b/eagcn_amd/csrc/attr.hip
@@ -113,6 +113,10 @@
     attr_pack_kernel<<<attr_grid((size_t)b->T * layout_ld(in)), 256, 0, s>>>(*b, afm, baseline, alpha, make_colmap(in), layout_ld(in),
                                                                            layout_width(in), attr_nin(b), x0);
     EAGCN_LAUNCH_CHECK();
+    float* xrep = nullptr;
+    rc = model_first_rep_slot(b, m, saved, saved_bytes, &xrep, "eagcn_attr_pack_input");
+    if (rc) return rc;
+    if (xrep) return launch_first_rep(x0, layout_ld(in), xrep, m->layer[0].K, b->meta, b->T, s);
     return EAGCN_OK;
 }
 
diff --git a/eagcn_amd/csrc/first.hip b/eagcn_amd/csrc/first.hip
--- /dev/null
+++ b/eagcn_amd/csrc/first.hip
@@ -0,0 +1,263 @@
+#include <stdlib.h>
+
+#include <algorithm>
+
+#include "common.h"
+#include "kernels.h"
+
+namespace eagcn {
+
+static int g_first_mode = [] { const char* e = getenv("EAGCN_FIRST_AGG"); return e ? (atoi(e) ? 1 : 0) : 1; }();
+int first_layer_mode() { return g_first_mode; }
+
+int first_slabs(int Tcap) { return std::max(1, std::min(64, cdiv(std::max(Tcap, 1), 32))); }
+
+__device__ __forceinline__ float f4_at(const float4& v, int i) { return i == 0 ? v.x : i == 1 ? v.y : i == 2 ? v.z : v.w; }
+
+__global__ __launch_bounds__(256) void first_rep_kernel(const float* __restrict__ x, int ld_in, float* __restrict__ xrep, int K,
+                                                         const int32_t* __restrict__ meta, int Tcap) {
+    const int T = min(meta[EAGCN_META_T], Tcap);
+    const uint32_t per = (uint32_t)K * (FIRST_VW / 4), total = (uint32_t)T * per;
+    for (uint32_t e = blockIdx.x * blockDim.x + threadIdx.x; e < total; e += gridDim.x * blockDim.x) {
+        const uint32_t r = e / per, c = e - r * per, q = c & (FIRST_VW / 4 - 1);
+        float4 v = make_float4(0.f, 0.f, 0.f, 0.f);
+        if ((int)(4 * q) < ld_in) v = *reinterpret_cast<const float4*>(x + (size_t)r * ld_in + 4 * q);
+        *reinterpret_cast<float4*>(xrep + (size_t)e * 4) = v;
+    }
+}
+
+struct FirstFwd {
+    const float* Z; const float* Wcat; float* Y; double* stats; const int32_t* meta;
+    ViewCols vc; int Tcap, ld_in, fp, rpw;
+};
+__global__ __launch_bounds__(256) void first_fwd_kernel(FirstFwd a) {
+    __shared__ __attribute__((aligned(16))) float Ws[FIRST_VW][FIRST_MAXW];
+    __shared__ __attribute__((aligned(16))) float Zs[64][FIRST_VW + 4];
+    __shared__ double red[16][FIRST_MAXW][2];
+    const int k = blockIdx.y, s = blockIdx.x, tid = threadIdx.x;
+    const int off = a.vc.off[k], wkp = a.vc.off[k + 1] - off;
+    const int T = min(a.meta[EAGCN_META_T], a.Tcap);
+    const int r_lo = min(s * a.rpw, T), r_hi = min(r_lo + a.rpw, T);
+    const int nfq = wkp >> 2, nrg = min(16, 256 / nfq);
+    const int fq = tid % nfq, rg = tid / nfq;
+    const bool act = rg < nrg;
+    const int ldz = a.vc.K * FIRST_VW;
+    for (int e = tid; e < FIRST_VW * wkp; e += 256) {
+        const int i = e / wkp, f = e - i * wkp;
+        Ws[i][f] = i < a.ld_in ? a.Wcat[(size_t)i * a.fp + off + f] : 0.0f;
+    }
+    double s1[4] = {0.0, 0.0, 0.0, 0.0}, s2[4] = {0.0, 0.0, 0.0, 0.0};
+    const int tr = nrg * 4;
+    for (int r0 = r_lo; r0 < r_hi; r0 += tr) {
+        __syncthreads();
+        for (int e = tid; e < tr * (FIRST_VW / 4); e += 256) {
+            const int rr = e >> 3, q = e & 7, r = r0 + rr;
+            float4 v = make_float4(0.f, 0.f, 0.f, 0.f);
+            if (r < r_hi) v = *reinterpret_cast<const float4*>(a.Z + (size_t)r * ldz + k * FIRST_VW + 4 * q);
+            *reinterpret_cast<float4*>(&Zs[rr][4 * q]) = v;
+        }
+        __syncthreads();
+        if (act) {
+            float4 acc[4];
+#pragma unroll
+            for (int rr = 0; rr < 4; ++rr) acc[rr] = make_float4(0.f, 0.f, 0.f, 0.f);
+#pragma unroll
+            for (int i4 = 0; i4 < FIRST_VW / 4; ++i4) {
+                if (4 * i4 >= a.ld_in) break;
+                float4 z[4];
+#pragma unroll
+                for (int rr = 0; rr < 4; ++rr) z[rr] = *reinterpret_cast<const float4*>(&Zs[rg * 4 + rr][4 * i4]);
+#pragma unroll
+                for (int ii = 0; ii < 4; ++ii) {
+                    const float4 w4 = *reinterpret_cast<const float4*>(&Ws[4 * i4 + ii][4 * fq]);
+#pragma unroll
+                    for (int rr = 0; rr < 4; ++rr) {
+                        const float zv = f4_at(z[rr], ii);
+                        acc[rr].x = fmaf(zv, w4.x, acc[rr].x); acc[rr].y = fmaf(zv, w4.y, acc[rr].y);
+                        acc[rr].z = fmaf(zv, w4.z, acc[rr].z); acc[rr].w = fmaf(zv, w4.w, acc[rr].w);
+                    }
+                }
+            }
+#pragma unroll
+            for (int rr = 0; rr < 4; ++rr) {
+                const int r = r0 + rg * 4 + rr;
+                if (r < r_hi) {
+                    *reinterpret_cast<float4*>(a.Y + (size_t)r * a.fp + off + 4 * fq) = acc[rr];
+                    s1[0] += (double)acc[rr].x; s2[0] += (double)acc[rr].x * (double)acc[rr].x;
+                    s1[1] += (double)acc[rr].y; s2[1] += (double)acc[rr].y * (double)acc[rr].y;
+                    s1[2] += (double)acc[rr].z; s2[2] += (double)acc[rr].z * (double)acc[rr].z;
+                    s1[3] += (double)acc[rr].w; s2[3] += (double)acc[rr].w * (double)acc[rr].w;
+                }
+            }
+        }
+    }
+    if (act) {
+#pragma unroll
+        for (int e = 0; e < 4; ++e) { red[rg][4 * fq + e][0] = s1[e]; red[rg][4 * fq + e][1] = s2[e]; }
+    }
+    __syncthreads();
+    if (tid < wkp) {
+        double t1 = 0.0, t2 = 0.0;
+        for (int g = 0; g < nrg; ++g) { t1 += red[g][tid][0]; t2 += red[g][tid][1]; }
+        *reinterpret_cast<double2*>(a.stats + ((size_t)s * a.fp + off + tid) * 2) = make_double2(t1, t2);
+    }
+}
+
+struct FirstBwd {
+    const float* dH; const float* Y; const float* bn; const float* cc;
+    const float* Z; const float* WcatT; float* dZ; float* dWs; const int32_t* meta;
+    ViewCols vc; int Tcap, ld_in, fp, rpw; size_t wslab;
+};
+constexpr int FB_RT = 64;
+constexpr int FB_LD = FIRST_MAXW + 1;
+__global__ __launch_bounds__(256) void first_bwd_kernel(FirstBwd a) {
+    __shared__ __attribute__((aligned(16))) float Wt[FIRST_MAXW][FIRST_VW];
+    __shared__ float dYs[FB_RT][FB_LD];
+    __shared__ __attribute__((aligned(16))) float Zs[FB_RT][FIRST_VW + 4];
+    __shared__ float cst[5][FIRST_MAXW];
+    const int k = blockIdx.y, s = blockIdx.x, tid = threadIdx.x;
+    const int off = a.vc.off[k], wkp = a.vc.off[k + 1] - off;
+    const int T = min(a.meta[EAGCN_META_T], a.Tcap);
+    const int r_lo = min(s * a.rpw, T), r_hi = min(r_lo + a.rpw, T);
+    const int ldz = a.vc.K * FIRST_VW, nfq = wkp >> 2;
+    for (int e = tid; e < wkp * FIRST_VW; e += 256) {
+        const int f = e >> 5, i = e & (FIRST_VW - 1);
+        Wt[f][i] = i < a.ld_in ? a.WcatT[(size_t)(off + f) * a.ld_in + i] : 0.0f;
+    }
+    if (a.bn && tid < wkp) {
+        const int cp = off + tid;
+        cst[0][tid] = a.bn[(size_t)BN_SC * a.fp + cp]; cst[1][tid] = a.bn[(size_t)BN_MU * a.fp + cp];
+        cst[2][tid] = a.bn[(size_t)BN_INV * a.fp + cp]; cst[3][tid] = a.cc[cp]; cst[4][tid] = a.cc[a.fp + cp];
+    }
+    const int nig = (a.ld_in + 7) >> 3, nitem = wkp * nig;
+    float dw[2][8];
+#pragma unroll
+    for (int j = 0; j < 2; ++j)
+#pragma unroll
+        for (int i = 0; i < 8; ++i) dw[j][i] = 0.0f;
+    for (int r0 = r_lo; r0 < r_hi; r0 += FB_RT) {
+        const int nr = min(FB_RT, r_hi - r0);
+        __syncthreads();
+        for (int e = tid; e < FB_RT * nfq; e += 256) {
+            const int rr = e / nfq, q = e - rr * nfq;
+            float4 d = make_float4(0.f, 0.f, 0.f, 0.f);
+            if (rr < nr) {
+                d = *reinterpret_cast<const float4*>(a.dH + (size_t)(r0 + rr) * a.fp + off + 4 * q);
+                if (a.bn) {
+                    const float4 y = *reinterpret_cast<const float4*>(a.Y + (size_t)(r0 + rr) * a.fp + off + 4 * q);
+                    const int c = 4 * q;
+                    d.x = cst[0][c] * (d.x - cst[3][c] - (y.x - cst[1][c]) * cst[2][c] * cst[4][c]);
+                    d.y = cst[0][c + 1] * (d.y - cst[3][c + 1] - (y.y - cst[1][c + 1]) * cst[2][c + 1] * cst[4][c + 1]);
+                    d.z = cst[0][c + 2] * (d.z - cst[3][c + 2] - (y.z - cst[1][c + 2]) * cst[2][c + 2] * cst[4][c + 2]);
+                    d.w = cst[0][c + 3] * (d.w - cst[3][c + 3] - (y.w - cst[1][c + 3]) * cst[2][c + 3] * cst[4][c + 3]);
+                }
+            }
+            dYs[rr][4 * q] = d.x; dYs[rr][4 * q + 1] = d.y; dYs[rr][4 * q + 2] = d.z; dYs[rr][4 * q + 3] = d.w;
+        }
+        for (int e = tid; e < FB_RT * (FIRST_VW / 4); e += 256) {
+            const int rr = e >> 3, q = e & 7;
+            float4 v = make_float4(0.f, 0.f, 0.f, 0.f);
+            if (rr < nr) v = *reinterpret_cast<const float4*>(a.Z + (size_t)(r0 + rr) * ldz + k * FIRST_VW + 4 * q);
+            *reinterpret_cast<float4*>(&Zs[rr][4 * q]) = v;
+        }
+        __syncthreads();
+        {
+            const int rr = tid & 63, ig = tid >> 6;
+            float4 z0 = make_float4(0.f, 0.f, 0.f, 0.f), z1 = z0;
+            for (int f = 0; f < wkp; ++f) {
+                const float d = dYs[rr][f];
+                const float4 w0 = *reinterpret_cast<const float4*>(&Wt[f][8 * ig]);
+                const float4 w1 = *reinterpret_cast<const float4*>(&Wt[f][8 * ig + 4]);
+                z0.x = fmaf(d, w0.x, z0.x); z0.y = fmaf(d, w0.y, z0.y); z0.z = fmaf(d, w0.z, z0.z); z0.w = fmaf(d, w0.w, z0.w);
+                z1.x = fmaf(d, w1.x, z1.x); z1.y = fmaf(d, w1.y, z1.y); z1.z = fmaf(d, w1.z, z1.z); z1.w = fmaf(d, w1.w, z1.w);
+            }
+            if (rr < nr) {
+                float* dst = a.dZ + (size_t)(r0 + rr) * ldz + k * FIRST_VW + 8 * ig;
+                *reinterpret_cast<float4*>(dst) = z0;
+                *reinterpret_cast<float4*>(dst + 4) = z1;
+            }
+        }
+#pragma unroll
+        for (int j = 0; j < 2; ++j) {
+            const int it = tid + 256 * j;
+            if (it < nitem) {
+                const int ig = it / wkp, f = it - ig * wkp;
+                for (int rr = 0; rr < nr; ++rr) {
+                    const float d = dYs[rr][f];
+                    const float4 z0 = *reinterpret_cast<const float4*>(&Zs[rr][8 * ig]);
+                    const float4 z1 = *reinterpret_cast<const float4*>(&Zs[rr][8 * ig + 4]);
+                    dw[j][0] = fmaf(z0.x, d, dw[j][0]); dw[j][1] = fmaf(z0.y, d, dw[j][1]);
+                    dw[j][2] = fmaf(z0.z, d, dw[j][2]); dw[j][3] = fmaf(z0.w, d, dw[j][3]);
+                    dw[j][4] = fmaf(z1.x, d, dw[j][4]); dw[j][5] = fmaf(z1.y, d, dw[j][5]);
+                    dw[j][6] = fmaf(z1.z, d, dw[j][6]); dw[j][7] = fmaf(z1.w, d, dw[j][7]);
+                }
+            }
+        }
+    }
+    float* slab = a.dWs + (size_t)s * a.wslab;
+#pragma unroll
+    for (int j = 0; j < 2; ++j) {
+        const int it = tid + 256 * j;
+        if (it < nitem) {
+            const int ig = it / wkp, f = it - ig * wkp;
+#pragma unroll
+            for (int i = 0; i < 8; ++i)
+                if (8 * ig + i < a.ld_in) slab[(size_t)(8 * ig + i) * a.fp + off + f] = dw[j][i];
+        }
+    }
+}
+
+bool first_shape_ok(const ViewCols& vc, int ld_in, int fp) {
+    if (ld_in > FIRST_VW || (ld_in & 3) || 2 * vc.K * FIRST_VW > fp) return false;
+    for (int k = 0; k < vc.K; ++k)
+        if (vc.off[k + 1] - vc.off[k] > FIRST_MAXW) return false;
+    return true;
+}
+ViewCols first_view_cols(int K, int ld_in) {
+    ViewCols v;
+    v.K = K;
+    for (int k = 0; k <= EAGCN_MAX_VIEWS; ++k) v.off[k] = std::min(k, K) * FIRST_VW;
+    for (int k = 0; k < EAGCN_MAX_VIEWS; ++k) v.width[k] = k < K ? ld_in : 0;
+    return v;
+}
+
+int launch_first_rep(const float* x, int ld_in, float* xrep, int K, const int32_t* meta, int Tcap, hipStream_t s) {
+    const size_t n = (size_t)std::max(Tcap, 1) * K * (FIRST_VW / 4);
+    ProfScope ps(PROF_PACK, s);
+    first_rep_kernel<<<(unsigned)std::max<size_t>(1, std::min<size_t>((n + 255) / 256, 2048)), 256, 0, s>>>(x, ld_in, xrep, K, meta, Tcap);
+    EAGCN_LAUNCH_CHECK();
+    return EAGCN_OK;
+}
+
+int launch_first_fwd(const float* Z, const float* Wcat, float* Y, double* stats, const eagcn_batch* b, const ViewCols& vc, int ld_in,
+                     int fp, double work, hipStream_t s) {
+    FirstFwd a;
+    a.Z = Z; a.Wcat = Wcat; a.Y = Y; a.stats = stats; a.meta = b->meta; a.vc = vc; a.Tcap = b->T; a.ld_in = ld_in; a.fp = fp;
+    const int ns = first_slabs(b->T);
+    a.rpw = cdiv(std::max(b->T, 1), ns);
+    ProfScope ps(PROF_GEMM, s, work);
+    first_fwd_kernel<<<dim3(ns, vc.K), 256, 0, s>>>(a);
+    EAGCN_LAUNCH_CHECK();
+    return EAGCN_OK;
+}
+
+int launch_first_bwd(const float* dH, const float* Y, const float* bn, const float* cc, const float* Z, const float* WcatT, float* dZ,
+                     float* dWs, size_t wslab, const eagcn_batch* b, const ViewCols& vc, int ld_in, int fp, double work, hipStream_t s) {
+    FirstBwd a;
+    a.dH = dH; a.Y = Y; a.bn = bn; a.cc = cc; a.Z = Z; a.WcatT = WcatT; a.dZ = dZ; a.dWs = dWs; a.meta = b->meta; a.vc = vc;
+    a.Tcap = b->T; a.ld_in = ld_in; a.fp = fp; a.wslab = wslab;
+    const int ns = first_slabs(b->T);
+    a.rpw = cdiv(std::max(b->T, 1), ns);
+    ProfScope ps(PROF_GEMM, s, work);
+    first_bwd_kernel<<<dim3(ns, vc.K), 256, 0, s>>>(a);
+    EAGCN_LAUNCH_CHECK();
+    return EAGCN_OK;
+}
+
+}
+
+extern "C" int eagcn_set_first_layer_mode(int mode) {
+    const int old = eagcn::g_first_mode;
+    eagcn::g_first_mode = mode ? 1 : 0;
+    return old;
+}
diff --git a/eagcn_amd/csrc/head.hip b/eagcn_amd/csrc/head.hip
--- a/eagcn_amd/csrc/head.hip
+++ b/eagcn_amd/csrc/head.hip
@@ -262,7 +262,8 @@
     EAGCN_CHECK_ARG(b && m && afm && saved, "eagcn_model_pack_input: null argument");
     ModelSaved sv;
     EAGCN_CHECK_ARG(carve_saved(saved, b, m, &sv) <= saved_bytes, "eagcn_model_pack_input: saved block too small");
-    return eagcn_pack_rows(b, afm, layout_width(&m->layer[0].in), &m->layer[0].in, sv.x0, stream);
+    return pack_rows_rep(b, afm, layout_width(&m->layer[0].in), &m->layer[0].in, sv.x0,
+                         layer_first_rep_wanted(b, &m->layer[0]) ? sv.L[0].P : nullptr, m->layer[0].K, stream);
 }
 
 struct HeadPlan {
@@ -349,7 +350,9 @@
     ZeroJob zj;
     RC(gemm3_zero_job(sc.layer, sc.layer_bytes, sc.hst, (HEAD_COPIES + 1) * sc.n_hst + HEAD_WS, &zj));
     if (!m->input_packed)
-        RC(eagcn_pack_rows(b, afm, layout_width(&m->layer[0].in), &m->layer[0].in, sv.x0, stream));
+        RC(pack_rows_rep(b, afm, layout_width(&m->layer[0].in), &m->layer[0].in, sv.x0,
+                         layer_first_rep_wanted(b, &m->layer[0]) ? sv.L[0].P : nullptr, m->layer[0].K, stream));
+    const bool xrep0 = layer_first_rep_wanted(b, &m->layer[0]);
     const float* x = sv.x0;
     {
         const eagcn_layer_params* ps[4];
@@ -367,7 +370,7 @@
         w.stats_hook = m->stats_hook; w.stats_user = m->stats_user;
         w.x_planes = l > 0 ? sv.L[l - 1].xout_planes : nullptr; w.xout_planes = L.xout_planes;
         const bool po = hidden_planes_only(b, m, sv, l);
-        RC(layer_forward_impl(b, &m->layer[l], &w, stream, true, l == m->n_layers - 1 && fused_readout(m), po));
+        RC(layer_forward_impl(b, &m->layer[l], &w, stream, true, l == m->n_layers - 1 && fused_readout(m), po, l == 0 && xrep0));
         x = po ? nullptr : L.xout;
     }
     const eagcn_layer_params* last = &m->layer[m->n_layers - 1];
@@ -732,6 +735,12 @@
                                m->n_layers - 1, 0, is.dx0, input_only, stream);
 }
 
+int eagcn::model_first_rep_slot(const eagcn_batch* b, const eagcn_model* m, void* saved, size_t saved_bytes, float** xrep, const char* who) {
+    ModelSaved sv;
+    EAGCN_CHECK_ARG(carve_saved(saved, b, m, &sv) <= saved_bytes, "%s: saved block too small", who);
+    *xrep = layer_first_rep_wanted(b, &m->layer[0]) ? sv.L[0].P : nullptr;
+    return EAGCN_OK;
+}
 int eagcn::model_input_slot(const eagcn_batch* b, const eagcn_model* m, void* saved, size_t saved_bytes, float** x0, const char* who) {
     ModelSaved sv;
     EAGCN_CHECK_ARG(carve_saved(saved, b, m, &sv) <= saved_bytes, "%s: saved block too small", who);
diff --git a/eagcn_amd/csrc/index.hip b/eagcn_amd/csrc/index.hip
--- a/eagcn_amd/csrc/index.hip
+++ b/eagcn_amd/csrc/index.hip
@@ -653,8 +653,17 @@
 }
 
 __global__ __launch_bounds__(256) void pack_rows_kernel(eagcn_batch bt, const float* __restrict__ dense,
-                                                         int F, ColMap m, int ld, float* __restrict__ packed, int Nin) {
+                                                         int F, ColMap m, int ld, float* __restrict__ packed, int Nin,
+                                                         float* __restrict__ xrep, int repK) {
     const uint32_t total = (uint32_t)dev_rows(bt) * (uint32_t)ld;
+    if (xrep) {
+        const uint32_t kv = (uint32_t)repK * FIRST_VW, tot2 = (uint32_t)dev_rows(bt) * kv;
+        for (uint32_t e = blockIdx.x * blockDim.x + threadIdx.x; e < tot2; e += gridDim.x * blockDim.x) {
+            const int r = (int)(e / kv), cp = (int)(e - (uint32_t)r * kv) & (FIRST_VW - 1);
+            const int ce = cp < ld ? packed_to_exact(m, cp) : -1;
+            xrep[e] = ce >= 0 ? dense[((size_t)bt.row_mol[r] * Nin + bt.row_loc[r]) * F + ce] : 0.0f;
+        }
+    }
     for (uint32_t e = blockIdx.x * blockDim.x + threadIdx.x; e < total; e += gridDim.x * blockDim.x) {
         int r = (int)(e / (uint32_t)ld), cp = (int)(e - (uint32_t)r * (uint32_t)ld);
         int ce = packed_to_exact(m, cp);
@@ -834,15 +843,20 @@
 
 extern "C" int eagcn_pack_rows(const eagcn_batch* b, const float* dense, int F, const eagcn_layout* lay,
                                float* packed, void* stream) {
+    return eagcn::pack_rows_rep(b, dense, F, lay, packed, nullptr, 0, stream);
+}
+int eagcn::pack_rows_rep(const eagcn_batch* b, const float* dense, int F, const eagcn_layout* lay, float* packed, float* xrep, int K,
+                         void* stream) {
     hipStream_t s = (hipStream_t)stream;
     EAGCN_CHECK_ARG(b && dense && lay && packed, "eagcn_pack_rows: null argument");
     EAGCN_CHECK_ARG(layout_width(lay) == F, "eagcn_pack_rows: layout width %d != F %d", layout_width(lay), F);
     if (b->T == 0) return EAGCN_OK;
     int ld = layout_ld(lay);
-    size_t total = (size_t)b->T * ld;
+    EAGCN_CHECK_ARG(!xrep || ld <= FIRST_VW, "eagcn_pack_rows: %d packed columns do not fit a view's block", ld);
+    size_t total = (size_t)b->T * (xrep ? K * FIRST_VW : ld);
     int grid = (int)std::min<size_t>((total + 255) / 256, 4096);
     ProfScope ps(PROF_PACK, s);
-    pack_rows_kernel<<<grid, 256, 0, s>>>(*b, dense, F, make_colmap(lay), ld, packed, b->n_logical > 0 ? b->n_logical : b->N);
+    pack_rows_kernel<<<grid, 256, 0, s>>>(*b, dense, F, make_colmap(lay), ld, packed, b->n_logical > 0 ? b->n_logical : b->N, xrep, K);
     EAGCN_LAUNCH_CHECK();
     return EAGCN_OK;
 }
diff --git a/eagcn_amd/csrc/kernels.h b/eagcn_amd/csrc/kernels.h
--- a/eagcn_amd/csrc/kernels.h
+++ b/eagcn_amd/csrc/kernels.h
@@ -37,6 +37,20 @@
 int launch_lagg_fwd(AggArgs a, hipStream_t s);
 int launch_lagg_bwd(AggArgs a, const EdgeArgs& e, hipStream_t s, bool edge = true);
 int launch_lagg_bwd_input(const AggArgs& a, const EdgeArgs& e, dim3 grid, hipStream_t s);
+
+constexpr int FIRST_VW = 32;
+constexpr int FIRST_MAXW = 128;
+int first_layer_mode();
+bool first_shape_ok(const ViewCols& vc, int ld_in, int fp);
+ViewCols first_view_cols(int K, int ld_in);
+int first_slabs(int Tcap);
+int launch_first_rep(const float* x, int ld_in, float* xrep, int K, const int32_t* meta, int Tcap, hipStream_t s);
+int pack_rows_rep(const eagcn_batch* b, const float* dense, int F, const eagcn_layout* lay, float* packed, float* xrep, int K, void* stream);
+bool layer_first_rep_wanted(const eagcn_batch* b, const eagcn_layer_params* p);
+int launch_first_fwd(const float* Z, const float* Wcat, float* Y, double* stats, const eagcn_batch* b, const ViewCols& vc, int ld_in,
+                     int fp, double work, hipStream_t s);
+int launch_first_bwd(const float* dH, const float* Y, const float* bn, const float* cc, const float* Z, const float* WcatT, float* dZ,
+                     float* dWs, size_t wslab, const eagcn_batch* b, const ViewCols& vc, int ld_in, int fp, double work, hipStream_t s);
 
 struct EdgeArgs {
     eagcn_batch bt;
@@ -214,8 +228,9 @@
 int launch_attr_dense(const eagcn_batch* b, const eagcn_layout* in, const float* acc, const float* x, const float* base, float* attr,
                       float* score, hipStream_t s);
 int model_input_slot(const eagcn_batch* b, const eagcn_model* m, void* saved, size_t saved_bytes, float** x0, const char* who);
+int model_first_rep_slot(const eagcn_batch* b, const eagcn_model* m, void* saved, size_t saved_bytes, float** xrep, const char* who);
 int layer_forward_impl(const eagcn_batch* b, const eagcn_layer_params* p, const eagcn_layer_bufs* w, void* stream,
-                       bool prepacked, bool skip_apply = false, bool planes_only = false);
+                       bool prepacked, bool skip_apply = false, bool planes_only = false, bool xrep_ready = false);
 bool layer_reads_planes_only(const eagcn_batch* b, const eagcn_layer_params* p, bool aux_stream);
 int layer_apply_impl(const eagcn_batch* b, const eagcn_layer_params* p, const eagcn_layer_bufs* w, void* stream);
 int pack_params_all(const eagcn_batch* b, const eagcn_layer_params* const* ps, void* const* packed,
diff --git a/eagcn_amd/csrc/layer.hip b/eagcn_amd/csrc/layer.hip
--- a/eagcn_amd/csrc/layer.hip
+++ b/eagcn_amd/csrc/layer.hip
@@ -575,11 +575,12 @@
                                                             int ld_in, int fp, const float* __restrict__ dWcat,
                                                             int nsplit, size_t slab, double* __restrict__ datt,
                                                             int nedge, const float* __restrict__ rsig, int wblocks,
-                                                            const int32_t* __restrict__ meta, int xk_G, int edge_drain, int bx_per, int bx_wide) {
+                                                            const int32_t* __restrict__ meta, int xk_G, int edge_drain, int bx_per, int bx_wide, int all_slabs) {
     nedge = nedge < 0 ? -nedge : min(nedge, (meta[EAGCN_META_T] + 15) / 16);
     const int bxm = bx_wide ? BX3W_BM : BX3_BM, bxn = bx_wide ? BX3W_BN : BX3_BN;
     nsplit = nsplit < 0 ? bx3_used_splits_wave(-nsplit, meta[EAGCN_META_T], ((ld_in + bxm - 1) / bxm) * ((fp + bxn - 1) / bxn),
                                           bx_per > 0 ? ((meta[EAGCN_META_T] + bxm - 1) / bxm) * ((ld_in + bxn - 1) / bxn) : 0, max(1, (fp + 31) >> 5), bx_per)
+                        : all_slabs ? nsplit
                         : max(1, min(nsplit, meta[EAGCN_META_T] >> 7));
     if ((int)blockIdx.x < wblocks) {
         const int tid = blockIdx.x * blockDim.x + threadIdx.x;
@@ -705,6 +706,8 @@
     size_t wpslab, wtpslab;
     int np;
     int bx_splits;
+    bool first_shape;
+    int fslabs;
 };
 static LayerDims layer_dims(const eagcn_batch* b, const eagcn_layer_params* p) {
     LayerDims d;
@@ -715,6 +718,9 @@
     d.ldo = p->structure == EAGCN_STRUCT_CONCATE ? d.fp : pad16(p->width[0]);
     d.gx = agg_grid_x(b);
     d.gslab = std::max(d.gx, lagg_use(b, 0, false, &d.vc) ? lagg_slabs(b) : 0);
+    d.first_shape = p->structure == EAGCN_STRUCT_CONCATE && b->T > 0 && d.ld_in < 128 && first_shape_ok(d.vc, d.ld_in, d.fp);
+    d.fslabs = d.first_shape ? first_slabs(b->T) : 0;
+    d.gslab = std::max(d.gslab, d.fslabs);
     {
         const long by_rows = cdiv(b->T + 1, BWD_ROWS);
         const long by_bytes = std::max<long>(64, (32L << 20) / ((long)d.fp * 16));
@@ -758,6 +764,7 @@
     uint16_t *Wp, *WTp;
     double *slab, *slab_da, *datt, *gsum;
     uint16_t *dPp, *xp;
+    float* P_re;
 };
 static size_t carve_fwd(void* base, const eagcn_batch* b, const LayerDims& d, FwdScratch* s) {
     Carver c(base);
@@ -792,15 +799,33 @@
     t.dY = c.take<float>((size_t)std::max(b->T, 1) * d.fp);
     t.dP = c.take<float>((size_t)std::max(b->T, 1) * d.fp);
     t.cc = c.take<float>((size_t)2 * d.fp);
-    t.dWcat = c.take<float>(d.wslab * std::max(std::max(d.nsplit, G3_XSEG), d.np ? d.bx_splits : 1));
+    t.dWcat = c.take<float>(d.wslab * std::max(std::max(std::max(d.nsplit, G3_XSEG), d.np ? d.bx_splits : 1), d.fslabs));
     t.slab = c.take<double>((size_t)d.gxb * d.fp * 2);
     t.slab_da = c.take<double>((size_t)d.gxb * cdiv(d.fp, 1024) * EAGCN_MAX_VIEWS);
     t.datt = c.take<double>((size_t)edge_grid_x(b) * EAGCN_MAX_VIEWS * EDGE_SLAB);
     t.gsum = c.take<double>((size_t)2 * d.fp + 8);
     t.dPp = c.take<uint16_t>(d.np ? (size_t)d.np * bx_plane_elems(b->T, d.fp) : 1);
     t.xp = c.take<uint16_t>(d.np ? (size_t)d.np * bx_plane_elems(b->T, d.ld_in) : 1);
+    t.P_re = c.take<float>(d.first_shape ? (size_t)b->T * d.fp : 1);
     if (s) *s = t;
     return c.off;
+}
+
+static bool first_path(const eagcn_batch* b, const eagcn_layer_bufs* w, const LayerDims& d, bool any_mode = false) {
+    static const bool edge_atomic = [] { const char* v = getenv("EAGCN_EDGE_SLABS"); return !(v && v[0] == '1'); }();
+    if ((!any_mode && !first_layer_mode()) || !d.first_shape || !w->x || w->x_planes || d.np || !edge_atomic) return false;
+    for (int k = 0; k < b->K; ++k)
+        if (b->rel_vec[k]) return false;
+    return lagg_use(b, 0, false, &d.vc) && lagg_use(b, 1, true);
+}
+
+bool eagcn::layer_first_rep_wanted(const eagcn_batch* b, const eagcn_layer_params* p) {
+    if (!b || !p || b->T <= 0 || p->K != b->K) return false;
+    const LayerDims d = layer_dims(b, p);
+    eagcn_layer_bufs w;
+    memset(&w, 0, sizeof(w));
+    w.x = reinterpret_cast<const float*>(static_cast<uintptr_t>(4096));
+    return first_path(b, &w, d, true);
 }
 
 static int check_layer(const eagcn_batch* b, const eagcn_layer_params* p, const char* who) {
@@ -914,7 +939,7 @@
 }
 
 int eagcn::layer_forward_impl(const eagcn_batch* b, const eagcn_layer_params* p, const eagcn_layer_bufs* w,
-                              void* stream, bool prepacked, bool skip_apply, bool planes_only) {
+                              void* stream, bool prepacked, bool skip_apply, bool planes_only, bool xrep_ready) {
     hipStream_t s = (hipStream_t)stream;
     int rc = check_layer(b, p, "eagcn_layer_forward");
     if (rc) return rc;
@@ -952,7 +977,24 @@
     for (int k = 0; k < p->K; ++k) fsum += p->width[k];
     const double gemm_work = 2.0 * (double)b->T * (double)d.fin * fsum;
     int nslab = 0, tiles_per_wg = agg_ksplit(b) ? 1 : 4;
-    if (b->T > 0) {
+    if (b->T > 0 && first_path(b, w, d)) {
+        const int kv = p->K * FIRST_VW;
+        float* xrep = w->P;
+        float* Z = w->P + (size_t)b->T * kv;
+        if (!xrep_ready) {
+            rc = launch_first_rep(w->x, d.ld_in, xrep, p->K, b->meta, b->T, s);
+            if (rc) return rc;
+        }
+        AggArgs a;
+        a.bt = *b; a.vc = first_view_cols(p->K, d.ld_in); a.src = xrep; a.lds = kv; a.dst = Z; a.ldd = kv;
+        a.sig = sc.sig; a.rsig = sc.rsig; a.rscale = w->rscale; a.stats = sc.stats; a.nchunk = 1;
+        rc = launch_lagg_fwd(a, s);
+        if (rc) return rc;
+        rc = launch_first_fwd(Z, sc.Wcat, w->Y, sc.stats, b, d.vc, d.ld_in, d.fp, gemm_work, s);
+        if (rc) return rc;
+        nslab = d.fslabs;
+        tiles_per_wg = 0;
+    } else if (b->T > 0) {
         GemmDesc g3{0, 1, b->T, d.fp, d.ld_in, w->x, d.ld_in, sc.WcatT, d.ld_in, w->P, d.fp, 1, 0, gemm_work};
         g3.M_dev = b->meta + EAGCN_META_T;
         BxProb bp;
@@ -1192,6 +1234,17 @@
     }
     const double M = (double)b->B * (double)b->N;
     const bool eval_in = input_only && !p->training;
+    const bool first_taken = b->T > 0 && first_path(b, w, d);
+    const bool first_bwd = first_taken && !dx && !input_only;
+    bool first_forms = false;
+    const float* P_used = w->P;
+    if (first_taken && !first_bwd && !input_only) {
+        GemmDesc gp0{0, 0, b->T, d.fp, d.ld_in, w->x, d.ld_in, sc.Wcat, d.fp, sc.P_re, d.fp, 1, 0, gemm_work};
+        gp0.M_dev = b->meta + EAGCN_META_T;
+        rc = launch_gemm(gp0, s);
+        if (rc) return rc;
+        P_used = sc.P_re;
+    }
     if (eval_in) {
         const bool wt = p->structure == EAGCN_STRUCT_WEIGHTED, dg = ba.rg.dg != nullptr;
         if (b->T > 0 && lagg_bwd) {
@@ -1256,10 +1309,36 @@
                     if (rc) return rc;
                 }
             } else if (bn_bwd_two_pass(wt)) launch_bn_bwd_pass(true, wt, dg, dr, dim3(std::max(1, std::min(b->T, d.gxb)), ny), ba, s);
+            else if (first_bwd) first_forms = true;
             else if (lagg_bwd && lagg_fuses_bn()) fused_bn_apply = true;
             else bn_bwd_apply_kernel<<<ew_grid((size_t)b->T * d.fp / 4), 256, 0, s>>>(*b, d.fp, w->Y, d.fp, w->bn, sc.cc, sc.dY);
             EAGCN_LAUNCH_CHECK();
         }
+    }
+    if (first_bwd) {
+        const int kv = p->K * FIRST_VW;
+        const ViewCols vcz = first_view_cols(p->K, d.ld_in);
+        const float* xrep = w->P;
+        const float* Z = w->P + (size_t)b->T * kv;
+        float* dZ = sc.dP;
+        float* dPz = sc.dP + (size_t)b->T * kv;
+        rc = launch_first_bwd(sc.dY, w->Y, first_forms ? w->bn : nullptr, sc.cc, Z, sc.WcatT, dZ, sc.dWcat, d.wslab, b, d.vc, d.ld_in, d.fp,
+                              gemm_work, s);
+        if (rc) return rc;
+        AggArgs a;
+        a.bt = *b; a.vc = vcz; a.src = dZ; a.lds = kv; a.dst = dPz; a.ldd = kv;
+        a.sig = sc.sig; a.rsig = sc.rsig; a.rscale = w->rscale; a.stats = nullptr; a.nchunk = 1;
+        EdgeArgs e;
+        e.bt = *b; e.vc = vcz; e.dY = dZ; e.Y = Z; e.P = xrep; e.ld = kv; e.sig = sc.sig;
+        e.rsig = sc.rsig; e.rscale = w->rscale; e.datt = sc.eacc; e.atomic = 1;
+        rc = launch_lagg_bwd(a, e, s);
+        if (rc) return rc;
+        const int wblocks = cdiv((int)d.wslab, 256);
+        ProfScope psu(PROF_PACK, s);
+        unpack_grads_kernel<<<wblocks + cdiv(p->K * EDGE_SLAB, 16), 256, 0, s>>>(gp, pp, d.vc, in, d.ld_in, d.fp, sc.dWcat, d.fslabs, d.wslab,
+                                                                                 sc.eacc, -EDGE_COPIES, sc.rsig, wblocks, b->meta, 0, 1, 0, 0, 1);
+        EAGCN_LAUNCH_CHECK();
+        return EAGCN_OK;
     }
     int nsplit = 0, nedge = 0, xk_G = 0;
     bool bx_slabs = false;
@@ -1295,7 +1374,7 @@
             return EAGCN_ERR_ARG;
         }
         EdgeArgs e;
-        e.bt = *b; e.vc = d.vc; e.dY = sc.dY; e.Y = w->Y; e.P = w->P; e.ld = d.fp; e.sig = sc.sig;
+        e.bt = *b; e.vc = d.vc; e.dY = sc.dY; e.Y = w->Y; e.P = P_used; e.ld = d.fp; e.sig = sc.sig;
         e.rsig = sc.rsig; e.rscale = w->rscale; e.datt = sc.datt; e.atomic = 0;
         static const bool edge_atomic = [] { const char* v = getenv("EAGCN_EDGE_SLABS"); return !(v && v[0] == '1'); }();
         bool general_rel = false;
@@ -1402,7 +1481,7 @@
         ProfScope psu(PROF_PACK, side);
         unpack_grads_kernel<<<wblocks + cdiv(p->K * EDGE_SLAB, 16), 256, 0, side>>>(gp, pp, d.vc, in, d.ld_in, d.fp, sc.dWcat,
                                                                                     bx_slabs ? -nsplit : nsplit, d.wslab, edge_src, nedge, sc.rsig,
-                                                                                    wblocks, b->meta, xk_G, edge_drain, bx_per, bx_wide);
+                                                                                    wblocks, b->meta, xk_G, edge_drain, bx_per, bx_wide, 0);
         EAGCN_LAUNCH_CHECK();
     }
     if (forked) { rc = stream_after(s, side); if (rc) return rc; }
diff --git a/eagcn_amd/ops.py b/eagcn_amd/ops.py
--- a/eagcn_amd/ops.py
+++ b/eagcn_amd/ops.py
@@ -344,7 +344,13 @@
         w = L.LayerBufs()
         w.x, w.P, w.Y, w.rscale, w.bn = x.data_ptr(), P.data_ptr(), Y.data_ptr(), rscale.data_ptr(), bn.data_ptr()
         w.xout, w.pad_row, w.scratch, w.scratch_bytes = xout.data_ptr(), pad_row.data_ptr(), scratch.data_ptr(), nbytes
-        L.check(lib.eagcn_layer_forward(index.ref(), C.byref(p), C.byref(w), _stream()), 'eagcn_layer_forward')
+        ctx.first_off = bool(ctx.needs_input_grad[5])
+        old = lib.eagcn_set_first_layer_mode(0) if ctx.first_off else None
+        try:
+            L.check(lib.eagcn_layer_forward(index.ref(), C.byref(p), C.byref(w), _stream()), 'eagcn_layer_forward')
+        finally:
+            if old is not None:
+                lib.eagcn_set_first_layer_mode(old)
         ctx.index, ctx.spec, ctx.training, ctx.seed, ctx.buffers = index, spec, training, seed, buffers
         ctx.save_for_backward(x, P, Y, rscale, bn, ave_w, *flat)
         if spec.structure == L.STRUCT_CONCATE:
@@ -384,8 +390,13 @@
         if spec.structure == L.STRUCT_WEIGHTED and dpad is not None:
             dpad = dpad.contiguous()
             dpad_ptr = _ptr(dpad)
-        L.check(lib.eagcn_layer_backward(index.ref(), C.byref(p), C.byref(w), _ptr(dxout), dpad_ptr, _ptr(dx),
-                                         C.byref(g), _stream()), 'eagcn_layer_backward')
+        old = lib.eagcn_set_first_layer_mode(0) if ctx.first_off else None
+        try:
+            L.check(lib.eagcn_layer_backward(index.ref(), C.byref(p), C.byref(w), _ptr(dxout), dpad_ptr, _ptr(dx),
+                                             C.byref(g), _stream()), 'eagcn_layer_backward')
+        finally:
+            if old is not None:
+                lib.eagcn_set_first_layer_mode(old)
         return (None, None, None, None, None, dx, dave, *grads)
 
 
diff --git a/include/eagcn_hip.h b/include/eagcn_hip.h
--- a/include/eagcn_hip.h
+++ b/include/eagcn_hip.h
@@ -323,6 +323,7 @@
 int eagcn_bx3_split(const float* x, int rows, int ld, uint16_t* planes, size_t plane_stride, int rows_cap, int np, void* stream);
 int eagcn_bx3_used_splits(int splits, int M, int N, int K);
 int eagcn_set_bx3_wide(int mode);
+int eagcn_set_first_layer_mode(int mode);
 int eagcn_bx3_pair_used_splits(int splits, int M, int N, int K, int M0, int N0, int K0);
 int eagcn_gemm_bx3(int tn, int M, int N, int K, const uint16_t* A, size_t a_pstride, int lda, int a_rows, const uint16_t* B,
                    size_t b_pstride, int ldb, int b_rows, float* C, int ldc, int splits, size_t slab, int np, void* stream);
```

New measurement: 571,100. 0.803x the previous value.
